# FurkanOM/tf-ssd

Measured on AMD Instinct MI355X. Metric: images/sec SSD300 (MobileNetV2) fwd+NMS, higher is better.
Workload: dtype f32

## Files before the change

### include/ssd_hip.h

```cpp
#ifndef SSD_HIP_H
#define SSD_HIP_H

#include <stddef.h>
#include <stdint.h>

#ifdef __cplusplus
extern "C" {
#endif

#define SSD_OK 0
#define SSD_E_INVALID (-1)
#define SSD_E_HIP (-2)
#define SSD_E_UNSUPPORTED (-3)
#define SSD_E_STATE (-4)

const char* ssd_version(void);
const char* ssd_last_error(void);
int ssd_init(int device);
void* ssd_stream_create(int high_priority);
void* ssd_stream_create_masked(const unsigned* cu_mask, int words);
int ssd_stream_destroy(void* stream);

int ssd_priors_count(const int* fmaps, const int* n_ars, int levels);
int ssd_priors(const int* fmaps, const float* const* ars, const int* n_ars, int levels,
// ... 320 lines not shown
int ssd_iou_loc_loss(const float* priors_dev, const float* variances, const float* actual_deltas_dev,
                     const float* pred_deltas_dev, int B, int N, int mode, float loc_loss_alpha,
                     float* loc_loss_dev, float* per_anchor_out_dev, float* grad_deltas_dev, float grad_scale,
                     void* workspace_dev, size_t workspace_bytes, void* stream);

#define SSD_LOSS_HARD_NEGATIVE 0
#define SSD_LOSS_FOCAL 1
typedef struct ssd_loss_config {
    int kind;
    float neg_pos_ratio, loc_loss_alpha, focal_alpha, focal_gamma;
    int loc_kind;
    const float* priors_dev;
    float variances[4];
} ssd_loss_config;
size_t ssd_loss_config_bytes(void);


enum ssd_act { SSD_ACT_NONE = 0, SSD_ACT_RELU = 1, SSD_ACT_RELU6 = 2 };

typedef struct ssd_conv_desc {
    int B, H, W, Cin;
    int Cout, kh, kw;
    int stride, dilation;
    int pad_t, pad_l, pad_b, pad_r;
    int act;
    int has_residual;
} ssd_conv_desc;

int ssd_same_pads(int in, int k, int stride, int dilation, int* before, int* after);
int ssd_conv_out_size(int in, int k, int stride, int dilation, int pad_before, int pad_after);

size_t ssd_conv_packed_weight_floats(int kh, int kw, int Cin, int Cout);
int ssd_conv_pack_weights(const float* hwio_dev, int kh, int kw, int Cin, int Cout,
                          float* packed_dev, void* stream);

int ssd_conv2d(const ssd_conv_desc* d, const float* in_dev, const float* packed_w_dev,
               const float* scale_dev, const float* shift_dev, const float* residual_dev,
               float* out_dev, long out_batch_stride, long out_pixel_stride, void* stream);

int ssd_conv_num_configs(void);
const char* ssd_conv_config_name(int config);
int ssd_conv2d_ex(const ssd_conv_desc* d, const float* in_dev, const float* packed_w_dev,
                  const float* scale_dev, const float* shift_dev, const float* residual_dev,
                  float* out_dev, long out_batch_stride, long out_pixel_stride, int config,
                  int split_k, float* splitk_ws_dev, void* stream);

int ssd_split_planes(const float* x_dev, long n, int channels, int planes, void* planes_dev, long plane_stride, void* stream);
int ssd_join_planes(const void* planes_dev, long n, int channels, int planes, long plane_stride, float* x_dev, void* stream);
int ssd_conv2d_planes(const ssd_conv_desc* d, const void* in_planes_dev, int planes, long in_plane_stride,
                      const float* packed_w_dev, const float* scale_dev, const float* shift_dev,
                      const float* residual_dev, float* out_dev, long out_batch_stride, long out_pixel_stride,
                      void* out_planes_dev, long out_plane_stride, int config, int split_k,
                      float* splitk_ws_dev, void* stream);

size_t ssd_conv_wino_weight_floats(int Cin, int Cout);
int ssd_conv_wino_pack_weights(const float* hwio_dev, int Cin, int Cout, float* wino_w_dev, void* stream);
int ssd_conv_wino_num_configs(void);
int ssd_conv2d_wino(const ssd_conv_desc* d, const float* in_dev, const float* wino_w_dev,
                    const float* scale_dev, const float* shift_dev, float* out_dev,
                    long out_batch_stride, long out_pixel_stride, int wino_config, int split_k,
                    float* splitk_ws_dev, void* stream);

int ssd_dwconv3x3(const float* in_dev, int B, int H, int W, int C, int stride,
                  int pad_t, int pad_l, int pad_b, int pad_r,
                  const float* w_dev, const float* scale_dev, const float* shift_dev,
                  int act, float* out_dev, void* stream);

int ssd_maxpool2d(const float* in_dev, int B, int H, int W, int C, int k, int stride,
                  int pad_t, int pad_l, int pad_b, int pad_r, float* out_dev, void* stream);

int ssd_l2norm(const float* in_dev, long pixels, int C, const float* gamma_dev,
               float* out_dev, void* stream);

int ssd_softmax(const float* in_dev, long rows, int L, float* out_dev, void* stream);

typedef struct ssd_net ssd_net;

enum ssd_backbone { SSD_MOBILENET_V2 = 0, SSD_VGG16 = 1 };

ssd_net* ssd_net_create(int backbone, int img_size, int levels, const int* n_ars,
                        int total_labels);
void ssd_net_destroy(ssd_net* net);

int ssd_net_num_params(const ssd_net* net);
const char* ssd_net_param_name(const ssd_net* net, int i);
int ssd_net_param_rank(const ssd_net* net, int i);
const int* ssd_net_param_shape(const ssd_net* net, int i);
int ssd_net_set_param(ssd_net* net, const char* name, const float* host_data, size_t count);
int ssd_net_get_param(const ssd_net* net, const char* name, float* host_out, size_t count);
int ssd_net_finalize(ssd_net* net, int max_batch);
long ssd_net_get_tuning(const ssd_net* net, char* buf, size_t cap);
int ssd_net_set_tuning(ssd_net* net, const char* text);
int ssd_net_tuning_stats(const ssd_net* net, int* from_table, int* timed);
int ssd_net_memory_bytes(const ssd_net* net, size_t out[4]);
const char* ssd_build_id(void);
int ssd_net_num_priors(const ssd_net* net);
int ssd_net_feature_map_size(const ssd_net* net, int level);

int ssd_net_forward(ssd_net* net, const float* image_dev, int B, float* deltas_out_dev,
                    float* probs_out_dev, void* stream);

int ssd_net_predict(ssd_net* net, const float* image_dev, int B, const float* priors_dev,
                    const float* var, int max_total, float iou_thr, float score_thr,
                    float* boxes_dev, float* labels_dev, float* scores_dev, int* valid_dev,
                    void* stream);
int ssd_net_predict_cfg(ssd_net* net, const float* image_dev, int B, const float* priors_dev, const float* var,
// ... 77 lines not shown
```

### tf-ssd_amd/csrc/ssd_bf16x3.h

```cpp
#pragma once
#include <hip/hip_runtime.h>

namespace ssd {

typedef float b3_f32x4 __attribute__((ext_vector_type(4)));
typedef short bf16x8 __attribute__((ext_vector_type(8)));

struct B3 {
    bf16x8 h, m, l;
};

__device__ __forceinline__ void split1(float x, short& h, short& m, short& l) {
    const unsigned hb = __float_as_uint(x) & 0xffff0000u;
    const float r1 = x - __uint_as_float(hb);
    const unsigned mb = __float_as_uint(r1) & 0xffff0000u;
    const float r2 = r1 - __uint_as_float(mb);
    h = (short)(hb >> 16);
    m = (short)(mb >> 16);
    l = (short)(__float_as_uint(r2) >> 16);
}
__device__ __forceinline__ void split4(const b3_f32x4 v, uint2& h, uint2& m, uint2& l) {
    unsigned hb[4], mb[4], lb[4];
#pragma unroll
    for (int j = 0; j < 4; ++j) {
        hb[j] = __float_as_uint(v[j]) & 0xffff0000u;
        const float r1 = v[j] - __uint_as_float(hb[j]);
        mb[j] = __float_as_uint(r1) & 0xffff0000u;
        lb[j] = __float_as_uint(r1 - __uint_as_float(mb[j]));
    }
    h = make_uint2(__builtin_amdgcn_perm(hb[1], hb[0], 0x07060302u), __builtin_amdgcn_perm(hb[3], hb[2], 0x07060302u));
    m = make_uint2(__builtin_amdgcn_perm(mb[1], mb[0], 0x07060302u), __builtin_amdgcn_perm(mb[3], mb[2], 0x07060302u));
    l = make_uint2(__builtin_amdgcn_perm(lb[1], lb[0], 0x07060302u), __builtin_amdgcn_perm(lb[3], lb[2], 0x07060302u));
}
__device__ __forceinline__ B3 split3(const b3_f32x4 a, const b3_f32x4 b) {
    B3 r;
#pragma unroll
    for (int j = 0; j < 4; ++j) {
        short h, m, l;
        split1(a[j], h, m, l);
        r.h[j] = h; r.m[j] = m; r.l[j] = l;
        split1(b[j], h, m, l);
        r.h[4 + j] = h; r.m[4 + j] = m; r.l[4 + j] = l;
    }
    return r;
}
__device__ __forceinline__ b3_f32x4 mma6(const B3& w, const B3& x, b3_f32x4 acc) {
    acc = __builtin_amdgcn_mfma_f32_16x16x32_bf16(w.m, x.m, acc, 0, 0, 0);
    acc = __builtin_amdgcn_mfma_f32_16x16x32_bf16(w.h, x.l, acc, 0, 0, 0);
    acc = __builtin_amdgcn_mfma_f32_16x16x32_bf16(w.l, x.h, acc, 0, 0, 0);
    acc = __builtin_amdgcn_mfma_f32_16x16x32_bf16(w.h, x.m, acc, 0, 0, 0);
    acc = __builtin_amdgcn_mfma_f32_16x16x32_bf16(w.m, x.h, acc, 0, 0, 0);
    acc = __builtin_amdgcn_mfma_f32_16x16x32_bf16(w.h, x.h, acc, 0, 0, 0);
    return acc;
}

typedef __bf16 bf16x2_t __attribute__((ext_vector_type(2)));
typedef float b3_f32x2 __attribute__((ext_vector_type(2)));

__device__ __forceinline__ unsigned rne2(float a, float b) {
    const bf16x2_t r = __builtin_convertvector(b3_f32x2{a, b}, bf16x2_t);
    return __builtin_bit_cast(unsigned, r);
}
__device__ __forceinline__ short rne1(float a) { return (short)(rne2(a, 0.f) & 0xffffu); }
__device__ __forceinline__ uint2 rne4(const b3_f32x4 v) { return make_uint2(rne2(v[0], v[1]), rne2(v[2], v[3])); }

template <int NP>
struct BP {
    bf16x8 p[NP];
};
template <int NP>
__device__ __forceinline__ BP<NP> splitN(const b3_f32x4 a, const b3_f32x4 b) {
    BP<NP> r;
    if constexpr (NP == 3) {
        const B3 s = split3(a, b);
        r.p[0] = s.h; r.p[1] = s.m; r.p[2] = s.l;
    } else {
        const uint4 u = make_uint4(rne2(a[0], a[1]), rne2(a[2], a[3]), rne2(b[0], b[1]), rne2(b[2], b[3]));
        r.p[0] = __builtin_bit_cast(bf16x8, u);
    }
    return r;
}
template <int NP>
__device__ __forceinline__ b3_f32x4 mmaN(const BP<NP>& w, const BP<NP>& x, b3_f32x4 acc) {
    if constexpr (NP == 3) {
        acc = __builtin_amdgcn_mfma_f32_16x16x32_bf16(w.p[1], x.p[1], acc, 0, 0, 0);
        acc = __builtin_amdgcn_mfma_f32_16x16x32_bf16(w.p[0], x.p[2], acc, 0, 0, 0);
        acc = __builtin_amdgcn_mfma_f32_16x16x32_bf16(w.p[2], x.p[0], acc, 0, 0, 0);
        acc = __builtin_amdgcn_mfma_f32_16x16x32_bf16(w.p[0], x.p[1], acc, 0, 0, 0);
        acc = __builtin_amdgcn_mfma_f32_16x16x32_bf16(w.p[1], x.p[0], acc, 0, 0, 0);
    }
    return __builtin_amdgcn_mfma_f32_16x16x32_bf16(w.p[0], x.p[0], acc, 0, 0, 0);
}
__device__ __forceinline__ void pack_planes(float x, int bf16_mode, short& h, short& m, short& l) {
    if (bf16_mode) { h = rne1(x); m = 0; l = 0; }
    else split1(x, h, m, l);
}

__device__ __host__ __forceinline__ long plane_elem(const long pix, const int c, const long P) {
    return (((long)(c >> 5) * P + pix) << 5) + (c & 31);
}
__device__ __forceinline__ void store_planes4(short* __restrict__ op, const long plane, const int np, const long pix, const int c,
                                              const long P, const b3_f32x4 v) {
    const long e = plane_elem(pix, c, P);
    if (np == 1) {
        *reinterpret_cast<uint2*>(op + e) = rne4(v);
    } else {
        uint2 h, m, l;
        split4(v, h, m, l);
        *reinterpret_cast<uint2*>(op + e) = h;
        *reinterpret_cast<uint2*>(op + plane + e) = m;
        *reinterpret_cast<uint2*>(op + 2 * plane + e) = l;
    }
}
__device__ __forceinline__ void store_planes4_lin(short* __restrict__ op, const long plane, const int np, const long e, const int C,
                                                  const long P, const b3_f32x4 v) {
    const long pix = e / C;
    store_planes4(op, plane, np, pix, (int)(e - pix * C), P, v);
}

}
```

### tf-ssd_amd/csrc/ssd_conv.h

```cpp
#pragma once
#include "common.h"

namespace ssd {

struct ConvParams {
    const float* in;
    const float* w;
    const short* w3;
    const float* scale;
    const float* shift;
    const float* residual;
    float* out;
    int B, H, W, Cin, Ho, Wo, Cout;
    int kh, kw, stride, dil, pad_t, pad_l;
    int K, Kpad, Npad;
    long M;
    long out_batch_stride, out_pixel_stride;
    int n_split;
    float* out2;
    long out2_batch_stride, out2_pixel_stride;
    int vec_store2;
    int act;
    int vec_store;
    int split_k;
    float* partial;
    const float* wino_w;
    int bf16;
    const short* xp;
    long xp_plane;
    int xp_np;
    short* op;
    long op_plane;
    int op_np;
};
bool conv_config_allowed(int cfg, int precision);
inline int conv_vec_store(const ConvParams& p) {
    return (((uintptr_t)p.out & 15) == 0) && (p.out_pixel_stride % 4 == 0) && (p.out_batch_stride % 4 == 0);
}

struct FusedBlockParams {
    const float* x;
    float* y;
    const float* we;
    const float *es, *eh;
    const float* wd;
    const float *ds, *dh;
    const float* wp;
    const float *ps, *ph;
    int residual;
    int B, H, W, Cin, Ce, Cout, Ho, Wo, stride, pad_t, pad_l;
    int kpad_e, kpad_p, npad_p;
    int tiles_y, tiles_x;
    int bf16;
    int groups;
    const short* we3;
    const short* wp3;
    int bands;
    float* slabs;
    unsigned* tickets;
    float* e_out;
    short* y_planes;
    long y_plane;
    short* e_planes;
    long e_plane;
    int planes_np;
    int planes_only;
    int form2;
};
struct StemParams {
    const float* x;
    float* y;
    const float* w1;
    const float *s1, *h1;
    const float* wd;
    const float *sd, *hd;
    const float* wp;
    const float *sp, *hp;
    int B, H, W, H1, W1, pad_t, pad_l, kpad1, kpadp;
    int tiles_y, tiles_x;
    int bf16;
};
struct DwProjParams {
    const float* e;
    const float* wd;
    const float* dh;
    const float* wp;
    const float* ph;
    const float* res;
    float* y;
    int B, H, W, Ce, Cout, Ho, Wo, stride, pad_t, pad_l;
    int kpad_p, npad_p;
    int tiles_y, tiles_x;
    int bf16;
};
bool dwproj_supported(const DwProjParams& p);
int launch_dwproj(DwProjParams p, hipStream_t st);
bool stem_supported(const StemParams& p);
int launch_stem(StemParams p, hipStream_t st);
bool image_block2_supported(const FusedBlockParams& p);
int launch_image_block2(FusedBlockParams p, hipStream_t st);
bool fused_block_supported(const FusedBlockParams& p);
int launch_fused_block(FusedBlockParams p, hipStream_t st);
bool band3_block_supported(const FusedBlockParams& p);
size_t band3_we_shorts(int Ce);
size_t band3_wp_shorts(int npad_p, int Ce);
int launch_band3_pack(const float* we, int Ce, int Cin, int kpad_e, short* we3, const float* wp, int npad_p, int kpad_p,
                      short* wp3, hipStream_t st);
int launch_band3_block(FusedBlockParams p, hipStream_t st);
bool band_block_supported(const FusedBlockParams& p);
int launch_band_block(FusedBlockParams p, hipStream_t st);
bool image_block_supported(const FusedBlockParams& p);
bool image_block_split_fits(FusedBlockParams p);
int image_block_groups(const FusedBlockParams& p, int B);
size_t image_block_slab_floats(const FusedBlockParams& p, int B);
int launch_image_block(FusedBlockParams p, hipStream_t st);

inline int round_up(int v, int a) { return (v + a - 1) / a * a; }
inline int conv_kpad(int K) { return round_up(K, 32); }
inline int conv_npad(int Cout) { return round_up(Cout, 16); }

int conv_num_configs();
const char* conv_config_name(int cfg);
bool conv_config_valid(int cfg, const ConvParams& p);
int conv_pick_config(const ConvParams& p);
long conv_grid_blocks(int cfg, const ConvParams& p);
int conv_k_tiles(int cfg, const ConvParams& p);
int conv_launch(const ConvParams& p, int cfg, hipStream_t st);
size_t conv_splitk_workspace_floats(const ConvParams& p, int cfg);

int fill_conv_params(const ssd_conv_desc* d, ConvParams* p);
int launch_splitk_reduce(const ConvParams& p, hipStream_t st);

int conv_num_mfma_configs();
int wino_num_configs();
const char* wino_config_name(int i);
bool wino_applicable(const ConvParams& p);
bool wino_config_valid(int i, const ConvParams& p);
long wino_grid_blocks(int i, const ConvParams& p);
int wino_k_tiles(const ConvParams& p);
int wino_launch(const ConvParams& p, int i, hipStream_t st);
size_t wino_weight_floats(int Cin, int Cout);
int launch_wino_pack(const float* hwio, int Cin, int Cout, int Npad, int row_off, float* U, hipStream_t st);

int skinny_num_configs();
const char* skinny_config_name(int i);
bool skinny_config_valid(int i, const ConvParams& p);
long skinny_grid_blocks(int i, const ConvParams& p);
int skinny_launch(const ConvParams& p, int i, hipStream_t st);

int mfma3_num_configs();
const char* mfma3_config_name(int i);
bool mfma3_config_valid(int i, const ConvParams& p);
long mfma3_grid_blocks(int i, const ConvParams& p);
int mfma3_k_tiles(const ConvParams& p);
void mfma3_tile(int i, int* BM, int* BN);
int mfma3_launch(const ConvParams& p, int i, hipStream_t st, bool bf16 = false);
const char* bf16_config_name(int i);

int dma_num_configs();
const char* dma_config_name(int i, int np);
bool dma_config_valid(int i, int np, const ConvParams& p);
long dma_grid_blocks(int i, const ConvParams& p);
int dma_k_tiles(int np, const ConvParams& p);
void dma_tile(int i, int* BM, int* BN);
int dma_launch(const ConvParams& p, int i, int np, hipStream_t st);
int launch_split_planes(const float* x, long n, int C, int np, short* planes, long plane, hipStream_t st);
int launch_join_planes(const short* planes, long n, int C, int np, long plane, float* x, hipStream_t st);
bool conv_config_is_dma(int cfg);
bool conv_config_writes_planes(int cfg, const ConvParams& p);

int launch_dwconv3x3(const float* in, int B, int H, int W, int C, int stride, int pad_t, int pad_l,
                     int Ho, int Wo, const float* w, const float* scale, const float* shift, int act,
                     float* out, hipStream_t st);
int launch_maxpool(const float* in, int B, int H, int W, int C, int k, int stride, int pad_t, int pad_l,
                   int Ho, int Wo, float* out, hipStream_t st, short* planes = nullptr, long plane = 0, int np = 0);
int launch_l2norm(const float* in, long pixels, int C, const float* gamma, float* out, hipStream_t st,
                  short* planes = nullptr, long plane = 0, int np = 0);
int launch_softmax(const float* in, long rows, int L, float* out, hipStream_t st);
bool decode_nms_fused_ok(int L);
int decode_nms_fused(const float* deltas, const float* logits, const float* priors, const float* var, int B, int N, int L,
                     int max_per_class, int max_total, float iou_thr, float score_thr, float* boxes, float* labels,
                     float* scores, int* valid, void* ws, size_t ws_bytes, int ws_batch, hipStream_t st);
int decode_nms_fused_cfg(const float* deltas, const float* logits, const float* priors, const float* var, int B, int N, int L,
                         const ssd_nms_config* cfg, float* boxes, float* labels, float* scores, int* valid, void* ws,
                         size_t ws_bytes, int ws_batch, hipStream_t st);
int launch_pack_weights(const float* hwio, int K, int Cout, int Kpad, int Npad, float* packed, hipStream_t st);
inline size_t conv_packed_floats(int K, int Cout) {
    const size_t n = (size_t)conv_kpad(K) * conv_npad(Cout);
    return n + 2 * n;
}
inline const short* conv_split_planes(const float* packed, int K, int Cout) {
    return reinterpret_cast<const short*>(packed + (size_t)conv_kpad(K) * conv_npad(Cout));
}
int launch_pack_split(float* packed, int K, int Cout, hipStream_t st, bool row_major = false);
int launch_scale_rows(const float* in, const float* scale, int rows, int nvalid, int cols, float* out, hipStream_t st);
int launch_scale_cols(const float* in, const float* scale, int rows, int cols, float* out, hipStream_t st);
int launch_fold_bn(const float* gamma, const float* beta, const float* mean, const float* var, float eps,
                   int C, float* scale, float* shift, hipStream_t st);

}
```

### tf-ssd_amd/csrc/ssd_conv.hip

```cpp
#include "ssd_conv.h"
#include "ssd_conv_mfma.h"

namespace ssd {


template <int V>
__global__ void splitk_reduce_kernel(const ConvParams p) {
    const long total = p.M * p.Cout;
    const long groups = total / V;
    const int HoWo = p.Ho * p.Wo;
    for (long g = (long)blockIdx.x * blockDim.x + threadIdx.x; g < groups; g += (long)gridDim.x * blockDim.x) {
        float t[V];
#pragma unroll
        for (int j = 0; j < V; ++j) t[j] = 0.f;
        for (int s = 0; s < p.split_k; ++s) {
            const float* src = p.partial + (long)s * total + g * V;
            if (V == 4) {
                const f32x4 v = *reinterpret_cast<const f32x4*>(src);
#pragma unroll
                for (int j = 0; j < V; ++j) t[j] += v[j];
            } else {
                t[0] += src[0];
            }
        }
// ... 168 lines not shown
struct ConvCfg {
    const char* name;
    int BM, BN, BK;
    conv_kernel_t gemm, general;
};
#define CFG(MT, NT, WM, WN, BK)                                                            \
    {"mfma_" #MT "x" #NT "_" #WM "x" #WN "_k" #BK, 16 * MT * WM, 16 * NT * WN, BK,          \
     conv_mfma_kernel<MT, NT, WM, WN, BK, true>, conv_mfma_kernel<MT, NT, WM, WN, BK, false>}
static const ConvCfg kCfgs[] = {
    CFG(2, 1, 4, 1, 32),
    CFG(2, 2, 4, 1, 32),
    CFG(2, 4, 4, 1, 32),
    CFG(2, 6, 4, 1, 32),
    CFG(2, 4, 2, 2, 32),
    CFG(1, 2, 2, 2, 32),
    CFG(4, 4, 2, 2, 32),
    CFG(1, 1, 4, 1, 32),
    CFG(2, 9, 4, 1, 32),
    CFG(2, 12, 4, 1, 32),
    CFG(1, 4, 1, 4, 32),
    CFG(2, 2, 2, 2, 32),
    CFG(2, 6, 4, 1, 16),
    CFG(1, 2, 1, 4, 32),
    CFG(4, 2, 4, 1, 32),
    CFG(2, 8, 2, 2, 32),
    CFG(2, 7, 4, 1, 32),
    CFG(2, 5, 2, 2, 32),
    CFG(1, 7, 4, 1, 32),
    CFG(1, 5, 2, 2, 32),
    CFG(4, 3, 2, 2, 32),
    CFG(4, 6, 2, 2, 32),
    CFG(1, 7, 4, 1, 64),
    CFG(1, 5, 2, 2, 64),
    CFG(2, 7, 4, 1, 64),
    CFG(2, 5, 2, 2, 64),
    CFG(1, 2, 2, 2, 64),
    CFG(2, 4, 2, 2, 64),
    CFG(1, 1, 4, 1, 64),
    CFG(2, 2, 2, 2, 64),
    CFG(4, 5, 2, 2, 32),
    CFG(4, 7, 4, 1, 32),
    CFG(4, 4, 4, 1, 32),
    CFG(4, 6, 4, 1, 32),
    CFG(4, 3, 4, 1, 32),
    CFG(4, 5, 4, 1, 32),
    CFG(2, 10, 2, 2, 32),
};
constexpr int kNumMfmaCfgs = sizeof(kCfgs) / sizeof(kCfgs[0]);
static int skinny_cfg0() { return kNumMfmaCfgs + wino_num_configs(); }
static int mfma3_cfg0() { return kNumMfmaCfgs + wino_num_configs() + skinny_num_configs(); }
static int bf16_cfg0() { return kNumMfmaCfgs + wino_num_configs() + skinny_num_configs() + mfma3_num_configs(); }
static int dma3_cfg0() { return kNumMfmaCfgs + wino_num_configs() + skinny_num_configs() + 2 * mfma3_num_configs(); }
static int dmab_cfg0() { return dma3_cfg0() + dma_num_configs(); }
static int direct_cfg() { return dma3_cfg0() + 2 * dma_num_configs(); }
#define kSkinnyCfg0 skinny_cfg0()
#define kMfma3Cfg0 mfma3_cfg0()
#define kBf16Cfg0 bf16_cfg0()
#define kDma3Cfg0 dma3_cfg0()
#define kDmabCfg0 dmab_cfg0()
#define kDirectCfg direct_cfg()
bool conv_config_is_dma(int cfg) { return cfg >= kDma3Cfg0 && cfg < kDirectCfg; }
bool conv_config_writes_planes(int cfg, const ConvParams& p) {
    if (cfg == kDirectCfg) return stem_ok(p);
    return (cfg >= 0 && cfg < kNumMfmaCfgs) || (cfg >= kMfma3Cfg0 && cfg < kDirectCfg);
}

int conv_num_mfma_configs() { return kNumMfmaCfgs; }
int conv_num_configs() { return kDirectCfg + 1; }
const char* conv_config_name(int cfg) {
    if (cfg == kDirectCfg) return "direct_valu";
    if (cfg >= kDmabCfg0 && cfg < kDirectCfg) return dma_config_name(cfg - kDmabCfg0, 1);
    if (cfg >= kDma3Cfg0 && cfg < kDmabCfg0) return dma_config_name(cfg - kDma3Cfg0, 3);
    if (cfg >= kBf16Cfg0 && cfg < kDma3Cfg0) return bf16_config_name(cfg - kBf16Cfg0);
    if (cfg >= kMfma3Cfg0 && cfg < kBf16Cfg0) return mfma3_config_name(cfg - kMfma3Cfg0);
    if (cfg >= kSkinnyCfg0 && cfg < kMfma3Cfg0) return skinny_config_name(cfg - kSkinnyCfg0);
    if (cfg >= kNumMfmaCfgs && cfg < kSkinnyCfg0) return wino_config_name(cfg - kNumMfmaCfgs);
    if (cfg < 0 || cfg >= kNumMfmaCfgs) return "?";
    return kCfgs[cfg].name;
}

bool conv_config_allowed(int cfg, int precision) {
    const bool bf16 = (cfg >= kBf16Cfg0 && cfg < kDma3Cfg0) || (cfg >= kDmabCfg0 && cfg < kDirectCfg);
    if (!precision) return !bf16;
    const bool split = (cfg >= kMfma3Cfg0 && cfg < kBf16Cfg0) || (cfg >= kDma3Cfg0 && cfg < kDmabCfg0);
    const bool wino = cfg >= kNumMfmaCfgs && cfg < kSkinnyCfg0;
    return !split && !wino;
}

static bool is_gemm1x1(const ConvParams& p) {
    return p.kh == 1 && p.kw == 1 && p.stride == 1 && p.pad_t == 0 && p.pad_l == 0 && p.Ho == p.H && p.Wo == p.W;
}

bool conv_config_valid(int cfg, const ConvParams& p) {
    if (cfg == kDirectCfg) return (size_t)p.K * ((p.Cout + 3) & ~3) * 4 <= 64 * 1024;
    if (cfg >= kDmabCfg0 && cfg < kDirectCfg) return dma_config_valid(cfg - kDmabCfg0, 1, p);
    if (cfg >= kDma3Cfg0 && cfg < kDmabCfg0) return dma_config_valid(cfg - kDma3Cfg0, 3, p);
    if (cfg >= kBf16Cfg0 && cfg < kDma3Cfg0) return mfma3_config_valid(cfg - kBf16Cfg0, p);
    if (cfg >= kMfma3Cfg0 && cfg < kBf16Cfg0) return mfma3_config_valid(cfg - kMfma3Cfg0, p);
    if (cfg >= kSkinnyCfg0 && cfg < kMfma3Cfg0) return skinny_config_valid(cfg - kSkinnyCfg0, p);
    if (cfg >= kNumMfmaCfgs && cfg < kSkinnyCfg0) return wino_config_valid(cfg - kNumMfmaCfgs, p);
    if (cfg < 0 || cfg >= kNumMfmaCfgs) return false;
    if (((uintptr_t)p.in & 15) || ((uintptr_t)p.w & 15)) return false;
    if (p.Cin % 4) return false;
    if (p.M > 0x7fffffffL - 1024) return false;
    if (is_gemm1x1(p)) return true;
    if (p.kh * p.kw > 32) return false;
    return p.Cin % kCfgs[cfg].BK == 0;
}

int conv_pick_config(const ConvParams& p) {
    int best = -1;
    double best_cost = 1e300;
    for (int c = 0; c < kNumMfmaCfgs; ++c) {
        if (!conv_config_valid(c, p)) continue;
        const ConvCfg& g = kCfgs[c];
        const double mb = (double)((p.M + g.BM - 1) / g.BM), nb = (double)((p.Cout + g.BN - 1) / g.BN);
        const double kk = (double)round_up(p.K, g.BK);
        const double blocks = mb * nb;
        const double waves = ceil(blocks / 256.0);
        const double t_mfma = waves * (double)g.BM * g.BN * kk * 2.0 / (157.3e12 / 256.0);
        const double bytes = (mb * g.BM * kk * nb + nb * g.BN * kk * mb) * 4.0 + (double)p.M * p.Cout * 4.0;
        const double t_mem = bytes / 6.0e12;
        const double cost = (t_mfma > t_mem ? t_mfma : t_mem) + 0.25 * (t_mfma < t_mem ? t_mfma : t_mem);
        if (cost < best_cost) { best_cost = cost; best = c; }
    }
    if (p.w3 && p.M >= 2048 && p.K >= 64) {
        for (int c = 0; c < mfma3_num_configs(); ++c) {
            if (!mfma3_config_valid(c, p)) continue;
            int BM, BN;
            mfma3_tile(c, &BM, &BN);
            const double mb = (double)((p.M + BM - 1) / BM), nb = (double)((p.Cout + BN - 1) / BN);
            const double kk = (double)round_up(p.K, 32);
            const double waves = ceil(mb * nb / 256.0);
            const double t_mfma = waves * (double)BM * BN * kk * 2.0 / ((p.bf16 ? 1000e12 : 260e12) / 256.0);
            const double bytes = mb * BM * kk * nb * 4.0 + nb * BN * kk * mb * (p.bf16 ? 2.0 : 6.0) + (double)p.M * p.Cout * 4.0;
            const double t_mem = bytes / 6.0e12;
            const double cost = (t_mfma > t_mem ? t_mfma : t_mem) + 0.25 * (t_mfma < t_mem ? t_mfma : t_mem);
            if (cost < best_cost) { best_cost = cost; best = (p.bf16 ? kBf16Cfg0 : kMfma3Cfg0) + c; }
        }
    }
    if (best < 0 && conv_config_valid(kDirectCfg, p)) best = kDirectCfg;
    return best;
}

long conv_grid_blocks(int cfg, const ConvParams& p) {
    if (cfg >= kDmabCfg0 && cfg < kDirectCfg) return dma_grid_blocks(cfg - kDmabCfg0, p);
    if (cfg >= kDma3Cfg0 && cfg < kDmabCfg0) return dma_grid_blocks(cfg - kDma3Cfg0, p);
    if (cfg >= kBf16Cfg0 && cfg < kDma3Cfg0) return mfma3_grid_blocks(cfg - kBf16Cfg0, p);
    if (cfg >= kMfma3Cfg0 && cfg < kBf16Cfg0) return mfma3_grid_blocks(cfg - kMfma3Cfg0, p);
    if (cfg >= kSkinnyCfg0 && cfg < kMfma3Cfg0) return skinny_grid_blocks(cfg - kSkinnyCfg0, p);
    if (cfg >= kNumMfmaCfgs && cfg < kSkinnyCfg0) return wino_grid_blocks(cfg - kNumMfmaCfgs, p);
    if (cfg < 0 || cfg >= kNumMfmaCfgs) return 0;
    const ConvCfg& g = kCfgs[cfg];
    return ((p.M + g.BM - 1) / g.BM) * ((p.Cout + g.BN - 1) / g.BN);
}
int conv_k_tiles(int cfg, const ConvParams& p) {
    if (cfg >= kDma3Cfg0 && cfg < kDirectCfg) return dma_k_tiles(cfg >= kDmabCfg0 ? 1 : 3, p);
    if (cfg >= kMfma3Cfg0 && cfg < kDma3Cfg0) return mfma3_k_tiles(p);
    if (cfg >= kSkinnyCfg0 && cfg < kMfma3Cfg0) return p.K / 16;
    if (cfg >= kNumMfmaCfgs && cfg < kSkinnyCfg0) return wino_k_tiles(p);
    if (cfg < 0 || cfg >= kNumMfmaCfgs) return 0;
    return (p.K + kCfgs[cfg].BK - 1) / kCfgs[cfg].BK;
}

size_t conv_splitk_workspace_floats(const ConvParams& p, int) {
    return p.split_k > 1 ? (size_t)p.split_k * p.M * p.Cout : 0;
}

int conv_launch(const ConvParams& p, int cfg, hipStream_t st) {
    if (p.M == 0 || p.Cout == 0) return SSD_OK;
    if (!conv_config_valid(cfg, p)) {
        set_error("conv2d: config %d (%s) cannot run Cin=%d k=%dx%d stride=%d", cfg, conv_config_name(cfg),
                  p.Cin, p.kh, p.kw, p.stride);
        return SSD_E_UNSUPPORTED;
    }
    SSD_UNSUPPORTED_IF(!p.out && !(p.op && !p.n_split && (p.Cout & 3) == 0 && conv_config_writes_planes(cfg, p)),
                       "conv2d: config %s cannot write a plane-only output", conv_config_name(cfg));
    if (cfg >= kDma3Cfg0 && cfg < kDirectCfg) {
        const bool b1 = cfg >= kDmabCfg0;
        const int rc = dma_launch(p, cfg - (b1 ? kDmabCfg0 : kDma3Cfg0), b1 ? 1 : 3, st);
        if (rc || p.split_k <= 1) return rc;
        return launch_splitk_reduce(p, st);
    }
    if (cfg >= kMfma3Cfg0 && cfg < kDma3Cfg0) {
        const bool bf16 = cfg >= kBf16Cfg0;
        const int rc = mfma3_launch(p, cfg - (bf16 ? kBf16Cfg0 : kMfma3Cfg0), st, bf16);
        if (rc || p.split_k <= 1) return rc;
        return launch_splitk_reduce(p, st);
    }
    if (cfg >= kSkinnyCfg0 && cfg < kMfma3Cfg0) return skinny_launch(p, cfg - kSkinnyCfg0, st);
    if (cfg >= kNumMfmaCfgs && cfg < kSkinnyCfg0) {
        const int rc = wino_launch(p, cfg - kNumMfmaCfgs, st);
        if (rc || p.split_k <= 1) return rc;
        return launch_splitk_reduce(p, st);
    }
    if (cfg == kDirectCfg && stem_ok(p)) {
        constexpr int PX = 2;
        const long blocks = cdiv(p.M, 256 * PX);
        dim3 grid((unsigned)(blocks < 65535 ? blocks : 65535), p.Cout / 32);
        hipLaunchKernelGGL(conv_stem_kernel<PX>, grid, dim3(256), 0, st, p);
        SSD_LAUNCH_CHECK();
        return SSD_OK;
    }
    if (cfg == kDirectCfg) {
        const long total = p.M * ((p.Cout + 3) / 4);
        const int blocks = (int)(cdiv(total, 256) < 8192 ? cdiv(total, 256) : 8192);
        const size_t lds = (size_t)p.K * ((p.Cout + 3) & ~3) * 4;
        hipLaunchKernelGGL(conv_direct_kernel, dim3(blocks), dim3(256), lds, st, p);
        SSD_LAUNCH_CHECK();
        return SSD_OK;
    }
    const ConvCfg& g = kCfgs[cfg];
    const long mb = (p.M + g.BM - 1) / g.BM;
    const int nb = (p.Cout + g.BN - 1) / g.BN;
    SSD_UNSUPPORTED_IF(mb * nb > 0x7fffffffL, "conv2d: grid too large");
    dim3 grid((unsigned)(mb * nb), p.split_k > 1 ? p.split_k : 1);
    conv_kernel_t k = is_gemm1x1(p) ? g.gemm : g.general;
    hipLaunchKernelGGL(k, grid, dim3(256), 0, st, p);
    SSD_LAUNCH_CHECK();
    if (p.split_k > 1) return launch_splitk_reduce(p, st);
    return SSD_OK;
}

int launch_splitk_reduce(const ConvParams& p, hipStream_t st) {
    const long total = p.M * p.Cout;
    const bool vec = (total % 4 == 0) && (((uintptr_t)p.partial & 15) == 0);
    SSD_UNSUPPORTED_IF(!vec && !p.out, "conv2d: a plane-only output needs the 4-wide split-K reduce (16-byte aligned workspace)");
    const long groups = vec ? total / 4 : total;
    const int blocks = (int)(cdiv(groups, 256) < 8192 ? cdiv(groups, 256) : 8192);
    if (vec) hipLaunchKernelGGL(splitk_reduce_kernel<4>, dim3(blocks), dim3(256), 0, st, p);
    else hipLaunchKernelGGL(splitk_reduce_kernel<1>, dim3(blocks), dim3(256), 0, st, p);
// ... 64 lines not shown
    if (kh < 1 || kw < 1 || Cin < 1 || Cout < 1) return 0;
    return conv_packed_floats(kh * kw * Cin, Cout);
}

int ssd_conv_pack_weights(const float* hwio_dev, int kh, int kw, int Cin, int Cout, float* packed_dev,
                          void* stream) {
    SSD_CHECK_ARG(hwio_dev && packed_dev, "ssd_conv_pack_weights: NULL pointer");
    SSD_CHECK_ARG(kh >= 1 && kw >= 1 && Cin >= 1 && Cout >= 1, "ssd_conv_pack_weights: bad shape");
    const int K = kh * kw * Cin;
    int rc = launch_pack_weights(hwio_dev, K, Cout, conv_kpad(K), conv_npad(Cout), packed_dev, (hipStream_t)stream);
    if (!rc) rc = launch_pack_split(packed_dev, K, Cout, (hipStream_t)stream);
    return rc;
}

int ssd_conv_num_configs(void) { return conv_num_configs(); }
const char* ssd_conv_config_name(int cfg) { return conv_config_name(cfg); }

int ssd_conv2d_ex(const ssd_conv_desc* d, const float* in_dev, const float* packed_w_dev,
                  const float* scale_dev, const float* shift_dev, const float* residual_dev, float* out_dev,
                  long out_batch_stride, long out_pixel_stride, int config, int split_k,
                  float* splitk_ws_dev, void* stream) {
    ConvParams p;
    int rc = fill_conv_params(d, &p);
    if (rc) return rc;
    if (p.M == 0) return SSD_OK;
    SSD_CHECK_ARG(in_dev && packed_w_dev && out_dev, "conv2d: NULL pointer");
    SSD_CHECK_ARG(!d->has_residual || residual_dev, "conv2d: has_residual set but residual is NULL");
    p.in = in_dev; p.w = packed_w_dev; p.scale = scale_dev; p.shift = shift_dev;
    p.w3 = conv_split_planes(packed_w_dev, p.K, p.Cout);
    p.residual = d->has_residual ? residual_dev : nullptr;
    p.out = out_dev;
    p.out_pixel_stride = out_pixel_stride > 0 ? out_pixel_stride : p.Cout;
    p.out_batch_stride = out_batch_stride > 0 ? out_batch_stride : (long)p.Ho * p.Wo * p.out_pixel_stride;
    p.vec_store = (((uintptr_t)out_dev & 15) == 0) && (p.out_pixel_stride % 4 == 0) && (p.out_batch_stride % 4 == 0);
    if (split_k > 1) {
        SSD_CHECK_ARG(splitk_ws_dev != nullptr, "conv2d: split_k > 1 needs a workspace");
        p.split_k = split_k;
        p.partial = splitk_ws_dev;
    }
    const int cfg = config >= 0 ? config : conv_pick_config(p);
    SSD_UNSUPPORTED_IF(cfg < 0, "conv2d: no kernel for Cin=%d Cout=%d k=%dx%d", p.Cin, p.Cout, p.kh, p.kw);
    if (cfg == conv_num_configs() - 1) p.split_k = 1;
    return conv_launch(p, cfg, (hipStream_t)stream);
}

int ssd_split_planes(const float* x_dev, long n, int channels, int planes, void* planes_dev, long plane_stride, void* stream) {
    SSD_CHECK_ARG(x_dev && planes_dev && n >= 0, "ssd_split_planes: bad arguments");
    SSD_CHECK_ARG(plane_stride >= n && plane_stride % 8 == 0, "ssd_split_planes: plane_stride %ld must be >= n and a multiple of 8", plane_stride);
    SSD_CHECK_ARG((((uintptr_t)x_dev | (uintptr_t)planes_dev) & 15) == 0, "ssd_split_planes: pointers must be 16-byte aligned");
    return launch_split_planes(x_dev, n, channels, planes, static_cast<short*>(planes_dev), plane_stride, (hipStream_t)stream);
}

int ssd_join_planes(const void* planes_dev, long n, int channels, int planes, long plane_stride, float* x_dev, void* stream) {
    SSD_CHECK_ARG(x_dev && planes_dev && n >= 0 && (planes == 1 || planes == 3) && plane_stride >= n, "ssd_join_planes: bad arguments");
    return launch_join_planes(static_cast<const short*>(planes_dev), n, channels, planes, plane_stride, x_dev, (hipStream_t)stream);
}

int ssd_conv2d_planes(const ssd_conv_desc* d, const void* in_planes_dev, int planes, long in_plane_stride,
                      const float* packed_w_dev, const float* scale_dev, const float* shift_dev, const float* residual_dev,
                      float* out_dev, long out_batch_stride, long out_pixel_stride, void* out_planes_dev,
                      long out_plane_stride, int config, int split_k, float* splitk_ws_dev, void* stream) {
    ConvParams p;
    int rc = fill_conv_params(d, &p);
    if (rc) return rc;
    if (p.M == 0) return SSD_OK;
    SSD_CHECK_ARG(in_planes_dev && packed_w_dev && (out_dev || out_planes_dev), "conv2d_planes: NULL pointer");
    SSD_CHECK_ARG(planes == 1 || planes == 3, "conv2d_planes: planes must be 1 (bf16 mode) or 3 (exact split)");
    SSD_CHECK_ARG(in_plane_stride >= (long)p.B * p.H * p.W * p.Cin, "conv2d_planes: in_plane_stride shorter than the tensor");
    SSD_CHECK_ARG(!d->has_residual || residual_dev, "conv2d_planes: has_residual set but residual is NULL");
    SSD_CHECK_ARG(config >= 0 && config < conv_num_configs() && conv_config_is_dma(config), "conv2d_planes: config %d is not an LDS-DMA tile", config);
    p.xp = static_cast<const short*>(in_planes_dev); p.xp_plane = in_plane_stride; p.xp_np = planes;
    p.bf16 = planes == 1;
    p.w = packed_w_dev; p.scale = scale_dev; p.shift = shift_dev;
    p.w3 = conv_split_planes(packed_w_dev, p.K, p.Cout);
    p.residual = d->has_residual ? residual_dev : nullptr;
    p.out = out_dev;
    p.out_pixel_stride = out_pixel_stride > 0 ? out_pixel_stride : p.Cout;
    p.out_batch_stride = out_batch_stride > 0 ? out_batch_stride : (long)p.Ho * p.Wo * p.out_pixel_stride;
    p.vec_store = (((uintptr_t)out_dev & 15) == 0) && (p.out_pixel_stride % 4 == 0) && (p.out_batch_stride % 4 == 0);
    if (out_planes_dev) {
        SSD_CHECK_ARG(p.out_pixel_stride == p.Cout && p.out_batch_stride == (long)p.Ho * p.Wo * p.Cout && p.Cout % 4 == 0,
                      "conv2d_planes: plane output needs a dense [B,Ho,Wo,Cout] destination with Cout %% 4 == 0");
        SSD_CHECK_ARG(out_plane_stride >= p.M * ((p.Cout + 31) / 32 * 32) && out_plane_stride % 8 == 0 && ((uintptr_t)out_planes_dev & 7) == 0,
                      "conv2d_planes: bad out_plane_stride (whole 32-channel slices of all %ld pixels) or unaligned planes", p.M);
        p.op = static_cast<short*>(out_planes_dev); p.op_plane = out_plane_stride; p.op_np = planes;
    }
    if (split_k > 1) {
        SSD_CHECK_ARG(splitk_ws_dev != nullptr, "conv2d_planes: split_k > 1 needs a workspace");
        p.split_k = split_k;
        p.partial = splitk_ws_dev;
    }
    return conv_launch(p, config, (hipStream_t)stream);
}

size_t ssd_conv_wino_weight_floats(int Cin, int Cout) {
    if (Cin < 1 || Cout < 1) return 0;
    return wino_weight_floats(Cin, Cout);
}

int ssd_conv_wino_pack_weights(const float* hwio_dev, int Cin, int Cout, float* wino_w_dev, void* stream) {
    SSD_CHECK_ARG(hwio_dev && wino_w_dev && Cin >= 1 && Cout >= 1, "ssd_conv_wino_pack_weights: bad arguments");
    SSD_HIP(hipMemsetAsync(wino_w_dev, 0, wino_weight_floats(Cin, Cout) * sizeof(float), (hipStream_t)stream));
    return launch_wino_pack(hwio_dev, Cin, Cout, conv_npad(Cout), 0, wino_w_dev, (hipStream_t)stream);
}

int ssd_conv_wino_num_configs(void) { return wino_num_configs(); }

int ssd_conv2d_wino(const ssd_conv_desc* d, const float* in_dev, const float* wino_w_dev, const float* scale_dev,
                    const float* shift_dev, float* out_dev, long out_batch_stride, long out_pixel_stride,
                    int wino_config, int split_k, float* splitk_ws_dev, void* stream) {
    ConvParams p;
    int rc = fill_conv_params(d, &p);
    if (rc) return rc;
    if (p.M == 0) return SSD_OK;
    SSD_CHECK_ARG(in_dev && wino_w_dev && out_dev, "conv2d_wino: NULL pointer");
    SSD_CHECK_ARG(!d->has_residual, "conv2d_wino: residual is not supported");
    p.in = in_dev; p.wino_w = wino_w_dev; p.scale = scale_dev; p.shift = shift_dev;
    p.out = out_dev;
    p.out_pixel_stride = out_pixel_stride > 0 ? out_pixel_stride : p.Cout;
    p.out_batch_stride = out_batch_stride > 0 ? out_batch_stride : (long)p.Ho * p.Wo * p.out_pixel_stride;
// ... 21 lines not shown
```

### tf-ssd_amd/csrc/ssd_convdma.hip

```cpp
#include "ssd_block_common.h"
#include "ssd_conv_mfma.h"

namespace ssd {

template <int MT, int NT, int WM, int WN, int NP, bool GEMM1X1>
__device__ __forceinline__ void conv_dma_body(const ConvParams& p, char* __restrict__ dsm) {
    constexpr int KS = NP == 1 ? 2 : 1;
    constexpr int WPL = NP == 1 ? 3 : 0;
    constexpr int BM = 16 * MT * WM, BN = 16 * NT * WN, NW = WM * WN;
    constexpr int RBX = BM / 16, RBW = BN / 16;
    constexpr int RPX = (RBX + NW - 1) / NW, RPW = (RBW + NW - 1) / NW;
    constexpr int XBYTES = KS * NP * BM * 64, STAGE = KS * NP * (BM + BN) * 64;

    const int tid = threadIdx.x, lane = tid & 63;
    const int wave = __builtin_amdgcn_readfirstlane(tid >> 6);
    const int wm = wave / WN, wn = wave % WN;
    const int nb_n = (p.Cout + BN - 1) / BN;
    const int mblk = blockIdx.x / nb_n, nblk = blockIdx.x - mblk * nb_n;
    const long m0 = (long)mblk * BM;
    const int n0 = nblk * BN;
    const int HoWo = p.Ho * p.Wo;
    const int ntaps = p.kh * p.kw;

    const int r16 = lane >> 2;
    const int q8 = ((lane & 3) ^ ((lane >> 3) & 3)) * 8;
    const int b_first = (int)(m0 / HoWo);
    const long npix = (long)p.B * p.H * p.W;
    const long xbase_e = (GEMM1X1 ? m0 : (long)b_first * p.H * p.W) * 32;
    const long xrange = min((long)0x7fffffffL, (npix * p.Cin - xbase_e) * 2);
    const int slice_b = (int)(npix * 64);
    __amdgpu_buffer_rsrc_t xrs[NP];
#pragma unroll
    for (int pl = 0; pl < NP; ++pl)
        xrs[pl] = __builtin_amdgcn_make_buffer_rsrc(const_cast<short*>(p.xp + pl * p.xp_plane + xbase_e), 0, (int)xrange, 0x00020000);
    const long wplane_b = (long)p.Npad * p.Kpad * 2;
    const __amdgpu_buffer_rsrc_t wrs = __builtin_amdgcn_make_buffer_rsrc(const_cast<short*>(p.w3), 0, (int)(4 * wplane_b), 0x00020000);

    int xoff[RPX];
    unsigned xvalid[RPX];
#pragma unroll
    for (int j = 0; j < RPX; ++j) {
        const int rb = wave + j * NW;
        const long m = m0 + rb * 16 + r16;
        xoff[j] = 0;
        xvalid[j] = 0;
        if (rb < RBX && m < p.M) {
            if (GEMM1X1) {
                xoff[j] = ((rb * 16 + r16) * 32 + q8) * 2;
                xvalid[j] = 1u;
            } else {
                const int b = (int)(m / HoWo);
                const int pix = (int)(m - (long)b * HoWo);
                const int oy = pix / p.Wo, ox = pix - oy * p.Wo;
                const int iy0 = oy * p.stride - p.pad_t, ix0 = ox * p.stride - p.pad_l;
                xoff[j] = ((((b - b_first) * p.H + iy0) * p.W + ix0) * 32 + q8) * 2;
                for (int ky = 0; ky < p.kh; ++ky)
                    for (int kx = 0; kx < p.kw; ++kx) {
                        const int iy = iy0 + ky * p.dil, ix = ix0 + kx * p.dil;
                        if ((unsigned)iy < (unsigned)p.H && (unsigned)ix < (unsigned)p.W) xvalid[j] |= 1u << (ky * p.kw + kx);
                    }
            }
        }
    }
    int woff[RPW];
#pragma unroll
    for (int j = 0; j < RPW; ++j) {
        const int rb = wave + j * NW;
        const int r = min(rb * 16 + r16, min(BN, p.Npad - n0) - 1);
        woff[j] = ((n0 + r) * 32 + q8) * 2;
    }

    const int nks = p.K / 32;
    const int ntiles = GEMM1X1 ? (nks + KS - 1) / KS : ntaps * (p.Cin / (32 * KS));
    int kt_begin = 0, kt_end = ntiles;
    if (p.split_k > 1) {
        const int per = (ntiles + p.split_k - 1) / p.split_k;
        kt_begin = blockIdx.y * per;
        kt_end = min(ntiles, kt_begin + per);
    }
    int l_k0 = 0, l_tap = 0, l_ci = 0, l_ky = 0, l_kx = 0, l_xtile = 0, l_xs = 0;
    auto tile_setup = [&](int kt) {
        if (GEMM1X1) {
            l_k0 = kt * 32 * KS;
            l_xtile = 0;
            l_xs = kt * KS * slice_b;
        } else {
            const int cs = kt / ntaps;
            l_tap = kt - cs * ntaps;
            l_ci = cs * 32 * KS;
            l_ky = l_tap / p.kw;
            l_kx = l_tap - l_ky * p.kw;
            l_k0 = l_tap * p.Cin + l_ci;
            l_xtile = (l_ky * p.dil * p.W + l_kx * p.dil) * 64;
            l_xs = (l_ci >> 5) * slice_b;
        }
    };
    auto tile_advance = [&]() {
        if (GEMM1X1) {
            l_k0 += 32 * KS;
            l_xs += KS * slice_b;
        } else {
            ++l_tap;
            if (++l_kx == p.kw) { l_kx = 0; ++l_ky; }
            if (l_tap == ntaps) { l_tap = 0; l_ky = 0; l_kx = 0; l_ci += 32 * KS; }
            l_k0 = l_tap * p.Cin + l_ci;
            l_xtile = (l_ky * p.dil * p.W + l_kx * p.dil) * 64;
            l_xs = (l_ci >> 5) * slice_b;
        }
    };
    auto steps_here = [&]() -> int { return KS == 1 ? 1 : min(KS, nks - l_k0 / 32); };

    auto issue = [&](int stage) {
        char* sb = dsm + stage * STAGE;
        const int ns = steps_here();
#pragma unroll
        for (int j = 0; j < RPX; ++j) {
            const int rb = wave + j * NW;
            if (RBX % NW != 0 && rb >= RBX) continue;
            const bool ok = GEMM1X1 ? (xvalid[j] != 0) : (((xvalid[j] >> l_tap) & 1u) != 0);
            const int vo = ok ? xoff[j] + l_xtile : (int)0x80000000;
#pragma unroll
            for (int s = 0; s < KS; ++s) {
                if (KS > 1 && s >= ns) break;
#pragma unroll
                for (int pl = 0; pl < NP; ++pl)
                    __builtin_amdgcn_raw_ptr_buffer_load_lds(xrs[pl], (lds_dst_t)(sb + ((s * NP + pl) * BM + rb * 16) * 64), 16, vo, l_xs + s * slice_b, 0, 0);
            }
        }
#pragma unroll
        for (int j = 0; j < RPW; ++j) {
            const int rb = wave + j * NW;
            if (RBW % NW != 0 && rb >= RBW) continue;
#pragma unroll
            for (int s = 0; s < KS; ++s) {
                if (KS > 1 && s >= ns) break;
#pragma unroll
                for (int pl = 0; pl < NP; ++pl)
                    __builtin_amdgcn_raw_ptr_buffer_load_lds(wrs, (lds_dst_t)(sb + XBYTES + ((s * NP + pl) * BN + rb * 16) * 64), 16, woff[j],
                                                             (int)((pl + WPL) * wplane_b) + ((l_k0 >> 5) + s) * p.Npad * 64, 0, 0);
            }
        }
    };

    f32x4 acc[MT][NT];
#pragma unroll
    for (int mi = 0; mi < MT; ++mi)
#pragma unroll
        for (int ni = 0; ni < NT; ++ni) acc[mi][ni] = f32x4{0.f, 0.f, 0.f, 0.f};

    const int frow = lane & 15;
    const int fq = ((lane >> 4) ^ ((frow >> 1) & 3)) << 4;
    auto mma_tile = [&](int stage, int ns) {
        const char* sb = dsm + stage * STAGE;
#pragma unroll
        for (int s = 0; s < KS; ++s) {
            if (KS > 1 && s >= ns) break;
            const char* Xb = sb + s * NP * BM * 64;
            const char* Wb = sb + XBYTES + s * NP * BN * 64;
            BP<NP> b[MT];
#pragma unroll
            for (int mi = 0; mi < MT; ++mi) {
                const char* r = Xb + ((wm * MT + mi) * 16 + frow) * 64 + fq;
#pragma unroll
                for (int pl = 0; pl < NP; ++pl) b[mi].p[pl] = *reinterpret_cast<const bf16x8*>(r + pl * BM * 64);
            }
#pragma unroll
            for (int ni = 0; ni < NT; ++ni) {
                const char* r = Wb + ((wn * NT + ni) * 16 + frow) * 64 + fq;
                BP<NP> a;
#pragma unroll
                for (int pl = 0; pl < NP; ++pl) a.p[pl] = *reinterpret_cast<const bf16x8*>(r + pl * BN * 64);
#pragma unroll
                for (int mi = 0; mi < MT; ++mi) acc[mi][ni] = mmaN<NP>(a, b[mi], acc[mi][ni]);
            }
        }
    };

    int ns_cur = 1;
    if (kt_begin < kt_end) {
        tile_setup(kt_begin);
        ns_cur = steps_here();
        issue(0);
    }
    asm volatile("s_waitcnt vmcnt(0)" ::: "memory");
    __syncthreads();
    for (int kt = kt_begin; kt < kt_end; ++kt) {
        const int stage = (kt - kt_begin) & 1;
        int ns_next = 1;
        if (kt + 1 < kt_end) {
            tile_advance();
            ns_next = steps_here();
            issue(stage ^ 1);
        }
        mma_tile(stage, ns_cur);
        ns_cur = ns_next;
        asm volatile("s_waitcnt vmcnt(0)" ::: "memory");
        __syncthreads();
    }
    conv_epilogue<MT, NT>(p, acc, m0, n0, wm, wn, lane, HoWo);
}

template <int MT, int NT, int WM, int WN, int NP, bool GEMM1X1>
__global__ __launch_bounds__(64 * WM * WN) void conv_dma_kernel(const ConvParams p) {
    extern __shared__ __attribute__((aligned(1024))) char dsm_dma[];
    conv_dma_body<MT, NT, WM, WN, NP, GEMM1X1>(p, dsm_dma);
}

namespace {

typedef void (*convd_kernel_t)(const ConvParams);
struct ConvDCfg {
    const char* name3;
    const char* name1;
    int BM, BN, threads;
    convd_kernel_t gemm3, general3, gemm1, general1;
};
#define DCFG(MT, NT, WM, WN)                                                                                  \
    {"dma3_" #MT "x" #NT "_" #WM "x" #WN, "dmab_" #MT "x" #NT "_" #WM "x" #WN, 16 * MT * WM, 16 * NT * WN, 64 * WM * WN, \
     conv_dma_kernel<MT, NT, WM, WN, 3, true>, conv_dma_kernel<MT, NT, WM, WN, 3, false>,                       \
     conv_dma_kernel<MT, NT, WM, WN, 1, true>, conv_dma_kernel<MT, NT, WM, WN, 1, false>}
const ConvDCfg kCfgD[] = {
    DCFG(4, 4, 4, 2),
    DCFG(2, 4, 4, 2),
    DCFG(4, 4, 2, 4),
    DCFG(4, 2, 4, 2),
    DCFG(2, 7, 8, 1),
    DCFG(4, 5, 4, 2),
    DCFG(4, 4, 2, 2),
    DCFG(2, 7, 4, 1),
    DCFG(2, 5, 2, 2),
    DCFG(2, 4, 6, 2),
    DCFG(3, 4, 4, 3),
    DCFG(2, 4, 8, 2),
    DCFG(2, 2, 2, 2),
    DCFG(2, 5, 6, 2),
};
constexpr int kNumCfgD = sizeof(kCfgD) / sizeof(kCfgD[0]);

bool cd_gemm1x1(const ConvParams& p) {
    return p.kh == 1 && p.kw == 1 && p.stride == 1 && p.pad_t == 0 && p.pad_l == 0 && p.Ho == p.H && p.Wo == p.W;
}

__global__ __launch_bounds__(256) void split_planes_kernel(const float* __restrict__ x, const long n4, const int C, const int np,
                                                           short* __restrict__ planes, const long plane) {
    const long P = n4 * 4 / C;
    for (long e = (long)blockIdx.x * 256 + threadIdx.x; e < n4; e += (long)gridDim.x * 256)
        store_planes4_lin(planes, plane, np, e * 4, C, P, *reinterpret_cast<const f32x4*>(x + e * 4));
}

__global__ __launch_bounds__(256) void join_planes_kernel(const short* __restrict__ planes, const long n, const int C, const int np,
                                                          const long plane, float* __restrict__ x) {
    const long P = n / C;
    for (long e = (long)blockIdx.x * 256 + threadIdx.x; e < n; e += (long)gridDim.x * 256) {
        const long pix = e / C;
        const long s = plane_elem(pix, (int)(e - pix * C), P);
        float v = __uint_as_float((unsigned)(unsigned short)planes[s] << 16);
        if (np == 3) {
            v += __uint_as_float((unsigned)(unsigned short)planes[plane + s] << 16);
            v += __uint_as_float((unsigned)(unsigned short)planes[2 * plane + s] << 16);
        }
        x[e] = v;
    }
}

}

int dma_num_configs() { return kNumCfgD; }
const char* dma_config_name(int i, int np) { return (i >= 0 && i < kNumCfgD) ? (np == 1 ? kCfgD[i].name1 : kCfgD[i].name3) : "?"; }
bool dma_config_valid(int i, int np, const ConvParams& p) {
    if (i < 0 || i >= kNumCfgD) return false;
    if (!p.xp || !p.w3 || p.xp_np != np) return false;
    if (((uintptr_t)p.xp & 15) || ((uintptr_t)p.w3 & 15) || (p.xp_plane & 7)) return false;
    if (p.M > 0x7fffffffL - 1024) return false;
    if (4 * (long)p.Npad * p.Kpad * 2 > 0x7fffffffL) return false;
    if ((long)p.B * p.H * p.W * p.Cin * 2 > 0x7fffffffL) return false;
    if (cd_gemm1x1(p)) return p.Cin % 32 == 0;
    if (p.kh * p.kw > 32) return false;
    if (((long)kCfgD[i].BM / (p.Ho * p.Wo) + 3) * p.H * p.W * 64 > 0x3fffffffL) return false;
    return p.Cin % (np == 1 ? 64 : 32) == 0;
}
long dma_grid_blocks(int i, const ConvParams& p) {
    if (i < 0 || i >= kNumCfgD) return 0;
    return ((p.M + kCfgD[i].BM - 1) / kCfgD[i].BM) * ((p.Cout + kCfgD[i].BN - 1) / kCfgD[i].BN);
}
int dma_k_tiles(int np, const ConvParams& p) { return (p.K + 31) / 32 / (np == 1 ? 2 : 1); }
void dma_tile(int i, int* BM, int* BN) {
    *BM = (i >= 0 && i < kNumCfgD) ? kCfgD[i].BM : 0;
    *BN = (i >= 0 && i < kNumCfgD) ? kCfgD[i].BN : 0;
}

int dma_launch(const ConvParams& p, int i, int np, hipStream_t st) {
    if (!dma_config_valid(i, np, p)) {
        set_error("conv2d: LDS-DMA config %d cannot run Cin=%d k=%dx%d (input planes %s)", i, p.Cin, p.kh, p.kw, p.xp ? "present" : "missing");
        return SSD_E_UNSUPPORTED;
    }
    const long blocks = dma_grid_blocks(i, p);
    SSD_UNSUPPORTED_IF(blocks > 0x7fffffffL, "conv2d: grid too large");
    const ConvDCfg& g = kCfgD[i];
    const convd_kernel_t fn = np == 1 ? (cd_gemm1x1(p) ? g.gemm1 : g.general1) : (cd_gemm1x1(p) ? g.gemm3 : g.general3);
    const int lds = 2 * (np == 1 ? 2 : 3) * (g.BM + g.BN) * 64;
    if (lds > 64 * 1024) SSD_HIP(hipFuncSetAttribute(reinterpret_cast<const void*>(fn), hipFuncAttributeMaxDynamicSharedMemorySize, lds));
    dim3 grid((unsigned)blocks, p.split_k > 1 ? p.split_k : 1);
    hipLaunchKernelGGL(fn, grid, dim3(g.threads), lds, st, p);
    SSD_LAUNCH_CHECK();
    return SSD_OK;
}

int launch_split_planes(const float* x, long n, int C, int np, short* planes, long plane, hipStream_t st) {
    SSD_CHECK_ARG(n % 4 == 0 && (np == 1 || np == 3), "split_planes: element count %ld must be a multiple of 4, planes 1 or 3", n);
    SSD_CHECK_ARG(C > 0 && C % 32 == 0 && n % C == 0, "split_planes: %d channels (slice-major planes need a multiple of 32 that divides the %ld elements)", C, n);
    SSD_UNSUPPORTED_IF((((uintptr_t)x) & 15) || (((uintptr_t)planes) & 7) || (plane & 3),
                       "split_planes: needs a 16-byte aligned source and 8-byte aligned planes (16-byte loads, 8-byte stores)");
    if (n == 0) return SSD_OK;
    const long n4 = n / 4;
    const int blocks = (int)((n4 + 255) / 256 < 16384 ? (n4 + 255) / 256 : 16384);
    hipLaunchKernelGGL(split_planes_kernel, dim3(blocks), dim3(256), 0, st, x, n4, C, np, planes, plane);
    SSD_LAUNCH_CHECK();
    return SSD_OK;
}

int launch_join_planes(const short* planes, long n, int C, int np, long plane, float* x, hipStream_t st) {
    if (n == 0) return SSD_OK;
    SSD_CHECK_ARG(C > 0 && n % C == 0, "join_planes: %d channels do not divide the %ld elements", C, n);
    const int blocks = (int)((n + 255) / 256 < 16384 ? (n + 255) / 256 : 16384);
    hipLaunchKernelGGL(join_planes_kernel, dim3(blocks), dim3(256), 0, st, planes, n, C, np, plane, x);
    SSD_LAUNCH_CHECK();
    return SSD_OK;
}

}
```

### tf-ssd_amd/csrc/ssd_imgblock.hip

```cpp

#include "ssd_bf16x3.h"
#include "ssd_block_common.h"
#include "ssd_conv.h"

namespace ssd {

namespace {

constexpr int kIC = 16;
constexpr int kILD = 24;
constexpr int kIThreads = 512;

__device__ __forceinline__ void gstore16_sc1(float* ptr, f32x4 v) {
    asm volatile("global_store_dwordx4 %0, %1, off sc1\n\ts_nop 1" ::"v"(ptr), "v"(v) : "memory");
}

template <int CIN, int NT, int T, int S = 1>
__global__ __launch_bounds__(kIThreads) void mbv2_image_block_kernel(const FusedBlockParams p) {
    constexpr int TO = S == 1 ? T : 1;
    constexpr int KC = CIN / 16;
    constexpr int LDW = CIN + 8;
    constexpr int NCH = T == 1 ? 2 : 1;
    constexpr int WE_U = kIC * CIN / 4, WE_R = (WE_U + kIThreads - 1) / kIThreads;
    constexpr int WP_U = NT * 16 * kIC / 4, WP_R = (WP_U + kIThreads - 1) / kIThreads;
// ... 87 lines not shown
            opo[t] = opix[t];
            realo[t] = real[t];
        } else {
            const int Po = Wo + 1, tile = wave * TO + t;
            const int q = tile * 16 + l15;
            const int ro = q / Po, co = q - ro * Po;
            realo[t] = tile * 16 < Ho * Po && q < Ho * Po && co < Wo;
            qo[t] = (tile * 16 < Ho * Po && q < Ho * Po) ? (2 * ro - p.pad_t + 1) * P + (2 * co - p.pad_l + 1) : 0;
            opo[t] = realo[t] ? ro * Wo + co : 0;
        }
    }
    for (int u = tid; u < 11 * (CeG / 4); u += kIThreads) {
        const int row = u / (CeG / 4), c4 = (u - row * (CeG / 4)) * 4;
        const float* src = row == 0 ? p.eh : row == 10 ? p.dh : p.wd + (long)(row - 1) * p.Ce;
        *reinterpret_cast<f32x4*>(Ps + row * CeG + c4) = *reinterpret_cast<const f32x4*>(src + cbeg + c4);
    }
    wait_prefetch(wer0);
    store_we_from(wer0, 0);
    wait_prefetch(wpr);
    store_wp(0);
    if (nchunk > 1) { wait_prefetch(wer); store_we(1); }
    __syncthreads();

    auto expand = [&](int j) {
        f32x4 ea[T][NCH];
        const f32x4 sh = *reinterpret_cast<const f32x4*>(Ps + j * kIC + g4 * 4);
#pragma unroll
        for (int t = 0; t < T; ++t) {
            ea[t][0] = sh;
            if (NCH == 2) ea[t][NCH - 1] = f32x4{0.f, 0.f, 0.f, 0.f};
        }
        const float* wes = Wes + ((j & 1) * kIC + l15) * LDW + g4 * 4;
#pragma unroll
        for (int kc = 0; kc < KC; ++kc) {
            const f32x4 wa = *reinterpret_cast<const f32x4*>(wes + kc * 16);
#pragma unroll
            for (int s = 0; s < 4; ++s)
#pragma unroll
                for (int t = 0; t < T; ++t)
                    ea[t][kc % NCH] = __builtin_amdgcn_mfma_f32_16x16x4f32(wa[s], xb[t][kc][s], ea[t][kc % NCH], 0, 0, 0);
        }
        float* es = Es + ((j & 1) * NE + P + 1) * kILD + g4 * 4;
#pragma unroll
        for (int t = 0; t < T; ++t) {
            f32x4 v = ea[t][0];
            if (NCH == 2) v = v + ea[t][NCH - 1];
            const float hi = real[t] ? 6.0f : 0.0f;
#pragma unroll
            for (int e = 0; e < 4; ++e) v[e] = __builtin_amdgcn_fmed3f(v[e], 0.0f, hi);
            if (tvalid[t]) *reinterpret_cast<f32x4*>(es + qs[t] * kILD) = v;
            if (p.e_out && real[t]) {
                const long eo = ((long)img * H * W + opix[t]) * p.Ce + cbeg + j * kIC + g4 * 4;
                if (!(p.planes_only & 2)) *reinterpret_cast<f32x4*>(p.e_out + eo) = v;
                if (p.e_planes) store_planes4(p.e_planes, p.e_plane, p.planes_np, (long)img * H * W + opix[t], cbeg + j * kIC + g4 * 4, (long)B * H * W, v);
            }
        }
    };

    f32x4 acc[TO][NT];
#pragma unroll
    for (int t = 0; t < TO; ++t)
#pragma unroll
        for (int ni = 0; ni < NT; ++ni) acc[t][ni] = f32x4{0.f, 0.f, 0.f, 0.f};

    expand(0);
    if (nchunk > 1) {
        load_wp(1);
        if (nchunk > 2) load_we(2);
    }

    for (int i = 0; i < nchunk; ++i) {
        lds_barrier();
        if (i + 1 < nchunk) {
            wait_prefetch(wpr);
            store_wp((i + 1) & 1);
            if (i + 2 < nchunk) {
                wait_prefetch(wer);
                store_we(i & 1);
                load_wp(i + 2);
                if (i + 3 < nchunk) load_we(i + 3);
            }
        }
        f32x4 a[TO];
        {
            const f32x4 dh = *reinterpret_cast<const f32x4*>(Ps + 10 * CeG + i * kIC + g4 * 4);
#pragma unroll
            for (int t = 0; t < TO; ++t) a[t] = dh;
            const float* es = Es + ((i & 1) * NE + P + 1) * kILD + g4 * 4;
#pragma unroll
            for (int dy = -1; dy <= 1; ++dy)
#pragma unroll
                for (int dx = -1; dx <= 1; ++dx) {
                    const f32x4 w = *reinterpret_cast<const f32x4*>(Ps + (1 + (dy + 1) * 3 + dx + 1) * CeG + i * kIC + g4 * 4);
#pragma unroll
                    for (int t = 0; t < TO; ++t) {
                        const f32x4 e = *reinterpret_cast<const f32x4*>(es + (qo[t] + dy * P + dx) * kILD);
                        a[t] += e * w;
                    }
                }
#pragma unroll
            for (int t = 0; t < TO; ++t)
#pragma unroll
                for (int e = 0; e < 4; ++e) a[t][e] = __builtin_amdgcn_fmed3f(a[t][e], 0.0f, 6.0f);
        }
        __builtin_amdgcn_sched_barrier(0);
        {
            const float* wps = Wps + ((i & 1) * NT * 16 + l15) * kILD + g4 * 4;
// ... 192 lines not shown
            const int ro = q / Po, co = q - ro * Po;
            realo[t] = tile * 16 < Ho * Po && q < Ho * Po && co < Wo;
            qo[t] = (tile * 16 < Ho * Po && q < Ho * Po) ? (2 * ro - p.pad_t + 1) * P + (2 * co - p.pad_l + 1) : 0;
            opo[t] = realo[t] ? ro * Wo + co : 0;
        }
    }
    for (int u = tid; u < 11 * (CeG / 4); u += kIThreads) {
        const int row = u / (CeG / 4), c4 = (u - row * (CeG / 4)) * 4;
        const float* src = row == 0 ? p.eh : row == 10 ? p.dh : p.wd + (long)(row - 1) * p.Ce;
        *reinterpret_cast<f32x4*>(Ps + row * CeG + c4) = *reinterpret_cast<const f32x4*>(src + cbeg + c4);
    }
    {
        bf16x8 w0[WE_N], w1[WE_N];
        stage_we_load_to(w0, 0);
        stage_we_load_to(w1, nchunk > 1 ? 1 : 0);
        stage_wp_load(0);
        stage_we_store_from(w0, 0);
        stage_we_store_from(w1, 1);
        stage_wp_store();
        if (nchunk > 2) stage_we_load(2);
        if (nchunk > 2) stage_wp_load(1);
    }
    __syncthreads();

    auto expand = [&](int j) {
        f32x4 ea[T][NCH];
        const f32x4 sh = *reinterpret_cast<const f32x4*>(Ps + j * kIC + g4 * 4);
#pragma unroll
        for (int t = 0; t < T; ++t) {
            ea[t][0] = sh;
            if (NCH == 2) ea[t][NCH - 1] = f32x4{0.f, 0.f, 0.f, 0.f};
        }
        const short* wl = Wes + ((j & 1) * NP * 16 + l15) * SEH + g4 * 8;
#pragma unroll
        for (int ks = 0; ks < KS; ++ks) {
            BP<NP> wea;
#pragma unroll
            for (int pl = 0; pl < NP; ++pl) wea.p[pl] = *reinterpret_cast<const bf16x8*>(wl + pl * 16 * SEH + ks * 32);
#pragma unroll
            for (int t = 0; t < T; ++t) ea[t][ks % NCH] = mmaN<NP>(wea, xs[t][ks], ea[t][ks % NCH]);
        }
        float* es = Es + ((j & 1) * NE + P + 1) * kILD + g4 * 4;
#pragma unroll
        for (int t = 0; t < T; ++t) {
            f32x4 v = ea[t][0];
            if (NCH == 2) v = v + ea[t][NCH - 1];
            const float hi = real[t] ? 6.0f : 0.0f;
#pragma unroll
            for (int e = 0; e < 4; ++e) v[e] = __builtin_amdgcn_fmed3f(v[e], 0.0f, hi);
            if (tvalid[t]) *reinterpret_cast<f32x4*>(es + qs[t] * kILD) = v;
            if (p.e_out && real[t]) {
                const long eo = ((long)img * H * W + opix[t]) * p.Ce + cbeg + j * kIC + g4 * 4;
                if (!(p.planes_only & 2)) *reinterpret_cast<f32x4*>(p.e_out + eo) = v;
                if (p.e_planes) store_planes4(p.e_planes, p.e_plane, p.planes_np, (long)img * H * W + opix[t], cbeg + j * kIC + g4 * 4, (long)B * H * W, v);
            }
        }
    };

    f32x4 acc[TO][NT];
#pragma unroll
    for (int t = 0; t < TO; ++t)
#pragma unroll
        for (int ni = 0; ni < NT; ++ni) acc[t][ni] = f32x4{0.f, 0.f, 0.f, 0.f};

    expand(0);
    f32x4 dprev[TO];

    for (int i = 0; i < nchunk; ++i) {
        lds_barrier();
        const bool odd = i & 1;
        const bool flush = odd || i + 1 == nchunk;
        {
            if (i + 2 < nchunk) stage_we_store(i & 1);
            if (i + 3 < nchunk) stage_we_load(i + 3);
            if (!odd && i > 0 && i + 1 < nchunk) {
                stage_wp_store();
                if (i + 2 < nchunk) stage_wp_load((i >> 1) + 1);
            }
        }
        f32x4 a[TO];
        {
            const f32x4 dh = *reinterpret_cast<const f32x4*>(Ps + 10 * CeG + i * kIC + g4 * 4);
#pragma unroll
            for (int t = 0; t < TO; ++t) a[t] = dh;
            const float* es = Es + ((i & 1) * NE + P + 1) * kILD + g4 * 4;
#pragma unroll
            for (int dy = -1; dy <= 1; ++dy)
#pragma unroll
                for (int dx = -1; dx <= 1; ++dx) {
                    const f32x4 w = *reinterpret_cast<const f32x4*>(Ps + (1 + (dy + 1) * 3 + dx + 1) * CeG + i * kIC + g4 * 4);
#pragma unroll
                    for (int t = 0; t < TO; ++t) {
                        const f32x4 e = *reinterpret_cast<const f32x4*>(es + (qo[t] + (S == 1 ? dy * P + dx : dy * P + dx)) * kILD);
                        a[t] += e * w;
                    }
                }
#pragma unroll
            for (int t = 0; t < TO; ++t)
#pragma unroll
                for (int e = 0; e < 4; ++e) a[t][e] = __builtin_amdgcn_fmed3f(a[t][e], 0.0f, 6.0f);
        }
        if (!flush) {
#pragma unroll
            for (int t = 0; t < TO; ++t) dprev[t] = a[t];
        } else {
            BP<NP> d[TO];
#pragma unroll
// ... 194 lines not shown
```

### tf-ssd_amd/csrc/ssd_imgblock2.hip

```cpp

#include "ssd_bf16x3.h"
#include "ssd_block_common.h"
#include "ssd_conv.h"

namespace ssd {

namespace {

constexpr int kC = 16;

template <int CIN, int NT, int NW, int T, int H, int W, int NP, int LOOP, int S = 1>
__device__ __forceinline__ void image16v2_body(const FusedBlockParams& p, float* __restrict__ sm2) {
    static_assert(CIN % 32 == 0, "whole 32-channel k-steps");
    constexpr int NTH = NW * 64;
    constexpr int P = W + 1, Q = H * P;
    static_assert(NW * 16 * T >= Q, "the waves' pixel slots cover the padded map");
    constexpr int NPIX = NW * 16 * T;
    constexpr int NE = NPIX + 2 * P + 2;
    constexpr int ROW = S == 2 ? 20 : (T & 1) ? 24 : 20;
    static_assert(((S == 2 ? 2 : T) * ROW) % 16 == 8, "neighbouring lanes must sit 8 (mod 16) words apart");
    constexpr int TO = S == 1 ? T : 1;
    constexpr int Ho = S == 1 ? H : (H + 1) / 2, Wo = S == 1 ? W : (W + 1) / 2, Po = Wo + 1;
    static_assert(S == 1 || NW * 16 >= Ho * Po, "stride 2: one output pixel per lane covers the output map");
    constexpr int WPL = NP == 1 ? 3 : 0;
// ... 71 lines not shown
        const float* src = row == 0 ? p.eh : row == 10 ? p.dh : p.wd + (long)(row - 1) * p.Ce;
        const int w = c4 & 31, j = 2 * (c4 >> 5) + ((w >> 2) & 1), r = (w >> 3) * 4;
        *reinterpret_cast<f32x4*>(Ps + (j * 11 + row) * kC + r) = *reinterpret_cast<const f32x4*>(src + cbeg + c4);
    }
    dma_wait();
    __syncthreads();

    const float* e_rd = Es + (q0 + P + 1) * ROW + g4 * 4;
    float* e_wr = Es + (q0 + P + 1) * ROW + g4 * 4;
    const float* ps_l = Ps + g4 * 4;
    const int fslot = l15 * 32 + ((g4 ^ ((l15 >> 1) & 3)) * 8);
    const short* we_l = Wes + fslot;
    const short* wp_l = Wps + fslot;
    float relu_hi[T];
#pragma unroll
    for (int t = 0; t < T; ++t) relu_hi[t] = real[t] ? 6.0f : 0.0f;
    bool realo[TO];
    int opo[TO];
    if constexpr (S == 1) {
#pragma unroll
        for (int t = 0; t < T; ++t) { realo[t] = real[t]; opo[t] = opix[t]; }
    } else {
        const int qo = wave * 16 + l15, ro = qo / Po, co = qo - ro * Po;
        const bool in = qo < Ho * Po;
        realo[0] = in && co < Wo;
        opo[0] = realo[0] ? ro * Wo + co : 0;
        e_rd = Es + ((in ? (2 * ro - p.pad_t + 1) * P + (2 * co - p.pad_l + 1) : 0) + P + 1) * ROW + g4 * 4;
    }

    auto expand = [&](const int j, const int pb) {
        f32x4 ea[T];
        const f32x4 sh = *reinterpret_cast<const f32x4*>(ps_l + j * PCH);
#pragma unroll
        for (int t = 0; t < T; ++t) ea[t] = sh;
        const short* wl = we_l + pb * NBE * 512;
#pragma unroll
        for (int ks = 0; ks < KS; ++ks) {
            BP<NP> wea;
#pragma unroll
            for (int pl = 0; pl < NP; ++pl) wea.p[pl] = *reinterpret_cast<const bf16x8*>(wl + (pl * KS + ks) * 512);
#pragma unroll
            for (int t = 0; t < T; ++t) ea[t] = mmaN<NP>(wea, xs[t][ks], ea[t]);
        }
        float* ew = e_wr + pb * EBUF;
#pragma unroll
        for (int t = 0; t < T; ++t) {
            f32x4 v = ea[t];
#pragma unroll
            for (int e = 0; e < 4; ++e) v[e] = __builtin_amdgcn_fmed3f(v[e], 0.0f, relu_hi[t]);
            *reinterpret_cast<f32x4*>(ew + t * ROW) = v;
            if (S == 2 && p.e_out && real[t]) {
                const int ch = cbeg + (j >> 1) * 32 + g4 * 8 + (j & 1) * 4;
                if (!(p.planes_only & 2)) *reinterpret_cast<f32x4*>(p.e_out + ((long)img * (H * W) + opix[t]) * p.Ce + ch) = v;
                if (p.e_planes) store_planes4(p.e_planes, p.e_plane, p.planes_np, (long)img * (H * W) + opix[t], ch, (long)B * (H * W), v);
            }
        }
    };
    auto depthwise = [&](const int i, const int pb, f32x4 (&a)[TO]) {
        const float* pc = ps_l + i * PCH;
        const f32x4 dh = *reinterpret_cast<const f32x4*>(pc + 10 * kC);
#pragma unroll
        for (int t = 0; t < TO; ++t) a[t] = dh;
        const float* es = e_rd + pb * EBUF;
#pragma unroll
        for (int dy = -1; dy <= 1; ++dy) {
            f32x4 w[3], e[TO + 2];
#pragma unroll
            for (int dx = 0; dx < 3; ++dx) w[dx] = *reinterpret_cast<const f32x4*>(pc + (1 + (dy + 1) * 3 + dx) * kC);
#pragma unroll
            for (int j = 0; j < TO + 2; ++j)
                e[j] = *reinterpret_cast<const f32x4*>(es + (dy * P + j - 1) * ROW);
#pragma unroll
            for (int dx = 0; dx < 3; ++dx)
#pragma unroll
                for (int t = 0; t < TO; ++t) a[t] += e[t + dx] * w[dx];
        }
#pragma unroll
        for (int t = 0; t < TO; ++t)
#pragma unroll
            for (int e = 0; e < 4; ++e) a[t][e] = __builtin_amdgcn_fmed3f(a[t][e], 0.0f, 6.0f);
    };
    f32x4 acc[TO][NT];
#pragma unroll
    for (int t = 0; t < TO; ++t)
#pragma unroll
        for (int ni = 0; ni < NT; ++ni) acc[t][ni] = f32x4{0.f, 0.f, 0.f, 0.f};
    auto project = [&](const f32x4 (&a0)[TO], const f32x4 (&a1)[TO]) {
        BP<NP> d[TO];
#pragma unroll
        for (int t = 0; t < TO; ++t) d[t] = splitN<NP>(a0[t], a1[t]);
#pragma unroll
        for (int ni = 0; ni < NT; ++ni) {
            BP<NP> wa;
#pragma unroll
            for (int pl = 0; pl < NP; ++pl) wa.p[pl] = *reinterpret_cast<const bf16x8*>(wp_l + (pl * NT + ni) * 512);
#pragma unroll
            for (int t = 0; t < TO; ++t) acc[t][ni] = mmaN<NP>(wa, d[t], acc[t][ni]);
        }
    };

    expand(0, 0);

    if constexpr (LOOP == 0) {
        f32x4 dprev[TO];
        for (int c = 0; c < nchunk; ++c) {
            dma_wait();
            lds_barrier();
// ... 131 lines not shown
```

### tf-ssd_amd/csrc/ssd_net.h

```cpp
#pragma once
#include <map>
#include <set>
#include <string>
#include <vector>

#include "ssd_conv.h"

struct ssd_train_state;
void ssd_train_state_free(ssd_train_state*);

namespace ssd {

enum LayerKind { LK_CONV = 0, LK_DW, LK_POOL, LK_L2NORM, LK_SOFTMAX, LK_FUSED };
static const char* kKindName[] = {"conv", "dw", "pool", "l2norm", "softmax", "fused"};

enum Route { RT_OFF = 0, RT_LAYER, RT_STEM, RT_DWPROJ, RT_TILE, RT_BAND, RT_BAND3, RT_IMAGE, RT_IMAGE_SPLIT };

struct Param {
    std::string name;
    std::vector<int> shape;
    size_t count = 0;
    float* dev = nullptr;
    bool set = false;
    bool in_flat = false;
};

struct Tensor {
    std::string name;
    int H = 0, W = 0, C = 0;
    size_t per_image = 0;
    float* dev = nullptr;
    short* planes = nullptr;
    long plane_stride = 0;
    int planes_np = 0;
    bool planes_live = false;
    bool plane_only = false;
};

struct Layer {
    std::string name;
    LayerKind kind = LK_CONV;
    int in = -1, out = -1, res = -1;
    int H = 0, W = 0, Cin = 0, Ho = 0, Wo = 0, Cout = 0;
    int kh = 1, kw = 1, stride = 1, dil = 1, pt = 0, pl = 0, pb = 0, pr = 0, act = 0;
    int p_kernel = -1, p_bias = -1, p_bn = -1;
    int p_kernel2 = -1, p_bias2 = -1, Cout1 = 0;
    int p_gamma = -1;
    int head_kind = 0;
    long head_off = 0, head_bs = 0, head_ps = 0;
    long head2_off = 0, head2_bs = 0, head2_ps = 0;
    float* packed = nullptr;
    float* wino = nullptr;
    float* scale = nullptr;
    float* shift = nullptr;
    int cfg = -1;
    int split_k = 1;
    int f_expand = -1, f_dw = -1, f_project = -1;
    int f_type = 0;
    int fused_by = -1;
    int e_out = -1;
    int img_choice = -1;
    int fused_by2 = -1;
    Route route = RT_OFF;
    float* splitk_part = nullptr;
    float *fz_we = nullptr, *fz_wd = nullptr, *fz_wp = nullptr;
    float *fz_we3 = nullptr, *fz_wp3 = nullptr;
    int side = 0;
    hipEvent_t ev_ready = nullptr;
};

inline void conv_route_head(ConvParams& p, const Layer& l, float* probs, float* deltas) {
    p.out = probs + l.head_off;
    p.out_pixel_stride = l.head_ps;
    p.out_batch_stride = l.head_bs;
    p.n_split = l.Cout1;
    p.out2 = deltas + l.head2_off;
    p.out2_pixel_stride = l.head2_ps;
    p.out2_batch_stride = l.head2_bs;
    p.vec_store2 = (p.out2_pixel_stride % 4 == 0) && (p.out2_batch_stride % 4 == 0);
}

struct ScopedDev {
    float* p = nullptr;
    ~ScopedDev() { if (p) (void)hipFree(p); }
};
struct ScopedEvent {
    hipEvent_t e = nullptr;
    ~ScopedEvent() { if (e) (void)hipEventDestroy(e); }
};

struct Step {
    int layer = -1;
    int sid = -1;
    int wait[2] = {-1, -1};
    bool after_main = false;
    bool publishes = false;
    bool join_first = false;
};

}

struct ssd_net {
    int backbone = 0, img_size = 300, levels = 6, L = 21;
    std::vector<int> n_ars;
    std::vector<ssd::Param> params;
    std::map<std::string, int> param_index;
    std::vector<ssd::Tensor> tensors;
    std::map<std::string, int> tensor_index;
    std::vector<ssd::Layer> layers;
    std::vector<int> fmap;
    std::vector<long> level_off;
    int num_priors = 0;
    bool finalized = false;
    bool fuse_blocks = true;
    bool fuse_softmax = true;
    bool fuse_dwproj = true;
    bool use_wino = true;
    int precision = 0;
    int fuse_band = 2;
    int fuse_image = 1;
    int lanes_hint = 1;
    bool tail_on_side = false;
    bool image_split = true;
    bool image_v2 = true;
    bool conv_dma = true;
    bool plane_only = true;
    bool image_ticket = false;
    float* img_slabs = nullptr;
    unsigned* img_tickets = nullptr;
    int max_batch = 0;
    int last_batch = 0;
    std::vector<float*> owned;
    float* arena = nullptr;
    size_t arena_bytes = 0, plane_bytes = 0, slab_bytes = 0;
    float* splitk_ws = nullptr;
    size_t splitk_floats = 0;
    float* deltas = nullptr;
    float* probs = nullptr;
    void* nms_ws = nullptr;
    size_t nms_ws_bytes = 0;
    int nms_ws_batch = 0;
    int nms_ws_total = 0;
    int scratch_batch = 0;
    std::map<std::string, std::pair<std::string, int>> preset;
    int n_preset = 0;
    int n_autotuned = 0;
    bool launch_raced = false;
    bool use_graph = true;
    bool graphs_unsafe = false;
    bool use_graph_auto = true;
    struct GraphEntry {
        std::vector<const void*> key;
        hipGraphExec_t exec = nullptr;
        hipGraph_t graph = nullptr;
        const float* image = nullptr;
        int batch = 0;
    };
    std::vector<GraphEntry> graphs;
    hipStream_t gstream = nullptr;
    bool overlap_heads = true;
    static constexpr int kSides = 2;
    hipStream_t side[kSides] = {nullptr, nullptr};
    hipEvent_t ev_side_done[kSides] = {nullptr, nullptr};
    std::vector<ssd::Step> steps;
    float* splitk_layers = nullptr;
    bool timing = false;
    ssd_train_state* train = nullptr;
    std::set<std::string> frozen;
    unsigned trainable_rev = 0;
    std::vector<std::vector<hipEvent_t>> timing_events;

    ~ssd_net() {
        for (auto& p : params)
            if (p.dev && !p.in_flat) (void)hipFree(p.dev);
        if (train) ssd_train_state_free(train);
        for (float* p : owned)
            if (p) (void)hipFree(p);
        if (arena) (void)hipFree(arena);
        if (splitk_ws) (void)hipFree(splitk_ws);
        if (deltas) (void)hipFree(deltas);
        if (probs) (void)hipFree(probs);
        if (nms_ws) (void)hipFree(nms_ws);
        for (auto& v : timing_events)
            for (auto e : v) (void)hipEventDestroy(e);
        drop_graphs();
        if (gstream) (void)hipStreamDestroy(gstream);
        for (int k = 0; k < kSides; ++k) {
// ... 18 lines not shown
```

### tf-ssd_amd/csrc/ssd_net.hip

```cpp
#include <algorithm>
#include <cstdlib>
#include <cstring>
#include <map>
#include <memory>
#include <string>
#include <vector>

#include "ssd_net.h"

using namespace ssd;

namespace ssd {

struct Builder {
    ssd_net& net;
    explicit Builder(ssd_net& n) : net(n) {}

    int add_param(const std::string& name, std::vector<int> shape) {
        Param p;
        p.name = name;
        p.shape = std::move(shape);
        p.count = 1;
        for (int d : p.shape) p.count *= (size_t)d;
        net.params.push_back(p);
// ... 211 lines not shown
        x = b.conv(e + "_1", e + "_1", x, extras[i - 1][0], 1, 1, 0, 1, "", true, SSD_ACT_RELU);
        x = b.conv(e + "_2", e + "_2", x, extras[i - 1][1], 3, 2, 1, 1, "", true, SSD_ACT_RELU);
        feats.push_back(x);
    }
    b.heads(feats);
}

static void build_vgg16(ssd_net& net) {
    Builder b(net);
    const int S = net.img_size;
    int x = b.add_tensor("input", S, S, 3);
    auto c3 = [&](const char* name, int cout) { x = b.conv(name, name, x, cout, 3, 1, 1, 1, "", true, SSD_ACT_RELU); };
    c3("conv1_1", 64); c3("conv1_2", 64); x = b.pool("pool1", x, 2, 2);
    c3("conv2_1", 128); c3("conv2_2", 128); x = b.pool("pool2", x, 2, 2);
    c3("conv3_1", 256); c3("conv3_2", 256); c3("conv3_3", 256); x = b.pool("pool3", x, 2, 2);
    c3("conv4_1", 512); c3("conv4_2", 512); c3("conv4_3", 512);
    const int conv4_3 = x;
    x = b.pool("pool4", x, 2, 2);
    c3("conv5_1", 512); c3("conv5_2", 512); c3("conv5_3", 512); x = b.pool("pool5", x, 3, 1);
    x = b.conv("conv6", "conv6", x, 1024, 3, 1, 1, 6, "", true, SSD_ACT_RELU);
    x = b.conv("conv7", "conv7", x, 1024, 1, 1, 1, 1, "", true, SSD_ACT_RELU);
    const int conv7 = x;
    x = b.conv("conv8_1", "conv8_1", x, 256, 1, 1, 0, 1, "", true, SSD_ACT_RELU);
    x = b.conv("conv8_2", "conv8_2", x, 512, 3, 2, 1, 1, "", true, SSD_ACT_RELU);
    const int conv8_2 = x;
    x = b.conv("conv9_1", "conv9_1", x, 128, 1, 1, 0, 1, "", true, SSD_ACT_RELU);
    x = b.conv("conv9_2", "conv9_2", x, 256, 3, 2, 1, 1, "", true, SSD_ACT_RELU);
    const int conv9_2 = x;
    x = b.conv("conv10_1", "conv10_1", x, 128, 1, 1, 0, 1, "", true, SSD_ACT_RELU);
    x = b.conv("conv10_2", "conv10_2", x, 256, 3, 1, 0, 1, "", true, SSD_ACT_RELU);
    const int conv10_2 = x;
    x = b.conv("conv11_1", "conv11_1", x, 128, 1, 1, 0, 1, "", true, SSD_ACT_RELU);
    x = b.conv("conv11_2", "conv11_2", x, 256, 3, 1, 0, 1, "", true, SSD_ACT_RELU);
    const int conv11_2 = x;
    Layer l;
    l.name = "l2_normalization";
    l.kind = LK_L2NORM;
    l.in = conv4_3;
    const Tensor t = net.tensors[conv4_3];
    l.H = l.Ho = t.H; l.W = l.Wo = t.W; l.Cin = l.Cout = t.C;
    l.p_gamma = b.add_param("l2_normalization/scale", {t.C});
    l.out = b.add_tensor("l2_normalization", t.H, t.W, t.C);
    net.layers.push_back(l);
    b.heads({l.out, conv7, conv8_2, conv9_2, conv10_2, conv11_2});
}

static ConvParams layer_conv_params(const ssd_net& net, const Layer& l, int B, const float* in, float* out,
                                    const float* res, float* deltas_out, float* probs_out) {
    ConvParams p{};
    p.in = in;
    p.w = l.packed;
    p.w3 = conv_split_planes(l.packed, l.kh * l.kw * l.Cin, l.Cout);
    p.bf16 = net.precision;
    if (l.in >= 0 && net.tensors[l.in].planes) {
        const Tensor& ti = net.tensors[l.in];
        p.xp = ti.planes; p.xp_plane = ti.plane_stride; p.xp_np = ti.planes_np;
    }
    if (l.out >= 0 && l.head_kind == 0 && net.tensors[l.out].planes_live && (l.Cout & 3) == 0) {
        const Tensor& to = net.tensors[l.out];
        p.op = to.planes; p.op_plane = to.plane_stride; p.op_np = to.planes_np;
    }
    p.wino_w = l.wino;
    p.scale = l.scale;
    p.shift = l.shift;
    p.residual = res;
    p.B = B; p.H = l.H; p.W = l.W; p.Cin = l.Cin; p.Ho = l.Ho; p.Wo = l.Wo; p.Cout = l.Cout;
    p.kh = l.kh; p.kw = l.kw; p.stride = l.stride; p.dil = l.dil; p.pad_t = l.pt; p.pad_l = l.pl;
    p.K = l.kh * l.kw * l.Cin;
    p.Kpad = conv_kpad(p.K);
    p.Npad = conv_npad(l.Cout);
    p.M = (long)B * l.Ho * l.Wo;
    p.act = l.act;
    p.split_k = l.split_k;
    p.partial = l.splitk_part ? l.splitk_part : net.splitk_ws;
    if (l.head_kind == 0) {
        p.out = l.out >= 0 && net.tensors[l.out].plane_only && p.op ? nullptr : out;
        p.out_pixel_stride = l.Cout;
        p.out_batch_stride = (long)l.Ho * l.Wo * l.Cout;
    } else {
        conv_route_head(p, l, probs_out, deltas_out);
    }
    p.vec_store = conv_vec_store(p);
    return p;
}

static FusedBlockParams fused_shape(const ssd_net& net, const Layer& f, int B) {
    const Layer& le = net.layers[f.f_expand];
    const Layer& ld = net.layers[f.f_dw];
    const Layer& lp = net.layers[f.f_project];
    FusedBlockParams p{};
    p.x = net.tensors[f.in].dev;
    p.y = net.tensors[f.out].dev;
    p.we = f.fz_we; p.es = le.scale; p.eh = le.shift;
    p.wd = f.fz_wd; p.ds = ld.scale; p.dh = ld.shift;
    p.wp = f.fz_wp; p.ps = lp.scale; p.ph = lp.shift;
    p.residual = lp.res >= 0 ? 1 : 0;
    p.B = B; p.H = f.H; p.W = f.W; p.Cin = f.Cin; p.Ce = le.Cout; p.Cout = f.Cout;
    p.Ho = f.Ho; p.Wo = f.Wo; p.stride = f.stride; p.pad_t = f.pt; p.pad_l = f.pl;
    p.kpad_e = conv_kpad(le.Cin);
    p.kpad_p = conv_kpad(lp.Cin);
    p.npad_p = conv_npad(lp.Cout);
    p.e_out = f.e_out >= 0 ? net.tensors[f.e_out].dev : nullptr;
    if (f.out >= 0 && net.tensors[f.out].planes_live) {
        const Tensor& to = net.tensors[f.out];
        p.y_planes = to.planes; p.y_plane = to.plane_stride; p.planes_np = to.planes_np;
    }
    if (f.e_out >= 0 && net.tensors[f.e_out].planes_live) {
        const Tensor& te = net.tensors[f.e_out];
        p.e_planes = te.planes; p.e_plane = te.plane_stride; p.planes_np = te.planes_np;
    }
    if (f.route == RT_IMAGE || f.route == RT_IMAGE_SPLIT)
        p.planes_only = (p.y_planes && net.tensors[f.out].plane_only ? 1 : 0) | (p.e_planes && net.tensors[f.e_out].plane_only ? 2 : 0);
    p.we3 = reinterpret_cast<const short*>(f.fz_we3);
    p.wp3 = reinterpret_cast<const short*>(f.fz_wp3);
    p.bf16 = net.precision;
    p.form2 = net.image_v2 ? 1 : 0;
    return p;
}

static FusedBlockParams fused_params(const ssd_net& net, const Layer& f, int B) {
    FusedBlockParams p = fused_shape(net, f, B);
    if (f.route == RT_IMAGE || f.route == RT_IMAGE_SPLIT) {
        const Layer& le = net.layers[f.f_expand];
        const Layer& lp = net.layers[f.f_project];
        p.we3 = conv_split_planes(f.fz_we, le.Cin, le.Cout);
        p.wp3 = conv_split_planes(f.fz_wp, lp.Cin, lp.Cout);
        p.groups = net.img_slabs ? image_block_groups(p, B * net.lanes_hint) : 1;
        p.slabs = net.img_slabs;
        p.tickets = net.image_ticket && !p.bf16 ? net.img_tickets : nullptr;
        if (f.route == RT_IMAGE_SPLIT) { p.bf16 = 3; p.tickets = nullptr; }
    }
    return p;
}

static DwProjParams dwproj_params(const ssd_net& net, const Layer& f, int B) {
    const Layer& ld = net.layers[f.f_dw];
    const Layer& lp = net.layers[f.f_project];
    DwProjParams p{};
    p.e = net.tensors[f.in].dev;
    p.y = net.tensors[f.out].dev;
    p.wd = f.fz_wd; p.dh = ld.shift;
    p.wp = f.fz_wp; p.ph = lp.shift;
    p.res = lp.res >= 0 ? net.tensors[lp.res].dev : nullptr;
    p.B = B; p.H = f.H; p.W = f.W; p.Ce = ld.Cout; p.Cout = f.Cout;
    p.Ho = f.Ho; p.Wo = f.Wo; p.stride = f.stride; p.pad_t = f.pt; p.pad_l = f.pl;
    p.kpad_p = conv_kpad(lp.Cin);
    p.npad_p = conv_npad(lp.Cout);
    p.bf16 = net.precision;
    return p;
}

static StemParams stem_params(const ssd_net& net, const Layer& f, int B) {
    const Layer& l1 = net.layers[f.f_expand];
    const Layer& ld = net.layers[f.f_dw];
    const Layer& lp = net.layers[f.f_project];
    StemParams p{};
    p.x = net.tensors[f.in].dev;
    p.y = net.tensors[f.out].dev;
    p.w1 = l1.packed; p.s1 = l1.scale; p.h1 = l1.shift;
    p.wd = net.params[ld.p_kernel].dev; p.sd = ld.scale; p.hd = ld.shift;
    p.wp = lp.packed; p.sp = lp.scale; p.hp = lp.shift;
    p.B = B; p.H = f.H; p.W = f.W; p.H1 = f.Ho; p.W1 = f.Wo; p.pad_t = f.pt; p.pad_l = f.pl;
// ... 80 lines not shown
    return f.kind == LK_FUSED && f.f_type == 0 && image_kernel_takes(fused_shape(net, f, 1));
}

static Route fused_route(const ssd_net& net, const Layer& f) {
    if (!net.fuse_blocks) return RT_OFF;
    if (f.f_type == 1) return stem_supported(stem_params(net, f, 1)) ? RT_STEM : RT_OFF;
    if (f.f_type == 2) {
        if (!net.fuse_dwproj) return RT_OFF;
        if (f.fused_by >= 0 && net.layers[f.fused_by].route != RT_OFF) return RT_OFF;
        return dwproj_supported(dwproj_params(net, f, 1)) ? RT_DWPROJ : RT_OFF;
    }
    const FusedBlockParams p = fused_shape(net, f, 1);
    if (fused_block_supported(p)) {
        if (net.fuse_band == 2 && f.fz_we3 && band3_block_supported(p)) return RT_BAND3;
        return net.fuse_band && band_block_supported(p) ? RT_BAND : RT_TILE;
    }
    if (!net.fuse_image || (net.fuse_image == 1 && f.img_choice < 1)) return RT_OFF;
    if (!image_block_supported(p)) return RT_OFF;
    return f.img_choice == 2 && net.precision == 0 ? RT_IMAGE_SPLIT : RT_IMAGE;
}

static void resolve_routes(ssd_net& net) {
    for (Layer& l : net.layers) {
        const bool owned = (l.fused_by >= 0 && net.layers[l.fused_by].route != RT_OFF) ||
                           (l.fused_by2 >= 0 && net.layers[l.fused_by2].route != RT_OFF);
        l.route = l.kind == LK_FUSED ? fused_route(net, l) : owned ? RT_OFF : RT_LAYER;
    }
}
static bool layer_runs(const Layer& l) { return l.route != RT_OFF; }

template <typename F>
static std::vector<char> plane_only_candidates(const ssd_net& net, F reads_planes) {
    const int nt = (int)net.tensors.size();
    std::vector<char> ok(nt, 0), readers(nt, 0);
    if (!net.plane_only || net.image_ticket) return ok;
    for (int t = 1; t < nt; ++t) ok[t] = net.tensors[t].planes != nullptr;
    auto bar = [&](int t) { if (t >= 0) ok[t] = 0; };
    for (int i = 0; i < (int)net.layers.size(); ++i) {
        const Layer& l = net.layers[i];
        if (!layer_runs(l)) continue;
        if (l.kind == LK_CONV && l.in >= 0 && reads_planes(i)) readers[l.in] = 1;
        else bar(l.in);
        bar(l.res);
        if (l.kind == LK_FUSED && l.f_project >= 0) bar(net.layers[l.f_project].res);
        const bool image = l.kind == LK_FUSED && (l.route == RT_IMAGE || l.route == RT_IMAGE_SPLIT);
        bool writes = image || l.kind == LK_POOL || l.kind == LK_L2NORM;
        if (l.kind == LK_CONV)
            writes = l.head_kind == 0 && (l.Cout & 3) == 0 && l.cfg >= 0 && l.cfg != conv_num_configs() - 1 &&
                     conv_config_writes_planes(l.cfg, ConvParams{});
        if (!writes) { bar(l.out); bar(l.e_out); }
    }
    for (int t = 0; t < nt; ++t) ok[t] = ok[t] && readers[t];
    return ok;
}

static int dev_alloc(ssd_net& net, size_t floats, float** out) {
    *out = nullptr;
    if (floats == 0) return SSD_OK;
    SSD_HIP(hipMalloc((void**)out, floats * sizeof(float)));
    net.owned.push_back(*out);
    return SSD_OK;
}

static int tune_image_blocks(ssd_net& net, int B, hipStream_t st) {
    ScopedEvent se0, se1;
    SSD_HIP(hipEventCreate(&se0.e));
    SSD_HIP(hipEventCreate(&se1.e));
    struct ModeGuard {
        ssd_net& n;
        int mode;
        ~ModeGuard() { n.fuse_image = mode; }
    } guard{net, net.fuse_image};
    net.fuse_image = 1;
    int rc = SSD_OK;
    for (size_t fi = 0; fi < net.layers.size() && !rc; ++fi) {
        Layer& f = net.layers[fi];
        if (f.kind != LK_FUSED || f.f_type != 0) continue;
        if (!image_kernel_takes(net, f)) { f.img_choice = 0; continue; }
        if (f.img_choice >= 0) continue;
        float ms[3] = {1e30f, 1e30f, 1e30f};
        const int nchoice = net.precision == 0 && net.image_split ? 3 : 2;
        for (int choice = 0; choice < nchoice && !rc; ++choice) {
            f.img_choice = choice;
            resolve_routes(net);
            if (choice == 2 && !image_block_split_fits(fused_params(net, f, B))) continue;
            for (int trial = 0; trial < 4 && !rc; ++trial) {
                (void)hipEventRecord(se0.e, st);
                for (int r = 0; r < 4 && !rc; ++r)
                    for (int j = (int)fi; j <= f.f_project && !rc; ++j)
                        if (layer_runs(net.layers[j])) rc = run_layer(net, net.layers[j], B, nullptr, nullptr, st);
                (void)hipEventRecord(se1.e, st);
                if (rc) break;
                SSD_HIP(hipEventSynchronize(se1.e));
                float t = 0.f;
                (void)hipEventElapsedTime(&t, se0.e, se1.e);
                if (trial && t < ms[choice]) ms[choice] = t;
            }
        }
        f.img_choice = ms[2] < ms[1] && ms[2] < ms[0] ? 2 : ms[1] < ms[0] ? 1 : 0;
    }
    return rc;
}

static int autotune(ssd_net& net, int B, hipStream_t st) {
    ScopedEvent se0, se1;
    SSD_HIP(hipEventCreate(&se0.e));
    SSD_HIP(hipEventCreate(&se1.e));
    hipEvent_t e0 = se0.e, e1 = se1.e;
    ScopedDev sd, spr;
    SSD_HIP(hipMalloc((void**)&sd.p, (size_t)B * net.num_priors * 4 * sizeof(float)));
    SSD_HIP(hipMalloc((void**)&spr.p, (size_t)B * net.num_priors * net.L * sizeof(float)));
    float *d = sd.p, *pr = spr.p;
    static const int kSplits[] = {1, 2, 3, 4, 5, 6, 7, 8, 10, 12, 14, 16, 20, 24, 32};
    constexpr int kNumSplits = sizeof(kSplits) / sizeof(kSplits[0]);
    size_t ws_floats = 0;
    for (auto& l : net.layers) {
        if (l.kind != LK_CONV) continue;
        const size_t mc = (size_t)B * l.Ho * l.Wo * l.Cout;
        if (mc <= (size_t)4 << 20) ws_floats = std::max(ws_floats, mc * 32);
    }
    if (ws_floats > net.splitk_floats) {
        if (net.splitk_ws) (void)hipFree(net.splitk_ws);
        net.splitk_ws = nullptr;
        SSD_HIP(hipMalloc((void**)&net.splitk_ws, ws_floats * sizeof(float)));
        net.splitk_floats = ws_floats;
    }
    int rc = SSD_OK;
    const bool dbg_sync = getenv("SSD_HIP_DEBUG_SYNC") != nullptr;
    const bool dbg_tune = getenv("SSD_HIP_DEBUG_TUNE") != nullptr;
    struct Best { float ms[2] = {1e30f, 1e30f}; int cfg[2] = {-1, -1}; int split[2] = {1, 1}; bool timed = false; };
    std::vector<Best> bests(net.layers.size());
    constexpr int kReps = 4;
    for (size_t li = 0; li < net.layers.size(); ++li) {
        Layer& l = net.layers[li];
        Best& bb = bests[li];
        if (l.kind != LK_CONV) continue;
        if (l.cfg >= 0) continue;
        bb.timed = true;
        const float* in = net.tensors[l.in].dev;
        float* out = l.out >= 0 ? net.tensors[l.out].dev : nullptr;
        const float* res = l.res >= 0 ? net.tensors[l.res].dev : nullptr;
        for (int c = 0; c < conv_num_configs() && !rc; ++c) {
            const int fam = conv_config_is_dma(c) ? 1 : 0;
            for (int si = 0; si < kNumSplits && !rc; ++si) {
                const int split = kSplits[si];
                l.split_k = split;
                ConvParams p = layer_conv_params(net, l, B, in, out, res, d, pr);
                if (!conv_config_valid(c, p) || !conv_config_allowed(c, net.precision)) break;
                const bool direct = (c == conv_num_configs() - 1);
                if (direct && (bb.cfg[0] >= 0 || bb.cfg[1] >= 0 || split > 1)) break;
                if (split > 1) {
                    const long blocks = conv_grid_blocks(c, p);
                    const int nkt = conv_k_tiles(c, p);
                    if (blocks > 384 || nkt < 4 * split) break;
                    if ((size_t)split * p.M * p.Cout > net.splitk_floats) break;
                }
                const int reps = kReps;
                if (dbg_sync) fprintf(stderr, "[ssd dbg] tune %s %s split %d\n", l.name.c_str(), conv_config_name(c), split);
                rc = conv_launch(p, c, st);
                if (rc) break;
                if (dbg_sync) SSD_HIP(hipStreamSynchronize(st));
                float ms = 1e30f;
                for (int trial = 0; trial < 3 && !rc; ++trial) {
                    (void)hipEventRecord(e0, st);
                    for (int r = 0; r < reps && !rc; ++r) rc = conv_launch(p, c, st);
                    (void)hipEventRecord(e1, st);
                    if (rc) break;
                    SSD_HIP(hipEventSynchronize(e1));
                    float t = 0.f;
                    (void)hipEventElapsedTime(&t, e0, e1);
                    ms = t < ms ? t : ms;
                    if (trial == 0 && ms > 1.5f * bb.ms[fam]) break;
                }
                if (rc) break;
                if (ms < bb.ms[fam]) { bb.ms[fam] = ms; bb.cfg[fam] = c; bb.split[fam] = split; }
            }
        }
        if (rc) break;
        if (bb.cfg[0] < 0 && bb.cfg[1] < 0) {
            set_error("finalize: no conv kernel can run layer %s", l.name.c_str());
            rc = SSD_E_UNSUPPORTED;
            break;
        }
        const int f0 = bb.cfg[0] >= 0 ? 0 : 1;
        l.cfg = bb.cfg[f0];
        l.split_k = bb.split[f0];
        if (dbg_tune)
            fprintf(stderr, "[ssd] tune %s: %s/s%d %.4f ms | %s/s%d %.4f ms\n", l.name.c_str(), bb.cfg[0] >= 0 ? conv_config_name(bb.cfg[0]) : "-",
                    bb.split[0], bb.cfg[0] >= 0 ? bb.ms[0] / kReps : 0.f, bb.cfg[1] >= 0 ? conv_config_name(bb.cfg[1]) : "-", bb.split[1],
                    bb.cfg[1] >= 0 ? bb.ms[1] / kReps : 0.f);
    }
    if (rc) return rc;
    std::vector<int> img_saved;
    for (auto& f : net.layers) {
        img_saved.push_back(f.img_choice);
        if (f.img_choice < 0 && image_kernel_takes(net, f)) f.img_choice = 1;
    }
    resolve_routes(net);
    for (size_t t = 1; t < net.tensors.size(); ++t) {
        const Tensor& tt = net.tensors[t];
        std::vector<size_t> flip;
        bool planes_anyway = false;
        double sum0 = 0, sum1 = 0;
        for (size_t li = 0; li < net.layers.size(); ++li) {
            const Layer& l = net.layers[li];
            if (l.kind != LK_CONV || l.in != (int)t) continue;
            const Best& bb = bests[li];
            if (!bb.timed) { if (layer_runs(l) && conv_config_is_dma(l.cfg)) planes_anyway = true; continue; }
            if (bb.cfg[1] < 0) continue;
            if (bb.cfg[0] < 0) { planes_anyway = true; continue; }
            if (!layer_runs(l)) {
                if (bb.ms[1] + kReps * ((double)B * tt.per_image * 2.0 * tt.planes_np / 3.0e12 * 1e3) < bb.ms[0]) {
                    net.layers[li].cfg = bb.cfg[1];
                    net.layers[li].split_k = bb.split[1];
                }
                continue;
            }
            flip.push_back(li);
            sum0 += bb.ms[0];
            sum1 += bb.ms[1];
        }
        if (flip.empty()) continue;
        for (size_t li : flip) { net.layers[li].cfg = bests[li].cfg[1]; net.layers[li].split_k = bests[li].split[1]; }
        const bool only = plane_only_candidates(net, [&](int i) { return conv_config_is_dma(net.layers[i].cfg); })[t];
        const double bytes = only ? 2.0 * tt.planes_np - 4.0 : planes_anyway ? 0.0 : 2.0 * tt.planes_np;
        const double store_ms = kReps * ((double)B * tt.per_image * bytes / 3.0e12 * 1e3);
        const bool take = sum1 + store_ms < sum0;
        if (!take)
            for (size_t li : flip) { net.layers[li].cfg = bests[li].cfg[0]; net.layers[li].split_k = bests[li].split[0]; }
        if (dbg_tune)
            fprintf(stderr, "[ssd] tune tensor %s: fp32 readers %.4f ms, plane readers %.4f + store %+.4f ms (%s) -> %s\n", tt.name.c_str(),
                    sum0 / kReps, sum1 / kReps, store_ms / kReps, only ? "plane-only" : "both copies", take ? "planes" : "fp32");
    }
    for (size_t i = 0; i < net.layers.size(); ++i) net.layers[i].img_choice = img_saved[i];
    resolve_routes(net);
    return rc;
}

}

template <typename F>
static int run_graphed(ssd_net* net, std::vector<const void*> key, hipStream_t& st, F body) {
    if (!net->use_graph || net->timing) return body();
    if (net->graphs_unsafe && net->overlap_heads) return body();
    const hipStream_t caller = st;
    if (st == nullptr) {
        if (!net->gstream && hipStreamCreateWithFlags(&net->gstream, hipStreamDefault) != hipSuccess) {
            (void)hipGetLastError();
            return body();
        }
        st = net->gstream;
    }
    key.push_back((const void*)st);
    for (auto& g : net->graphs)
        if (g.key == key) {
            SSD_HIP(hipGraphLaunch(g.exec, st));
            net->tensors[0].dev = const_cast<float*>(g.image);
            net->last_batch = g.batch;
            return SSD_OK;
        }
    if (net->graphs.size() >= 16) net->drop_graphs();
    st = caller;
    int rc = body();
    if (rc) return rc;
    st = caller ? caller : net->gstream;
    ssd_net::GraphEntry e;
    e.key = std::move(key);
    if (hipStreamBeginCapture(st, hipStreamCaptureModeThreadLocal) != hipSuccess) {
        (void)hipGetLastError();
        return SSD_OK;
    }
    rc = body();
    const hipError_t ce = hipStreamEndCapture(st, &e.graph);
    if (rc || ce != hipSuccess || !e.graph) {
        (void)hipGetLastError();
        if (e.graph) (void)hipGraphDestroy(e.graph);
        net->use_graph = false;
        return rc ? rc : SSD_OK;
    }
    if (hipGraphInstantiate(&e.exec, e.graph, nullptr, nullptr, 0) != hipSuccess) {
        (void)hipGetLastError();
        (void)hipGraphDestroy(e.graph);
        net->use_graph = false;
        return SSD_OK;
    }
// ... 98 lines not shown
    SSD_HIP(hipMalloc((void**)&del.p, (size_t)B * net->num_priors * 4 * sizeof(float)));
    SSD_HIP(hipMalloc((void**)&prb.p, (size_t)B * net->num_priors * net->L * sizeof(float)));
    SSD_HIP(hipMemset(img.p, 0, n_img * sizeof(float)));
    hipStream_t st = nullptr;
    SSD_HIP(hipStreamCreateWithFlags(&st, hipStreamNonBlocking));
    ScopedEvent e0, e1;
    int rc = SSD_OK;
    float ms[2] = {1e30f, 1e30f};
    if (hipEventCreate(&e0.e) != hipSuccess || hipEventCreate(&e1.e) != hipSuccess) rc = SSD_E_HIP;
    for (int mode = 0; mode < 2 && !rc; ++mode) {
        net->use_graph = mode != 0;
        for (int w = 0; w < 3 && !rc; ++w) rc = ssd_net_forward(net, img.p, B, del.p, prb.p, st);
    }
    for (int trial = 0; trial < 4 && !rc; ++trial)
        for (int mode = 0; mode < 2 && !rc; ++mode) {
            net->use_graph = mode != 0;
            (void)hipEventRecord(e0.e, st);
            for (int r = 0; r < 6 && !rc; ++r) rc = ssd_net_forward(net, img.p, B, del.p, prb.p, st);
            (void)hipEventRecord(e1.e, st);
            if (rc || hipEventSynchronize(e1.e) != hipSuccess) { rc = rc ? rc : SSD_E_HIP; break; }
            float t = 0.f;
            (void)hipEventElapsedTime(&t, e0.e, e1.e);
            if (t < ms[mode]) ms[mode] = t;
        }
    (void)hipStreamSynchronize(st);
    net->drop_graphs();
    (void)hipStreamDestroy(st);
    net->tensors[0].dev = nullptr;
    net->use_graph = rc ? true : ms[1] < ms[0] * 0.99f;
    net->launch_raced = !rc;
    if (getenv("SSD_HIP_DEBUG_TUNE"))
        fprintf(stderr, "[ssd] launch mode race at B=%d: direct %.4f ms, graph replay %.4f ms per forward -> %s\n", B, ms[0] / 6,
                ms[1] / 6, net->use_graph ? "replay" : "direct");
    return rc;
}


static int finalize_pack_conv(ssd_net* net, Layer& l, hipStream_t st) {
    const int K = l.kh * l.kw * l.Cin;
    int rc = dev_alloc(*net, conv_packed_floats(K, l.Cout), &l.packed);
    if (rc) return rc;
    if (l.p_kernel2 < 0) {
        rc = launch_pack_weights(net->params[l.p_kernel].dev, K, l.Cout, conv_kpad(K), conv_npad(l.Cout),
                                 l.packed, st);
    } else {
        SSD_HIP(hipMemsetAsync(l.packed, 0, (size_t)conv_kpad(K) * conv_npad(l.Cout) * sizeof(float), st));
        rc = launch_pack_weights(net->params[l.p_kernel].dev, K, l.Cout1, conv_kpad(K), l.Cout1, l.packed, st);
        if (!rc)
            rc = launch_pack_weights(net->params[l.p_kernel2].dev, K, l.Cout - l.Cout1, conv_kpad(K),
                                     l.Cout - l.Cout1, l.packed + (size_t)l.Cout1 * conv_kpad(K), st);
    }
    if (!rc) rc = launch_pack_split(l.packed, K, l.Cout, st);
    if (rc) return rc;
    if (l.kh == 3 && l.kw == 3 && l.stride == 1 && l.dil == 1 && l.Cin % 16 == 0 && l.res < 0 && net->use_wino) {
        const int np = conv_npad(l.Cout);
        rc = dev_alloc(*net, wino_weight_floats(l.Cin, l.Cout), &l.wino);
        if (rc) return rc;
        SSD_HIP(hipMemsetAsync(l.wino, 0, wino_weight_floats(l.Cin, l.Cout) * sizeof(float), st));
        if (l.p_kernel2 < 0) {
            rc = launch_wino_pack(net->params[l.p_kernel].dev, l.Cin, l.Cout, np, 0, l.wino, st);
        } else {
            rc = launch_wino_pack(net->params[l.p_kernel].dev, l.Cin, l.Cout1, np, 0, l.wino, st);
            if (!rc) rc = launch_wino_pack(net->params[l.p_kernel2].dev, l.Cin, l.Cout - l.Cout1, np, l.Cout1, l.wino, st);
        }
    }
    return rc;
}

static int finalize_fold_bn(ssd_net* net, Layer& l, hipStream_t st) {
    if (l.p_bn >= 0) {
        int rc = dev_alloc(*net, l.Cout, &l.scale);
        if (!rc) rc = dev_alloc(*net, l.Cout, &l.shift);
        if (rc) return rc;
        return launch_fold_bn(net->params[l.p_bn].dev, net->params[l.p_bn + 1].dev, net->params[l.p_bn + 2].dev,
                              net->params[l.p_bn + 3].dev, 1e-3f, l.Cout, l.scale, l.shift, st);
    }
    if (l.p_bias2 >= 0) {
        const int rc = dev_alloc(*net, l.Cout, &l.shift);
        if (rc) return rc;
        SSD_HIP(hipMemcpyAsync(l.shift, net->params[l.p_bias].dev, (size_t)l.Cout1 * sizeof(float),
                               hipMemcpyDeviceToDevice, st));
        SSD_HIP(hipMemcpyAsync(l.shift + l.Cout1, net->params[l.p_bias2].dev,
                               (size_t)(l.Cout - l.Cout1) * sizeof(float), hipMemcpyDeviceToDevice, st));
    } else if (l.p_bias >= 0) {
        l.shift = net->params[l.p_bias].dev;
    }
    return SSD_OK;
}

static int finalize_fused_weights(ssd_net* net, hipStream_t st) {
    for (auto& f : net->layers) {
        if (f.kind == LK_FUSED && f.f_type == 2) {
            const Layer& ld = net->layers[f.f_dw];
            const Layer& lp = net->layers[f.f_project];
            const size_t nd = (size_t)9 * ld.Cout, np = (size_t)conv_kpad(lp.Cin) * conv_npad(lp.Cout);
            int rc = dev_alloc(*net, nd, &f.fz_wd);
            if (!rc) rc = dev_alloc(*net, np, &f.fz_wp);
            if (rc) return rc;
            rc = launch_scale_cols(net->params[ld.p_kernel].dev, ld.scale, 9, ld.Cout, f.fz_wd, st);
            if (!rc) rc = launch_scale_rows(lp.packed, lp.scale, conv_npad(lp.Cout), lp.Cout, conv_kpad(lp.Cin), f.fz_wp, st);
            if (rc) return rc;
            continue;
        }
        if (f.kind != LK_FUSED || f.f_type != 0) continue;
        const Layer& le = net->layers[f.f_expand];
        const Layer& ld = net->layers[f.f_dw];
// ... 7 lines not shown
        if (!rc) rc = launch_scale_cols(net->params[ld.p_kernel].dev, ld.scale, 9, ld.Cout, f.fz_wd, st);
        if (!rc) rc = launch_scale_rows(lp.packed, lp.scale, conv_npad(lp.Cout), lp.Cout, conv_kpad(lp.Cin), f.fz_wp, st);
        if (!rc) rc = launch_pack_split(f.fz_we, le.Cin, le.Cout, st, true);
        if (!rc) rc = launch_pack_split(f.fz_wp, lp.Cin, lp.Cout, st, true);
        if (rc) return rc;
        f.fz_we3 = f.fz_wp3 = nullptr;
        if (band3_block_supported(fused_shape(*net, f, 1))) {
            rc = dev_alloc(*net, (band3_we_shorts(le.Cout) + 1) / 2, &f.fz_we3);
            if (!rc) rc = dev_alloc(*net, (band3_wp_shorts(conv_npad(lp.Cout), le.Cout) + 1) / 2, &f.fz_wp3);
            if (!rc) rc = launch_band3_pack(f.fz_we, le.Cout, le.Cin, conv_kpad(le.Cin), reinterpret_cast<short*>(f.fz_we3), f.fz_wp,
                                            conv_npad(lp.Cout), conv_kpad(lp.Cin), reinterpret_cast<short*>(f.fz_wp3), st);
            if (rc) return rc;
        }
    }
    return SSD_OK;
}

static int finalize_image_slabs(ssd_net* net, int max_batch, hipStream_t st) {
    size_t slab = 0;
    for (auto& f : net->layers) {
        if (!image_kernel_takes(*net, f)) continue;
        const FusedBlockParams p = fused_shape(*net, f, 1);
        for (int b = 1; b <= max_batch; ++b) slab = std::max(slab, image_block_slab_floats(p, b));
    }
    net->img_slabs = nullptr;
    net->img_tickets = nullptr;
    net->slab_bytes = slab * sizeof(float);
    if (slab) {
        float* tk = nullptr;
        int rc = dev_alloc(*net, slab, &net->img_slabs);
        if (!rc) rc = dev_alloc(*net, (size_t)max_batch, &tk);
        if (rc) return rc;
        net->img_tickets = reinterpret_cast<unsigned*>(tk);
        SSD_HIP(hipMemsetAsync(tk, 0, (size_t)max_batch * sizeof(unsigned), st));
    }
    return SSD_OK;
}

static int finalize_arena(ssd_net* net, int max_batch, hipStream_t st) {
    if (net->arena) (void)hipFree(net->arena);
    net->arena = nullptr;
    const bool poison = getenv("SSD_HIP_DEBUG_POISON") != nullptr;
    const size_t gap = poison ? 1024 : 0;
    size_t total = gap;
    for (auto& t : net->tensors) total += align_up(t.per_image * max_batch, 64) + gap;
    SSD_HIP(hipMalloc((void**)&net->arena, total * sizeof(float)));
    net->arena_bytes = total * sizeof(float);
    size_t off = gap;
    for (auto& t : net->tensors) {
        t.dev = net->arena + off;
        off += align_up(t.per_image * max_batch, 64) + gap;
    }
    SSD_HIP(hipMemset(net->arena, poison ? 0xFF : 0, total * sizeof(float)));
    for (auto& t : net->tensors) { t.planes = nullptr; t.planes_live = false; t.plane_only = false; t.planes_np = 0; t.plane_stride = 0; }
    if (net->conv_dma)
        for (const auto& l : net->layers) {
            if (l.kind != LK_CONV || l.in < 0 || l.Cin % 32 != 0) continue;
            Tensor& t = net->tensors[l.in];
            if (t.planes) continue;
            t.planes_np = net->precision ? 1 : 3;
            t.plane_stride = (long)align_up(t.per_image * max_batch, 64);
            float* pl = nullptr;
            const int rcp = dev_alloc(*net, (size_t)t.planes_np * t.plane_stride / 2 + 64, &pl);
            if (rcp) return rcp;
            t.planes = reinterpret_cast<short*>(pl);
            SSD_HIP(hipMemsetAsync(pl, 0, ((size_t)t.planes_np * t.plane_stride / 2 + 64) * sizeof(float), st));
        }
    net->max_batch = max_batch;
    return SSD_OK;
}

static int finalize_apply_preset(ssd_net* net, int max_batch, bool* image_preset_ok) {
    for (auto& l : net->layers) { l.cfg = -1; l.split_k = 1; }
    size_t ws_need = 0;
    int n_tuned = 0, n_preset = 0;
    for (auto& l : net->layers) {
        if (l.kind != LK_CONV) continue;
        auto it = net->preset.find(l.name);
        if (it == net->preset.end()) { ++n_tuned; continue; }
        int cfg = -1;
        for (int c = 0; c < conv_num_configs(); ++c)
            if (it->second.first == conv_config_name(c)) cfg = c;
        if (cfg < 0 || !conv_config_allowed(cfg, net->precision)) { ++n_tuned; continue; }
        l.cfg = cfg;
        l.split_k = it->second.second;
        ConvParams p = layer_conv_params(*net, l, max_batch, net->tensors[l.in].dev,
                                         l.out >= 0 ? net->tensors[l.out].dev : nullptr, nullptr,
                                         net->arena, net->arena);
        const bool split_ok = l.split_k == 1 || conv_k_tiles(cfg, p) >= l.split_k;
        if (l.split_k < 1 || !split_ok || !conv_config_valid(cfg, p)) { l.cfg = -1; l.split_k = 1; ++n_tuned; continue; }
        ++n_preset;
        if (l.split_k > 1) ws_need = std::max(ws_need, (size_t)l.split_k * p.M * p.Cout);
    }
    *image_preset_ok = true;
    for (auto& f : net->layers) {
        if (f.kind != LK_FUSED || f.f_type != 0) continue;
        f.img_choice = -1;
        if (!image_kernel_takes(*net, f)) continue;
        auto it = net->preset.find(f.name);
        if (it == net->preset.end() || it->second.first != "image") { *image_preset_ok = false; continue; }
        f.img_choice = it->second.second < 0 ? 0 : it->second.second > 2 ? 2 : it->second.second;
        if (f.img_choice == 2 && (net->precision != 0 || !net->image_split)) f.img_choice = 1;
    }
    if (ws_need > net->splitk_floats) {
        if (net->splitk_ws) (void)hipFree(net->splitk_ws);
        net->splitk_ws = nullptr;
        SSD_HIP(hipMalloc((void**)&net->splitk_ws, ws_need * sizeof(float)));
        net->splitk_floats = ws_need;
    }
    net->n_autotuned = n_tuned;
    net->n_preset = n_preset;
    return SSD_OK;
}

static int finalize_free_unread_planes(ssd_net* net, hipStream_t st) {
    std::vector<char> read(net->tensors.size(), 0);
    for (const auto& l : net->layers)
        if (l.kind == LK_CONV && l.in >= 0 && conv_config_is_dma(l.cfg)) read[l.in] = 1;
    SSD_HIP(hipStreamSynchronize(st));
    net->plane_bytes = 0;
    for (size_t i = 0; i < net->tensors.size(); ++i) {
        Tensor& t = net->tensors[i];
        if (!t.planes) continue;
        const size_t bytes = ((size_t)t.planes_np * t.plane_stride / 2 + 64) * sizeof(float);
        if (read[i]) { net->plane_bytes += bytes; continue; }
        float* pl = reinterpret_cast<float*>(t.planes);
        net->owned.erase(std::remove(net->owned.begin(), net->owned.end(), pl), net->owned.end());
        (void)hipFree(pl);
        t.planes = nullptr; t.planes_np = 0; t.plane_stride = 0;
    }
    return SSD_OK;
}

static int finalize_streams(ssd_net* net, int max_batch) {
    size_t total_ws = 0;
    for (auto& l : net->layers)
        if (l.kind == LK_CONV && l.split_k > 1) total_ws += align_up((size_t)l.split_k * max_batch * l.Ho * l.Wo * l.Cout, 64);
    if (total_ws) {
        SSD_HIP(hipMalloc((void**)&net->splitk_layers, total_ws * sizeof(float)));
        size_t o = 0;
        for (auto& l : net->layers)
            if (l.kind == LK_CONV && l.split_k > 1) {
                l.splitk_part = net->splitk_layers + o;
                o += align_up((size_t)l.split_k * max_batch * l.Ho * l.Wo * l.Cout, 64);
            }
    }
    for (int k = 0; k < ssd_net::kSides; ++k) {
        if (!net->side[k]) SSD_HIP(hipStreamCreateWithFlags(&net->side[k], hipStreamNonBlocking));
        if (!net->ev_side_done[k]) SSD_HIP(hipEventCreateWithFlags(&net->ev_side_done[k], hipEventDisableTiming));
    }
    for (auto& l : net->layers)
        if (!l.ev_ready) SSD_HIP(hipEventCreateWithFlags(&l.ev_ready, hipEventDisableTiming));
    return SSD_OK;
}

int ssd_net_finalize(ssd_net* net, int max_batch) {
    SSD_CHECK_ARG(net && max_batch >= 1, "ssd_net_finalize: bad arguments");
    for (const auto& p : net->params)
        if (!p.set) {
            set_error("ssd_net_finalize: parameter '%s' was never set", p.name.c_str());
            return SSD_E_STATE;
        }
    hipStream_t st = nullptr;
    for (float* p : net->owned)
        if (p) (void)hipFree(p);
    net->owned.clear();
    if (net->splitk_layers) (void)hipFree(net->splitk_layers);
    net->splitk_layers = nullptr;
    int rc = SSD_OK;
    for (auto& l : net->layers) {
        l.packed = l.scale = l.shift = nullptr;
        l.wino = nullptr;
        l.splitk_part = nullptr;
        if (l.kind == LK_CONV) rc = finalize_pack_conv(net, l, st);
        if (!rc && (l.kind == LK_CONV || l.kind == LK_DW)) rc = finalize_fold_bn(net, l, st);
        if (rc) return rc;
    }
    rc = finalize_fused_weights(net, st);
    if (!rc) rc = finalize_image_slabs(net, max_batch, st);
    if (!rc) rc = finalize_arena(net, max_batch, st);
    bool image_preset_ok = true;
    if (!rc) rc = finalize_apply_preset(net, max_batch, &image_preset_ok);
    if (!rc && net->n_autotuned) rc = autotune(*net, max_batch, st);
    if (!rc) rc = finalize_free_unread_planes(net, st);
    if (!rc) rc = finalize_streams(net, max_batch);
    if (rc) return rc;
    if (!image_preset_ok) {
        rc = tune_image_blocks(*net, max_batch, st);
        if (rc) return rc;
        ++net->n_autotuned;
    }
    SSD_HIP(hipDeviceSynchronize());
    net->drop_graphs();
    resolve_routes(*net);
    net->finalized = true;
    return tune_launch_mode(net, max_batch);
}

long ssd_net_get_tuning(const ssd_net* net, char* buf, size_t cap) {
    if (!net) return SSD_E_INVALID;
    std::string out;
    for (const auto& l : net->layers)
        if (l.kind == LK_CONV && l.cfg >= 0)
            out += l.name + " " + conv_config_name(l.cfg) + " " + std::to_string(l.split_k) + "\n";
    for (const auto& l : net->layers)
        if (l.img_choice >= 0 && image_kernel_takes(*net, l)) out += l.name + " image " + std::to_string(l.img_choice) + "\n";
    if (net->finalized && net->use_graph_auto && net->launch_raced)
        out += std::string("__launch graph ") + (net->use_graph ? "1" : "0") + "\n";
    if (buf && cap > out.size()) memcpy(buf, out.c_str(), out.size() + 1);
    return (long)out.size();
}

int ssd_net_memory_bytes(const ssd_net* net, size_t out[4]) {
    SSD_CHECK_ARG(net != nullptr && out != nullptr, "ssd_net_memory_bytes: NULL argument");
    SSD_CHECK_ARG(net->finalized, "ssd_net_memory_bytes: net is not finalized");
    out[0] = net->arena_bytes;
    out[1] = net->plane_bytes;
    out[2] = net->slab_bytes;
    size_t sk = net->splitk_floats;
    for (const auto& l : net->layers)
        if (l.kind == LK_CONV && l.split_k > 1) sk += align_up((size_t)l.split_k * net->max_batch * l.Ho * l.Wo * l.Cout, 64);
    out[3] = sk * sizeof(float);
    return SSD_OK;
}

int ssd_net_tuning_stats(const ssd_net* net, int* from_table, int* timed) {
    SSD_CHECK_ARG(net != nullptr, "ssd_net_tuning_stats: net is NULL");
    if (from_table) *from_table = net->n_preset;
    if (timed) *timed = net->n_autotuned;
    return SSD_OK;
}

int ssd_net_set_tuning(ssd_net* net, const char* text) {
    SSD_CHECK_ARG(net && text, "ssd_net_set_tuning: NULL argument");
    net->preset.clear();
    std::string s(text);
// ... 239 lines not shown
                                      valid_dev, nullptr, net->nms_ws, net->nms_ws_bytes, (void*)st);
        if (fused_sm)
            return decode_nms_fused(net->deltas, net->probs, priors_dev, v4, B, N, L, max_total, max_total, iou_thr, score_thr,
                                    boxes_dev, labels_dev, scores_dev, valid_dev, net->nms_ws, net->nms_ws_bytes, net->nms_ws_batch, st);
        return ssd_decode_nms(net->deltas, net->probs, priors_dev, v4, B, N, L, max_total, max_total, iou_thr,
                              score_thr, boxes_dev, labels_dev, scores_dev, valid_dev, nullptr, net->nms_ws,
                              net->nms_ws_bytes, (void*)st);
    });
    if (rc && fused_sm && net->nms_ws) {
        (void)hipDeviceSynchronize();
        (void)hipMemset(net->nms_ws, 0, net->nms_ws_bytes);
    }
    if (!rc && net->timing && !net->timing_events.empty())
        (void)hipEventRecord(net->timing_events.back().back(), st);
    return rc;
}

int ssd_net_predict(ssd_net* net, const float* image_dev, int B, const float* priors_dev, const float* var,
                    int max_total, float iou_thr, float score_thr, float* boxes_dev, float* labels_dev,
                    float* scores_dev, int* valid_dev, void* stream) {
    return predict_impl(net, image_dev, B, priors_dev, var, max_total, iou_thr, score_thr, nullptr, boxes_dev, labels_dev,
                        scores_dev, valid_dev, stream);
}

int ssd_net_predict_cfg(ssd_net* net, const float* image_dev, int B, const float* priors_dev, const float* var,
                        const ssd_nms_config* cfg, float* boxes_dev, float* labels_dev, float* scores_dev,
                        int* valid_dev, void* stream) {
    SSD_CHECK_ARG(cfg != nullptr, "ssd_net_predict_cfg: config is NULL");
    return predict_impl(net, image_dev, B, priors_dev, var, cfg->max_total, cfg->iou_threshold, cfg->score_threshold, cfg,
                        boxes_dev, labels_dev, scores_dev, valid_dev, stream);
}

struct OptionSpec {
    const char* name;
    bool ssd_net::*flag;
    int ssd_net::*num;
    int lo, hi, refinalize;
};
static const OptionSpec kOptions[] = {
    {"fuse_blocks", &ssd_net::fuse_blocks, nullptr, 0, 1, 0},
    {"precision", nullptr, &ssd_net::precision, 0, 1, 1},
    {"fuse_band", nullptr, &ssd_net::fuse_band, 0, 2, 0},
    {"fuse_image", nullptr, &ssd_net::fuse_image, 0, 2, 0},
    {"lanes_hint", nullptr, &ssd_net::lanes_hint, 1, 8, 0},
    {"tail_on_side", &ssd_net::tail_on_side, nullptr, 0, 1, 0},
    {"image_split", &ssd_net::image_split, nullptr, 0, 1, 1},
    {"image_ticket", &ssd_net::image_ticket, nullptr, 0, 1, 0},
    {"fuse_softmax", &ssd_net::fuse_softmax, nullptr, 0, 1, 0},
    {"fuse_dwproj", &ssd_net::fuse_dwproj, nullptr, 0, 1, 0},
    {"overlap_heads", &ssd_net::overlap_heads, nullptr, 0, 1, 0},
    {"use_wino", &ssd_net::use_wino, nullptr, 0, 1, 2},
    {"image_v2", &ssd_net::image_v2, nullptr, 0, 1, 0},
    {"conv_dma", &ssd_net::conv_dma, nullptr, 0, 1, 1},
    {"plane_only", &ssd_net::plane_only, nullptr, 0, 1, 0},
    {"use_graph", &ssd_net::use_graph, nullptr, 0, 1, 0},
};

int ssd_net_set_option(ssd_net* net, const char* name, int value) {
    SSD_CHECK_ARG(net && name, "ssd_net_set_option: NULL argument");
    const std::string n(name);
    const OptionSpec* o = nullptr;
    for (const OptionSpec& k : kOptions)
        if (n == k.name) o = &k;
    if (!o) {
        set_error("ssd_net_set_option: unknown option '%s'", name);
        return SSD_E_INVALID;
    }
    if (n == "precision") SSD_CHECK_ARG(value == 0 || value == 1, "ssd_net_set_option: precision must be 0 (fp32) or 1 (bf16)");
    if (n == "use_graph") {
        if (value && net->graphs_unsafe && net->overlap_heads) {
            set_error("ssd_net_set_option: use_graph 1 needs overlap_heads 0 with GPU_MAX_HW_QUEUES < 4 (hipGraph capture of the forked step crashes in the runtime; a single in-order stream replays fine)");
            return SSD_E_UNSUPPORTED;
        }
        net->use_graph_auto = false;
    }
    const int v = o->flag ? value != 0 : std::min(std::max(value, o->lo), o->hi);
    const int old = o->flag ? (int)(net->*o->flag) : net->*o->num;
    if (o->flag) net->*o->flag = v != 0;
    else net->*o->num = v;
    if (o->refinalize == 2 || (o->refinalize == 1 && v != old)) net->finalized = false;
    net->drop_graphs();
    resolve_routes(*net);
    if (n == "fuse_softmax" && net->nms_ws) {
        (void)hipDeviceSynchronize();
        SSD_HIP(hipMemset(net->nms_ws, 0, net->nms_ws_bytes));
    }
    return SSD_OK;
}

int ssd_net_set_timing(ssd_net* net, int enabled) {
    SSD_CHECK_ARG(net != nullptr, "ssd_net_set_timing: net is NULL");
    net->timing = enabled != 0;
    net->steps.clear();
    return SSD_OK;
}

int ssd_net_read_timing(ssd_net* net, float* ms_sum_out, int* forwards_out) {
    SSD_CHECK_ARG(net && ms_sum_out && forwards_out, "ssd_net_read_timing: NULL argument");
    const size_t nl = net->layers.size();
    for (size_t i = 0; i <= nl; ++i) ms_sum_out[i] = 0.f;
    SSD_HIP(hipDeviceSynchronize());
    for (auto& ev : net->timing_events) {
        for (size_t i = 0; i < nl; ++i) {
            float ms = 0.f;
            if (hipEventElapsedTime(&ms, ev[i], ev[i + 1]) == hipSuccess) ms_sum_out[i] += ms;
        }
// ... 158 lines not shown
```

### tf-ssd_amd/models/_net.py

```python
import ctypes
import os
import re

import numpy as np
import torch

import ssd_hip as _h

_TABLE_OPTIONS = ("use_wino", "image_split", "conv_dma")
_REFINALIZE_OPTIONS = ("precision", "image_split", "use_wino", "conv_dma")
_STALE_WARNED = set()


class _LayerProxy(object):

    def __init__(self, model, name):
        self._model = model
        self.name = name

    @property
    def trainable(self):
        return self._model._is_trainable(self.name)

    @trainable.setter
    def trainable(self, value):
        self._model._set_trainable(self.name, bool(value))


class SSDModel(object):

    def __init__(self, backbone, hyper_params, max_batch=None, precision="fp32"):
        if precision not in ("fp32", "bf16"):
            raise ValueError("precision must be 'fp32' or 'bf16', got %r" % (precision,))
        self.precision = precision
        self.backbone = backbone
        self.hyper_params = hyper_params
        self.img_size = int(hyper_params["img_size"])
        self.total_labels = int(hyper_params["total_labels"])
        n_ars = [len(a) for a in hyper_params["aspect_ratios"]]
        arr = (ctypes.c_int * len(n_ars))(*n_ars)
        lib = _h.lib()
        self._net = lib.ssd_net_create(_h.MOBILENET_V2 if backbone == "mobilenet_v2" else _h.VGG16,
                                       self.img_size, len(n_ars), arr, self.total_labels)
        if not self._net:
            raise ValueError("ssd_net_create: %s" % lib.ssd_last_error().decode())
        self.param_specs = []
        for i in range(lib.ssd_net_num_params(self._net)):
            name = lib.ssd_net_param_name(self._net, i).decode()
            rank = lib.ssd_net_param_rank(self._net, i)
            shp = lib.ssd_net_param_shape(self._net, i)
            self.param_specs.append((name, tuple(shp[j] for j in range(rank))))
        self.num_priors = lib.ssd_net_num_priors(self._net)
        fm = [lib.ssd_net_feature_map_size(self._net, l) for l in range(len(n_ars))]
        if list(fm) != [int(f) for f in hyper_params["feature_map_shapes"]]:
            raise ValueError("feature_map_shapes %s do not match the %s graph at img_size %d (%s)" % (
                hyper_params["feature_map_shapes"], backbone, self.img_size, fm))
        self._max_batch = max_batch
        self._finalized_for = 0
        self._weights_set = False
        self._weights_version = 0
        self._options = {}
        if precision == "bf16":
            self.set_option("precision", 1)
# ... 620 lines not shown
```

### tf-ssd_amd/ssd_hip.py

```python
import ctypes
import os
import sys


def configure_serving(lanes=3):
    if "GPU_MAX_HW_QUEUES" in os.environ:
        return os.environ["GPU_MAX_HW_QUEUES"] == str(lanes)
    t = sys.modules.get("torch")
    try:
        if t is not None and t.cuda.is_initialized():
            return False
    except Exception:
        return False
    os.environ["GPU_MAX_HW_QUEUES"] = str(int(lanes))
    return True


if os.environ.get("SSD_HIP_HW_QUEUES", "").isdigit() and int(os.environ["SSD_HIP_HW_QUEUES"]) > 0:
    configure_serving(int(os.environ["SSD_HIP_HW_QUEUES"]))

import numpy as np
import torch

_HERE = os.path.dirname(os.path.abspath(__file__))
# ... 122 lines not shown
    "ssd_png_encode_workspace_bytes": (ctypes.c_size_t, [vp, ctypes.c_int]),
    "ssd_png_encode": (ctypes.c_int, [vp, ctypes.c_size_t, vp, vp, ctypes.c_int, vp, ctypes.c_size_t, vp, vp, ctypes.c_size_t, vp]),
    "ssd_png_encode_host": (ctypes.c_int, [vp, ctypes.c_int, ctypes.c_int, ctypes.c_int, vp, ctypes.c_size_t,
                                            ctypes.POINTER(ctypes.c_size_t)]),
    "ssd_png_parse": (ctypes.c_int, [vp, ctypes.c_size_t, ctypes.POINTER(PngInfo)]),
    "ssd_png_idat": (ctypes.c_int, [vp, ctypes.c_size_t, ctypes.POINTER(PngInfo), vp, ctypes.c_size_t]),
    "ssd_png_decode_host": (ctypes.c_int, [ctypes.POINTER(PngInfo), vp, ctypes.c_size_t, vp, ctypes.c_size_t]),
    "ssd_png_decode_workspace_bytes": (ctypes.c_size_t, [vp, ctypes.c_int]),
    "ssd_png_decode": (ctypes.c_int, [vp, ctypes.c_size_t, vp, vp, ctypes.c_int, vp, ctypes.c_size_t, vp, ctypes.c_size_t, vp]),
    "ssd_png_inflate": (ctypes.c_int, [vp, ctypes.c_size_t, vp, vp, ctypes.c_int, vp, vp]),
    "ssd_png_inflate_host": (ctypes.c_int, [vp, ctypes.c_size_t, vp, ctypes.c_size_t, ctypes.c_longlong, c_int_p]),
    "ssd_jpeg_scan_plan": (ctypes.c_int, [vp, ctypes.c_size_t, ctypes.POINTER(JpegInfo), ctypes.POINTER(JpegScanPlan), vp, ctypes.c_size_t]),
    "ssd_jpeg_entropy_decode_subseq": (ctypes.c_int, [vp, ctypes.c_size_t, ctypes.POINTER(JpegInfo), vp, ctypes.c_size_t, ctypes.c_int]),
    "ssd_jpeg_unpack_slots": (ctypes.c_int, [ctypes.c_longlong, ctypes.c_int, ctypes.c_int]),
    "ssd_jpeg_unpack_workspace_bytes": (ctypes.c_size_t, [vp, ctypes.c_int, ctypes.c_int]),
    "ssd_jpeg_unpack": (ctypes.c_int, [vp, ctypes.c_size_t, vp, vp, ctypes.c_int, ctypes.c_int, vp, ctypes.c_size_t, vp, vp,
                                        ctypes.c_size_t, vp]),
    "ssd_image_mean": (ctypes.c_int, [vp] + [ctypes.c_int] * 4 + [vp, vp, vp]),
    "ssd_augment_geometry": (ctypes.c_int, [vp] + [ctypes.c_int] * 6 + [vp, vp, vp, vp]),
    "ssd_augment_color": (ctypes.c_int, [vp] + [ctypes.c_int] * 3 + [vp, vp, vp, vp]),
    "ssd_augment_plan": (ctypes.c_int, [vp, vp, vp] + [ctypes.c_int] * 4 + [ctypes.c_ulonglong] + [vp] * 7),
    "ssd_image_minmax_workspace_bytes": (ctypes.c_size_t, [ctypes.c_int]),
    "ssd_image_minmax": (ctypes.c_int, [vp] + [ctypes.c_int] * 4 + [vp, vp, ctypes.c_size_t, vp]),
    "ssd_draw_detections": (ctypes.c_int, [vp, vp] + [ctypes.c_int] * 4 + [vp, vp, vp, vp, ctypes.c_int, ctypes.c_int, vp,
                                           ctypes.c_int, vp, ctypes.c_int, ctypes.c_int, vp, vp]),
    "ssd_draw_bounding_boxes": (ctypes.c_int, [vp] + [ctypes.c_int] * 4 + [vp, ctypes.c_int, vp, ctypes.c_int, vp, vp]),
    "ssd_loss_workspace_bytes": (ctypes.c_size_t, [ctypes.c_int, ctypes.c_int]),
    "ssd_loss": (ctypes.c_int, [vp, vp, vp, vp, ctypes.c_int, ctypes.c_int, ctypes.c_int, ctypes.c_float,
                                ctypes.c_float, vp, vp, vp, vp, vp, vp, ctypes.c_float, vp, ctypes.c_size_t, vp]),
    "ssd_focal_loss_tile": (ctypes.c_int, [ctypes.c_int, c_int_p]),
    "ssd_focal_loss_workspace_bytes": (ctypes.c_size_t, [ctypes.c_int, ctypes.c_int, ctypes.c_int]),
    "ssd_focal_loss": (ctypes.c_int, [vp, vp, vp, vp, ctypes.c_int, ctypes.c_int, ctypes.c_int, ctypes.c_float,
                                      ctypes.c_float, ctypes.c_float, vp, vp, vp, vp, vp, vp, ctypes.c_float, vp,
                                      ctypes.c_size_t, vp]),
    "ssd_iou_loc_loss_tile": (ctypes.c_int, []),
    "ssd_iou_loc_loss_workspace_bytes": (ctypes.c_size_t, [ctypes.c_int, ctypes.c_int]),
    "ssd_iou_loc_loss": (ctypes.c_int, [vp, ctypes.POINTER(ctypes.c_float), vp, vp, ctypes.c_int, ctypes.c_int, ctypes.c_int,
                                        ctypes.c_float, vp, vp, vp, ctypes.c_float, vp, ctypes.c_size_t, vp]),
    "ssd_loss_config_bytes": (ctypes.c_size_t, []),
    "ssd_same_pads": (ctypes.c_int, [ctypes.c_int] * 4 + [c_int_p, c_int_p]),
    "ssd_conv_out_size": (ctypes.c_int, [ctypes.c_int] * 6),
    "ssd_conv_packed_weight_floats": (ctypes.c_size_t, [ctypes.c_int] * 4),
    "ssd_conv_pack_weights": (ctypes.c_int, [vp] + [ctypes.c_int] * 4 + [vp, vp]),
    "ssd_conv2d": (ctypes.c_int, [ctypes.POINTER(ConvDesc), vp, vp, vp, vp, vp, vp,
                                  ctypes.c_long, ctypes.c_long, vp]),
    "ssd_conv_num_configs": (ctypes.c_int, []),
    "ssd_conv_config_name": (ctypes.c_char_p, [ctypes.c_int]),
    "ssd_conv2d_ex": (ctypes.c_int, [ctypes.POINTER(ConvDesc), vp, vp, vp, vp, vp, vp,
                                     ctypes.c_long, ctypes.c_long, ctypes.c_int, ctypes.c_int, vp, vp]),
    "ssd_split_planes": (ctypes.c_int, [vp, ctypes.c_long, ctypes.c_int, ctypes.c_int, vp, ctypes.c_long, vp]),
    "ssd_join_planes": (ctypes.c_int, [vp, ctypes.c_long, ctypes.c_int, ctypes.c_int, ctypes.c_long, vp, vp]),
    "ssd_conv2d_planes": (ctypes.c_int, [ctypes.POINTER(ConvDesc), vp, ctypes.c_int, ctypes.c_long, vp, vp, vp, vp, vp,
                                         ctypes.c_long, ctypes.c_long, vp, ctypes.c_long, ctypes.c_int, ctypes.c_int, vp, vp]),
    "ssd_conv_wino_weight_floats": (ctypes.c_size_t, [ctypes.c_int, ctypes.c_int]),
    "ssd_conv_wino_pack_weights": (ctypes.c_int, [vp, ctypes.c_int, ctypes.c_int, vp, vp]),
    "ssd_conv_wino_num_configs": (ctypes.c_int, []),
    "ssd_conv2d_wino": (ctypes.c_int, [ctypes.POINTER(ConvDesc), vp, vp, vp, vp, vp, ctypes.c_long, ctypes.c_long,
                                       ctypes.c_int, ctypes.c_int, vp, vp]),
    "ssd_dwconv3x3": (ctypes.c_int, [vp] + [ctypes.c_int] * 9 + [vp, vp, vp, ctypes.c_int, vp, vp]),
    "ssd_maxpool2d": (ctypes.c_int, [vp] + [ctypes.c_int] * 10 + [vp, vp]),
    "ssd_l2norm": (ctypes.c_int, [vp, ctypes.c_long, ctypes.c_int, vp, vp, vp]),
    "ssd_softmax": (ctypes.c_int, [vp, ctypes.c_long, ctypes.c_int, vp, vp]),
    "ssd_net_create": (vp, [ctypes.c_int, ctypes.c_int, ctypes.c_int, c_int_p, ctypes.c_int]),
    "ssd_net_destroy": (None, [vp]),
    "ssd_net_num_params": (ctypes.c_int, [vp]),
    "ssd_net_param_name": (ctypes.c_char_p, [vp, ctypes.c_int]),
    "ssd_net_param_rank": (ctypes.c_int, [vp, ctypes.c_int]),
    "ssd_net_param_shape": (c_int_p, [vp, ctypes.c_int]),
    "ssd_net_set_param": (ctypes.c_int, [vp, ctypes.c_char_p, c_float_p, ctypes.c_size_t]),
    "ssd_net_get_param": (ctypes.c_int, [vp, ctypes.c_char_p, c_float_p, ctypes.c_size_t]),
    "ssd_net_finalize": (ctypes.c_int, [vp, ctypes.c_int]),
    "ssd_net_get_tuning": (ctypes.c_long, [vp, ctypes.c_char_p, ctypes.c_size_t]),
    "ssd_net_set_tuning": (ctypes.c_int, [vp, ctypes.c_char_p]),
    "ssd_net_tuning_stats": (ctypes.c_int, [vp, ctypes.POINTER(ctypes.c_int), ctypes.POINTER(ctypes.c_int)]),
    "ssd_net_memory_bytes": (ctypes.c_int, [vp, ctypes.POINTER(ctypes.c_size_t)]),
    "ssd_build_id": (ctypes.c_char_p, []),
    "ssd_stream_create": (vp, [ctypes.c_int]),
    "ssd_stream_create_masked": (vp, [ctypes.POINTER(ctypes.c_uint), ctypes.c_int]),
    "ssd_stream_destroy": (ctypes.c_int, [vp]),
    "ssd_net_regularization_loss": (ctypes.c_int, [vp, c_float_p]),
    "ssd_net_train_set_buckets": (ctypes.c_int, [vp, ctypes.c_int, ctypes.POINTER(ctypes.c_long)]),
    "ssd_net_train_wait_bucket": (ctypes.c_int, [vp, ctypes.c_int, vp]),
    "ssd_net_num_priors": (ctypes.c_int, [vp]),
    "ssd_net_feature_map_size": (ctypes.c_int, [vp, ctypes.c_int]),
    "ssd_net_forward": (ctypes.c_int, [vp, vp, ctypes.c_int, vp, vp, vp]),
    "ssd_net_predict": (ctypes.c_int, [vp, vp, ctypes.c_int, vp, c_float_p, ctypes.c_int,
                                       ctypes.c_float, ctypes.c_float, vp, vp, vp, vp, vp]),
    "ssd_net_predict_cfg": (ctypes.c_int, [vp, vp, ctypes.c_int, vp, c_float_p, ctypes.POINTER(NmsConfig), vp, vp, vp, vp, vp]),
    "ssd_net_fetch_activation": (ctypes.c_long, [vp, ctypes.c_char_p, c_float_p, ctypes.c_size_t]),
    "ssd_net_fetch_planes": (ctypes.c_long, [vp, ctypes.c_char_p, c_float_p, ctypes.c_size_t, c_int_p]),
    "ssd_net_num_layers": (ctypes.c_int, [vp]),
    "ssd_net_layer_name": (ctypes.c_char_p, [vp, ctypes.c_int]),
    "ssd_net_layer_kind": (ctypes.c_char_p, [vp, ctypes.c_int]),
    "ssd_net_layer_config": (ctypes.c_char_p, [vp, ctypes.c_int]),
    "ssd_net_layer_flops": (ctypes.c_double, [vp, ctypes.c_int, ctypes.c_int]),
    "ssd_net_layer_bytes": (ctypes.c_double, [vp, ctypes.c_int, ctypes.c_int]),
    "ssd_net_layer_executed_flops": (ctypes.c_double, [vp, ctypes.c_int, ctypes.c_int]),
    "ssd_net_set_option": (ctypes.c_int, [vp, ctypes.c_char_p, ctypes.c_int]),
    "ssd_net_set_timing": (ctypes.c_int, [vp, ctypes.c_int]),
    "ssd_net_read_timing": (ctypes.c_int, [vp, c_float_p, c_int_p]),
    "ssd_net_profile_layers": (ctypes.c_int, [vp, vp, ctypes.c_int, ctypes.c_int, c_float_p, vp]),
    "ssd_net_train_begin": (ctypes.c_int, [vp, ctypes.c_int]),
    "ssd_net_trainable_floats": (ctypes.c_size_t, [vp]),
    "ssd_net_trainable_offset": (ctypes.c_long, [vp, ctypes.c_char_p]),
    "ssd_net_train_forward_backward": (ctypes.c_int, [vp, vp, ctypes.c_int, vp, vp, ctypes.c_float, ctypes.c_float,
                                                      vp, vp, vp, vp]),
# ... 206 lines not shown
```

Before: 58830.

## Add two-plane fp16 split MFMA conv path for fp32 nets

Adds a new family of DMA conv configs that store activations as two scaled fp16 planes (hi/lo) and weights as exponent-scaled fp16 hi/lo planes. Each product then takes three f16 MFMAs instead of the six bf16 MFMAs of the three-plane bf16 split. Plane traffic also drops from three planes to two. The path is enabled by default through the conv_f16x2 option, applies only to layers whose input is ReLU6-bounded, and falls back to the bf16x3 twin otherwise. The risk is accuracy, because fp16 range and split error depend on the activation scaling.

New measurement: 63340, median of 6. 1.08x the previous value.

```diff
diff --git a/include/ssd_hip.h b/include/ssd_hip.h
--- a/include/ssd_hip.h
+++ b/include/ssd_hip.h
@@ -396,6 +396,15 @@
                       const float* residual_dev, float* out_dev, long out_batch_stride, long out_pixel_stride,
                       void* out_planes_dev, long out_plane_stride, int config, int split_k,
                       float* splitk_ws_dev, void* stream);
+
+size_t ssd_conv_f16x2_weight_bytes(int kh, int kw, int Cin, int Cout);
+int ssd_conv_pack_weights_f16x2(const float* packed_w_dev, int kh, int kw, int Cin, int Cout, void* w_planes_dev,
+                                int* k_out, void* stream);
+int ssd_conv2d_planes_f16x2(const ssd_conv_desc* d, const void* in_planes_dev, long in_plane_stride,
+                            const float* packed_w_dev, const void* w_planes_dev, int w_exp, const float* scale_dev,
+                            const float* shift_dev, const float* residual_dev, float* out_dev,
+                            long out_batch_stride, long out_pixel_stride, void* out_planes_dev,
+                            long out_plane_stride, int config, int split_k, float* splitk_ws_dev, void* stream);
 
 size_t ssd_conv_wino_weight_floats(int Cin, int Cout);
 int ssd_conv_wino_pack_weights(const float* hwio_dev, int Cin, int Cout, float* wino_w_dev, void* stream);
diff --git a/tf-ssd_amd/csrc/ssd_bf16x3.h b/tf-ssd_amd/csrc/ssd_bf16x3.h
--- a/tf-ssd_amd/csrc/ssd_bf16x3.h
+++ b/tf-ssd_amd/csrc/ssd_bf16x3.h
@@ -64,6 +64,26 @@
 __device__ __forceinline__ short rne1(float a) { return (short)(rne2(a, 0.f) & 0xffffu); }
 __device__ __forceinline__ uint2 rne4(const b3_f32x4 v) { return make_uint2(rne2(v[0], v[1]), rne2(v[2], v[3])); }
 
+typedef _Float16 f16x2_t __attribute__((ext_vector_type(2)));
+typedef _Float16 f16x8 __attribute__((ext_vector_type(8)));
+constexpr float kF16x2ActScale = 256.f;
+
+__device__ __forceinline__ void split_h2(const float a, const float b, unsigned& h, unsigned& l) {
+    const f16x2_t hh = __builtin_convertvector(b3_f32x2{a, b}, f16x2_t);
+    const b3_f32x2 back = __builtin_convertvector(hh, b3_f32x2);
+    const f16x2_t ll = __builtin_convertvector(b3_f32x2{a - back[0], b - back[1]}, f16x2_t);
+    h = __builtin_bit_cast(unsigned, hh);
+    l = __builtin_bit_cast(unsigned, ll);
+}
+__device__ __forceinline__ void split4_h(const b3_f32x4 v, uint2& h, uint2& l) {
+    split_h2(v[0] * kF16x2ActScale, v[1] * kF16x2ActScale, h.x, l.x);
+    split_h2(v[2] * kF16x2ActScale, v[3] * kF16x2ActScale, h.y, l.y);
+}
+__device__ __forceinline__ float join_h(const short h, const short l) {
+    const float fh = (float)__builtin_bit_cast(_Float16, h), fl = (float)__builtin_bit_cast(_Float16, l);
+    return (fh + fl) * (1.f / kF16x2ActScale);
+}
+
 template <int NP>
 struct BP {
     bf16x8 p[NP];
@@ -82,6 +102,13 @@
 }
 template <int NP>
 __device__ __forceinline__ b3_f32x4 mmaN(const BP<NP>& w, const BP<NP>& x, b3_f32x4 acc) {
+    if constexpr (NP == 2) {
+        const f16x8 wh = __builtin_bit_cast(f16x8, w.p[0]), wl = __builtin_bit_cast(f16x8, w.p[1]);
+        const f16x8 xh = __builtin_bit_cast(f16x8, x.p[0]), xl = __builtin_bit_cast(f16x8, x.p[1]);
+        acc = __builtin_amdgcn_mfma_f32_16x16x32_f16(wl, xh, acc, 0, 0, 0);
+        acc = __builtin_amdgcn_mfma_f32_16x16x32_f16(wh, xl, acc, 0, 0, 0);
+        return __builtin_amdgcn_mfma_f32_16x16x32_f16(wh, xh, acc, 0, 0, 0);
+    }
     if constexpr (NP == 3) {
         acc = __builtin_amdgcn_mfma_f32_16x16x32_bf16(w.p[1], x.p[1], acc, 0, 0, 0);
         acc = __builtin_amdgcn_mfma_f32_16x16x32_bf16(w.p[0], x.p[2], acc, 0, 0, 0);
@@ -104,6 +131,11 @@
     const long e = plane_elem(pix, c, P);
     if (np == 1) {
         *reinterpret_cast<uint2*>(op + e) = rne4(v);
+    } else if (np == 2) {
+        uint2 h, l;
+        split4_h(v, h, l);
+        *reinterpret_cast<uint2*>(op + e) = h;
+        *reinterpret_cast<uint2*>(op + plane + e) = l;
     } else {
         uint2 h, m, l;
         split4(v, h, m, l);
diff --git a/tf-ssd_amd/csrc/ssd_conv.h b/tf-ssd_amd/csrc/ssd_conv.h
--- a/tf-ssd_amd/csrc/ssd_conv.h
+++ b/tf-ssd_amd/csrc/ssd_conv.h
@@ -1,4 +1,7 @@
 #pragma once
+#include <cmath>
+#include <cstring>
+
 #include "common.h"
 
 namespace ssd {
@@ -32,6 +35,8 @@
     short* op;
     long op_plane;
     int op_np;
+    const short* wh;
+    float acc_scale;
 };
 bool conv_config_allowed(int cfg, int precision);
 inline int conv_vec_store(const ConvParams& p) {
@@ -64,6 +69,7 @@
     short* e_planes;
     long e_plane;
     int planes_np;
+    int e_planes_np;
     int planes_only;
     int form2;
 };
@@ -164,6 +170,25 @@
 int dma_k_tiles(int np, const ConvParams& p);
 void dma_tile(int i, int* BM, int* BN);
 int dma_launch(const ConvParams& p, int i, int np, hipStream_t st);
+int dmah_num_configs();
+const char* dmah_config_name(int j);
+int dmah_tile_index(int j);
+bool dmah_config_valid(int j, const ConvParams& p);
+int dmah_k_tiles(int j, const ConvParams& p);
+int dmah_launch(const ConvParams& p, int j, hipStream_t st);
+int launch_absmax_bits(const float* packed, int K, int Cout, unsigned* absmax_bits_dev, hipStream_t st);
+int launch_pack_f16x2(const float* packed, int K, int Cout, int k, short* planes, hipStream_t st);
+inline int conv_f16x2_weight_exp(unsigned absmax_bits) {
+    float wmax;
+    std::memcpy(&wmax, &absmax_bits, sizeof(float));
+    if (!(wmax > 0.f)) return 0;
+    int e = 0;
+    (void)std::frexp(wmax, &e);
+    return 14 - e;
+}
+inline size_t conv_f16x2_plane_shorts(int K, int Cout) { return (size_t)2 * conv_kpad(K) * conv_npad(Cout); }
+bool conv_config_is_dmah(int cfg);
+int conv_dmah_twin(int cfg);
 int launch_split_planes(const float* x, long n, int C, int np, short* planes, long plane, hipStream_t st);
 int launch_join_planes(const short* planes, long n, int C, int np, long plane, float* x, hipStream_t st);
 bool conv_config_is_dma(int cfg);
diff --git a/tf-ssd_amd/csrc/ssd_conv.hip b/tf-ssd_amd/csrc/ssd_conv.hip
--- a/tf-ssd_amd/csrc/ssd_conv.hip
+++ b/tf-ssd_amd/csrc/ssd_conv.hip
@@ -244,14 +244,18 @@
 static int bf16_cfg0() { return kNumMfmaCfgs + wino_num_configs() + skinny_num_configs() + mfma3_num_configs(); }
 static int dma3_cfg0() { return kNumMfmaCfgs + wino_num_configs() + skinny_num_configs() + 2 * mfma3_num_configs(); }
 static int dmab_cfg0() { return dma3_cfg0() + dma_num_configs(); }
-static int direct_cfg() { return dma3_cfg0() + 2 * dma_num_configs(); }
+static int dmah_cfg0() { return dma3_cfg0() + 2 * dma_num_configs(); }
+static int direct_cfg() { return dmah_cfg0() + dmah_num_configs(); }
 #define kSkinnyCfg0 skinny_cfg0()
 #define kMfma3Cfg0 mfma3_cfg0()
 #define kBf16Cfg0 bf16_cfg0()
 #define kDma3Cfg0 dma3_cfg0()
 #define kDmabCfg0 dmab_cfg0()
+#define kDmahCfg0 dmah_cfg0()
 #define kDirectCfg direct_cfg()
 bool conv_config_is_dma(int cfg) { return cfg >= kDma3Cfg0 && cfg < kDirectCfg; }
+bool conv_config_is_dmah(int cfg) { return cfg >= kDmahCfg0 && cfg < kDirectCfg; }
+int conv_dmah_twin(int cfg) { return conv_config_is_dmah(cfg) ? kDma3Cfg0 + dmah_tile_index(cfg - kDmahCfg0) : cfg; }
 bool conv_config_writes_planes(int cfg, const ConvParams& p) {
     if (cfg == kDirectCfg) return stem_ok(p);
     return (cfg >= 0 && cfg < kNumMfmaCfgs) || (cfg >= kMfma3Cfg0 && cfg < kDirectCfg);
@@ -261,7 +265,8 @@
 int conv_num_configs() { return kDirectCfg + 1; }
 const char* conv_config_name(int cfg) {
     if (cfg == kDirectCfg) return "direct_valu";
-    if (cfg >= kDmabCfg0 && cfg < kDirectCfg) return dma_config_name(cfg - kDmabCfg0, 1);
+    if (cfg >= kDmahCfg0 && cfg < kDirectCfg) return dmah_config_name(cfg - kDmahCfg0);
+    if (cfg >= kDmabCfg0 && cfg < kDmahCfg0) return dma_config_name(cfg - kDmabCfg0, 1);
     if (cfg >= kDma3Cfg0 && cfg < kDmabCfg0) return dma_config_name(cfg - kDma3Cfg0, 3);
     if (cfg >= kBf16Cfg0 && cfg < kDma3Cfg0) return bf16_config_name(cfg - kBf16Cfg0);
     if (cfg >= kMfma3Cfg0 && cfg < kBf16Cfg0) return mfma3_config_name(cfg - kMfma3Cfg0);
@@ -272,9 +277,9 @@
 }
 
 bool conv_config_allowed(int cfg, int precision) {
-    const bool bf16 = (cfg >= kBf16Cfg0 && cfg < kDma3Cfg0) || (cfg >= kDmabCfg0 && cfg < kDirectCfg);
+    const bool bf16 = (cfg >= kBf16Cfg0 && cfg < kDma3Cfg0) || (cfg >= kDmabCfg0 && cfg < kDmahCfg0);
     if (!precision) return !bf16;
-    const bool split = (cfg >= kMfma3Cfg0 && cfg < kBf16Cfg0) || (cfg >= kDma3Cfg0 && cfg < kDmabCfg0);
+    const bool split = (cfg >= kMfma3Cfg0 && cfg < kBf16Cfg0) || (cfg >= kDma3Cfg0 && cfg < kDmabCfg0) || conv_config_is_dmah(cfg);
     const bool wino = cfg >= kNumMfmaCfgs && cfg < kSkinnyCfg0;
     return !split && !wino;
 }
@@ -285,7 +290,8 @@
 
 bool conv_config_valid(int cfg, const ConvParams& p) {
     if (cfg == kDirectCfg) return (size_t)p.K * ((p.Cout + 3) & ~3) * 4 <= 64 * 1024;
-    if (cfg >= kDmabCfg0 && cfg < kDirectCfg) return dma_config_valid(cfg - kDmabCfg0, 1, p);
+    if (cfg >= kDmahCfg0 && cfg < kDirectCfg) return dmah_config_valid(cfg - kDmahCfg0, p);
+    if (cfg >= kDmabCfg0 && cfg < kDmahCfg0) return dma_config_valid(cfg - kDmabCfg0, 1, p);
     if (cfg >= kDma3Cfg0 && cfg < kDmabCfg0) return dma_config_valid(cfg - kDma3Cfg0, 3, p);
     if (cfg >= kBf16Cfg0 && cfg < kDma3Cfg0) return mfma3_config_valid(cfg - kBf16Cfg0, p);
     if (cfg >= kMfma3Cfg0 && cfg < kBf16Cfg0) return mfma3_config_valid(cfg - kMfma3Cfg0, p);
@@ -336,7 +342,8 @@
 }
 
 long conv_grid_blocks(int cfg, const ConvParams& p) {
-    if (cfg >= kDmabCfg0 && cfg < kDirectCfg) return dma_grid_blocks(cfg - kDmabCfg0, p);
+    if (cfg >= kDmahCfg0 && cfg < kDirectCfg) return dma_grid_blocks(dmah_tile_index(cfg - kDmahCfg0), p);
+    if (cfg >= kDmabCfg0 && cfg < kDmahCfg0) return dma_grid_blocks(cfg - kDmabCfg0, p);
     if (cfg >= kDma3Cfg0 && cfg < kDmabCfg0) return dma_grid_blocks(cfg - kDma3Cfg0, p);
     if (cfg >= kBf16Cfg0 && cfg < kDma3Cfg0) return mfma3_grid_blocks(cfg - kBf16Cfg0, p);
     if (cfg >= kMfma3Cfg0 && cfg < kBf16Cfg0) return mfma3_grid_blocks(cfg - kMfma3Cfg0, p);
@@ -347,7 +354,8 @@
     return ((p.M + g.BM - 1) / g.BM) * ((p.Cout + g.BN - 1) / g.BN);
 }
 int conv_k_tiles(int cfg, const ConvParams& p) {
-    if (cfg >= kDma3Cfg0 && cfg < kDirectCfg) return dma_k_tiles(cfg >= kDmabCfg0 ? 1 : 3, p);
+    if (cfg >= kDmahCfg0 && cfg < kDirectCfg) return dmah_k_tiles(cfg - kDmahCfg0, p);
+    if (cfg >= kDma3Cfg0 && cfg < kDmahCfg0) return dma_k_tiles(cfg >= kDmabCfg0 ? 1 : 3, p);
     if (cfg >= kMfma3Cfg0 && cfg < kDma3Cfg0) return mfma3_k_tiles(p);
     if (cfg >= kSkinnyCfg0 && cfg < kMfma3Cfg0) return p.K / 16;
     if (cfg >= kNumMfmaCfgs && cfg < kSkinnyCfg0) return wino_k_tiles(p);
@@ -368,7 +376,12 @@
     }
     SSD_UNSUPPORTED_IF(!p.out && !(p.op && !p.n_split && (p.Cout & 3) == 0 && conv_config_writes_planes(cfg, p)),
                        "conv2d: config %s cannot write a plane-only output", conv_config_name(cfg));
-    if (cfg >= kDma3Cfg0 && cfg < kDirectCfg) {
+    if (cfg >= kDmahCfg0 && cfg < kDirectCfg) {
+        const int rc = dmah_launch(p, cfg - kDmahCfg0, st);
+        if (rc || p.split_k <= 1) return rc;
+        return launch_splitk_reduce(p, st);
+    }
+    if (cfg >= kDma3Cfg0 && cfg < kDmahCfg0) {
         const bool b1 = cfg >= kDmabCfg0;
         const int rc = dma_launch(p, cfg - (b1 ? kDmabCfg0 : kDma3Cfg0), b1 ? 1 : 3, st);
         if (rc || p.split_k <= 1) return rc;
@@ -539,20 +552,78 @@
 }
 
 int ssd_join_planes(const void* planes_dev, long n, int channels, int planes, long plane_stride, float* x_dev, void* stream) {
-    SSD_CHECK_ARG(x_dev && planes_dev && n >= 0 && (planes == 1 || planes == 3) && plane_stride >= n, "ssd_join_planes: bad arguments");
+    SSD_CHECK_ARG(x_dev && planes_dev && n >= 0 && planes >= 1 && planes <= 3 && plane_stride >= n, "ssd_join_planes: bad arguments");
     return launch_join_planes(static_cast<const short*>(planes_dev), n, channels, planes, plane_stride, x_dev, (hipStream_t)stream);
 }
+
+size_t ssd_conv_f16x2_weight_bytes(int kh, int kw, int Cin, int Cout) {
+    if (kh < 1 || kw < 1 || Cin < 1 || Cout < 1) return 0;
+    return conv_f16x2_plane_shorts(kh * kw * Cin, Cout) * sizeof(short);
+}
+
+int ssd_conv_pack_weights_f16x2(const float* packed_w_dev, int kh, int kw, int Cin, int Cout, void* w_planes_dev, int* k_out,
+                                void* stream) {
+    SSD_CHECK_ARG(packed_w_dev && w_planes_dev && k_out, "ssd_conv_pack_weights_f16x2: NULL pointer");
+    SSD_CHECK_ARG(kh >= 1 && kw >= 1 && Cin >= 1 && Cout >= 1, "ssd_conv_pack_weights_f16x2: bad shape");
+    SSD_CHECK_ARG(((uintptr_t)w_planes_dev & 15) == 0, "ssd_conv_pack_weights_f16x2: the planes must be 16-byte aligned");
+    const int K = kh * kw * Cin;
+    hipStream_t st = (hipStream_t)stream;
+    unsigned* bits_dev = nullptr;
+    unsigned bits = 0;
+    SSD_HIP(hipMalloc((void**)&bits_dev, sizeof(unsigned)));
+    int rc = hipMemsetAsync(bits_dev, 0, sizeof(unsigned), st) == hipSuccess ? SSD_OK : SSD_E_HIP;
+    if (!rc) rc = launch_absmax_bits(packed_w_dev, K, Cout, bits_dev, st);
+    if (!rc && (hipMemcpyAsync(&bits, bits_dev, sizeof(unsigned), hipMemcpyDeviceToHost, st) != hipSuccess ||
+                hipStreamSynchronize(st) != hipSuccess)) rc = SSD_E_HIP;
+    (void)hipFree(bits_dev);
+    if (rc) return rc;
+    SSD_UNSUPPORTED_IF(bits >= 0x7f800000u, "ssd_conv_pack_weights_f16x2: a non-finite weight: the layer cannot take the two-plane fp16 tiles");
+    *k_out = conv_f16x2_weight_exp(bits);
+    return launch_pack_f16x2(packed_w_dev, K, Cout, *k_out, static_cast<short*>(w_planes_dev), st);
+}
+
+static int conv2d_planes_impl(const ssd_conv_desc* d, const void* in_planes_dev, int planes, long in_plane_stride,
+                              const float* packed_w_dev, const void* w_planes_dev, int w_exp, const float* scale_dev,
+                              const float* shift_dev, const float* residual_dev, float* out_dev, long out_batch_stride,
+                              long out_pixel_stride, void* out_planes_dev, long out_plane_stride, int config, int split_k,
+                              float* splitk_ws_dev, void* stream);
 
 int ssd_conv2d_planes(const ssd_conv_desc* d, const void* in_planes_dev, int planes, long in_plane_stride,
                       const float* packed_w_dev, const float* scale_dev, const float* shift_dev, const float* residual_dev,
                       float* out_dev, long out_batch_stride, long out_pixel_stride, void* out_planes_dev,
                       long out_plane_stride, int config, int split_k, float* splitk_ws_dev, void* stream) {
+    return conv2d_planes_impl(d, in_planes_dev, planes, in_plane_stride, packed_w_dev, nullptr, 0, scale_dev, shift_dev, residual_dev,
+                              out_dev, out_batch_stride, out_pixel_stride, out_planes_dev, out_plane_stride, config, split_k,
+                              splitk_ws_dev, stream);
+}
+
+int ssd_conv2d_planes_f16x2(const ssd_conv_desc* d, const void* in_planes_dev, long in_plane_stride, const float* packed_w_dev,
+                            const void* w_planes_dev, int w_exp, const float* scale_dev, const float* shift_dev,
+                            const float* residual_dev, float* out_dev, long out_batch_stride, long out_pixel_stride,
+                            void* out_planes_dev, long out_plane_stride, int config, int split_k, float* splitk_ws_dev,
+                            void* stream) {
+    SSD_CHECK_ARG(w_planes_dev != nullptr, "conv2d_planes_f16x2: the fp16 weight planes are NULL");
+    SSD_CHECK_ARG(w_exp >= -100 && w_exp <= 100, "conv2d_planes_f16x2: weight exponent %d out of range", w_exp);
+    return conv2d_planes_impl(d, in_planes_dev, 2, in_plane_stride, packed_w_dev, w_planes_dev, w_exp, scale_dev, shift_dev,
+                              residual_dev, out_dev, out_batch_stride, out_pixel_stride, out_planes_dev, out_plane_stride, config,
+                              split_k, splitk_ws_dev, stream);
+}
+
+static int conv2d_planes_impl(const ssd_conv_desc* d, const void* in_planes_dev, int planes, long in_plane_stride,
+                              const float* packed_w_dev, const void* w_planes_dev, int w_exp, const float* scale_dev,
+                              const float* shift_dev, const float* residual_dev, float* out_dev, long out_batch_stride,
+                              long out_pixel_stride, void* out_planes_dev, long out_plane_stride, int config, int split_k,
+                              float* splitk_ws_dev, void* stream) {
     ConvParams p;
     int rc = fill_conv_params(d, &p);
     if (rc) return rc;
     if (p.M == 0) return SSD_OK;
     SSD_CHECK_ARG(in_planes_dev && packed_w_dev && (out_dev || out_planes_dev), "conv2d_planes: NULL pointer");
-    SSD_CHECK_ARG(planes == 1 || planes == 3, "conv2d_planes: planes must be 1 (bf16 mode) or 3 (exact split)");
+    SSD_CHECK_ARG(planes >= 1 && planes <= 3, "conv2d_planes: planes must be 1 (bf16 mode), 2 (fp16 pair) or 3 (exact split)");
+    if (w_planes_dev) {
+        p.wh = static_cast<const short*>(w_planes_dev);
+        p.acc_scale = ldexpf(1.f, -(8 + w_exp));
+    }
     SSD_CHECK_ARG(in_plane_stride >= (long)p.B * p.H * p.W * p.Cin, "conv2d_planes: in_plane_stride shorter than the tensor");
     SSD_CHECK_ARG(!d->has_residual || residual_dev, "conv2d_planes: has_residual set but residual is NULL");
     SSD_CHECK_ARG(config >= 0 && config < conv_num_configs() && conv_config_is_dma(config), "conv2d_planes: config %d is not an LDS-DMA tile", config);
diff --git a/tf-ssd_amd/csrc/ssd_convdma.hip b/tf-ssd_amd/csrc/ssd_convdma.hip
--- a/tf-ssd_amd/csrc/ssd_convdma.hip
+++ b/tf-ssd_amd/csrc/ssd_convdma.hip
@@ -3,9 +3,9 @@
 
 namespace ssd {
 
-template <int MT, int NT, int WM, int WN, int NP, bool GEMM1X1>
+template <int MT, int NT, int WM, int WN, int NP, bool GEMM1X1, int KSH = 1>
 __device__ __forceinline__ void conv_dma_body(const ConvParams& p, char* __restrict__ dsm) {
-    constexpr int KS = NP == 1 ? 2 : 1;
+    constexpr int KS = NP == 1 ? 2 : NP == 2 ? KSH : 1;
     constexpr int WPL = NP == 1 ? 3 : 0;
     constexpr int BM = 16 * MT * WM, BN = 16 * NT * WN, NW = WM * WN;
     constexpr int RBX = BM / 16, RBW = BN / 16;
@@ -34,7 +34,7 @@
     for (int pl = 0; pl < NP; ++pl)
         xrs[pl] = __builtin_amdgcn_make_buffer_rsrc(const_cast<short*>(p.xp + pl * p.xp_plane + xbase_e), 0, (int)xrange, 0x00020000);
     const long wplane_b = (long)p.Npad * p.Kpad * 2;
-    const __amdgpu_buffer_rsrc_t wrs = __builtin_amdgcn_make_buffer_rsrc(const_cast<short*>(p.w3), 0, (int)(4 * wplane_b), 0x00020000);
+    const __amdgpu_buffer_rsrc_t wrs = __builtin_amdgcn_make_buffer_rsrc(const_cast<short*>(NP == 2 ? p.wh : p.w3), 0, (int)((NP == 2 ? 2 : 4) * wplane_b), 0x00020000);
 
     int xoff[RPX];
     unsigned xvalid[RPX];
@@ -71,7 +71,8 @@
     }
 
     const int nks = p.K / 32;
-    const int ntiles = GEMM1X1 ? (nks + KS - 1) / KS : ntaps * (p.Cin / (32 * KS));
+    const int nsl = p.Cin / 32;
+    const int ntiles = GEMM1X1 ? (nks + KS - 1) / KS : ntaps * (NP == 2 ? (nsl + KS - 1) / KS : p.Cin / (32 * KS));
     int kt_begin = 0, kt_end = ntiles;
     if (p.split_k > 1) {
         const int per = (ntiles + p.split_k - 1) / p.split_k;
@@ -108,7 +109,11 @@
             l_xs = (l_ci >> 5) * slice_b;
         }
     };
-    auto steps_here = [&]() -> int { return KS == 1 ? 1 : min(KS, nks - l_k0 / 32); };
+    auto steps_here = [&]() -> int {
+        if (KS == 1) return 1;
+        if (NP == 2 && !GEMM1X1) return min(KS, nsl - (l_ci >> 5));
+        return min(KS, nks - l_k0 / 32);
+    };
 
     auto issue = [&](int stage) {
         char* sb = dsm + stage * STAGE;
@@ -197,13 +202,19 @@
         asm volatile("s_waitcnt vmcnt(0)" ::: "memory");
         __syncthreads();
     }
+    if constexpr (NP == 2) {
+#pragma unroll
+        for (int mi = 0; mi < MT; ++mi)
+#pragma unroll
+            for (int ni = 0; ni < NT; ++ni) acc[mi][ni] *= p.acc_scale;
+    }
     conv_epilogue<MT, NT>(p, acc, m0, n0, wm, wn, lane, HoWo);
 }
 
-template <int MT, int NT, int WM, int WN, int NP, bool GEMM1X1>
+template <int MT, int NT, int WM, int WN, int NP, bool GEMM1X1, int KSH = 1>
 __global__ __launch_bounds__(64 * WM * WN) void conv_dma_kernel(const ConvParams p) {
     extern __shared__ __attribute__((aligned(1024))) char dsm_dma[];
-    conv_dma_body<MT, NT, WM, WN, NP, GEMM1X1>(p, dsm_dma);
+    conv_dma_body<MT, NT, WM, WN, NP, GEMM1X1, KSH>(p, dsm_dma);
 }
 
 namespace {
@@ -212,13 +223,23 @@
 struct ConvDCfg {
     const char* name3;
     const char* name1;
+    const char* nameh;
+    const char* nameh2;
     int BM, BN, threads;
-    convd_kernel_t gemm3, general3, gemm1, general1;
+    convd_kernel_t gemm3, general3, gemm1, general1, gemmh, generalh, gemmh2, generalh2;
 };
+template <int MT, int NT, int WM, int WN, bool GEMM1X1>
+constexpr convd_kernel_t dmah_ks2_kernel() {
+    if constexpr (16 * MT * WM + 16 * NT * WN <= 320) return conv_dma_kernel<MT, NT, WM, WN, 2, GEMM1X1, 2>;
+    else return nullptr;
+}
 #define DCFG(MT, NT, WM, WN)                                                                                  \
-    {"dma3_" #MT "x" #NT "_" #WM "x" #WN, "dmab_" #MT "x" #NT "_" #WM "x" #WN, 16 * MT * WM, 16 * NT * WN, 64 * WM * WN, \
+    {"dma3_" #MT "x" #NT "_" #WM "x" #WN, "dmab_" #MT "x" #NT "_" #WM "x" #WN, "dmah_" #MT "x" #NT "_" #WM "x" #WN,          \
+     "dmah_" #MT "x" #NT "_" #WM "x" #WN "_ks2", 16 * MT * WM, 16 * NT * WN, 64 * WM * WN,                       \
      conv_dma_kernel<MT, NT, WM, WN, 3, true>, conv_dma_kernel<MT, NT, WM, WN, 3, false>,                       \
-     conv_dma_kernel<MT, NT, WM, WN, 1, true>, conv_dma_kernel<MT, NT, WM, WN, 1, false>}
+     conv_dma_kernel<MT, NT, WM, WN, 1, true>, conv_dma_kernel<MT, NT, WM, WN, 1, false>,                       \
+     conv_dma_kernel<MT, NT, WM, WN, 2, true>, conv_dma_kernel<MT, NT, WM, WN, 2, false>,                       \
+     dmah_ks2_kernel<MT, NT, WM, WN, true>(), dmah_ks2_kernel<MT, NT, WM, WN, false>()}
 const ConvDCfg kCfgD[] = {
     DCFG(4, 4, 4, 2),
     DCFG(2, 4, 4, 2),
@@ -236,6 +257,18 @@
     DCFG(2, 5, 6, 2),
 };
 constexpr int kNumCfgD = sizeof(kCfgD) / sizeof(kCfgD[0]);
+struct DmahList {
+    int n = 0, tile[2 * kNumCfgD], ks[2 * kNumCfgD];
+    DmahList() {
+        for (int i = 0; i < kNumCfgD; ++i) { tile[n] = i; ks[n++] = 1; }
+        for (int i = 0; i < kNumCfgD; ++i)
+            if (kCfgD[i].gemmh2) { tile[n] = i; ks[n++] = 2; }
+    }
+};
+const DmahList& dmah_list() {
+    static const DmahList l;
+    return l;
+}
 
 bool cd_gemm1x1(const ConvParams& p) {
     return p.kh == 1 && p.kw == 1 && p.stride == 1 && p.pad_t == 0 && p.pad_l == 0 && p.Ho == p.H && p.Wo == p.W;
@@ -254,6 +287,10 @@
     for (long e = (long)blockIdx.x * 256 + threadIdx.x; e < n; e += (long)gridDim.x * 256) {
         const long pix = e / C;
         const long s = plane_elem(pix, (int)(e - pix * C), P);
+        if (np == 2) {
+            x[e] = join_h(planes[s], planes[plane + s]);
+            continue;
+        }
         float v = __uint_as_float((unsigned)(unsigned short)planes[s] << 16);
         if (np == 3) {
             v += __uint_as_float((unsigned)(unsigned short)planes[plane + s] << 16);
@@ -263,14 +300,32 @@
     }
 }
 
+__global__ __launch_bounds__(256) void absmax_bits_kernel(const float* __restrict__ w, const long total, unsigned* __restrict__ out) {
+    unsigned m = 0;
+    for (long e = (long)blockIdx.x * 256 + threadIdx.x; e < total; e += (long)gridDim.x * 256) m = max(m, __float_as_uint(w[e]) & 0x7fffffffu);
+    atomicMax(out, m);
+}
+__global__ __launch_bounds__(256) void pack_f16x2_kernel(const float* __restrict__ w, const long total, const int Kpad, const int Npad,
+                                                         const float scale, short* __restrict__ out) {
+    for (long e = (long)blockIdx.x * 256 + threadIdx.x; e < total; e += (long)gridDim.x * 256) {
+        const long n = e / Kpad;
+        const long d = plane_elem(n, (int)(e - n * Kpad), Npad);
+        unsigned h, l;
+        split_h2(w[e] * scale, 0.f, h, l);
+        out[d] = (short)(h & 0xffffu);
+        out[total + d] = (short)(l & 0xffffu);
+    }
+}
+
 }
 
 int dma_num_configs() { return kNumCfgD; }
 const char* dma_config_name(int i, int np) { return (i >= 0 && i < kNumCfgD) ? (np == 1 ? kCfgD[i].name1 : kCfgD[i].name3) : "?"; }
 bool dma_config_valid(int i, int np, const ConvParams& p) {
     if (i < 0 || i >= kNumCfgD) return false;
-    if (!p.xp || !p.w3 || p.xp_np != np) return false;
-    if (((uintptr_t)p.xp & 15) || ((uintptr_t)p.w3 & 15) || (p.xp_plane & 7)) return false;
+    const short* wpl = np == 2 ? p.wh : p.w3;
+    if (!p.xp || !wpl || p.xp_np != np) return false;
+    if (((uintptr_t)p.xp & 15) || ((uintptr_t)wpl & 15) || (p.xp_plane & 7)) return false;
     if (p.M > 0x7fffffffL - 1024) return false;
     if (4 * (long)p.Npad * p.Kpad * 2 > 0x7fffffffL) return false;
     if ((long)p.B * p.H * p.W * p.Cin * 2 > 0x7fffffffL) return false;
@@ -306,8 +361,60 @@
     return SSD_OK;
 }
 
+int dmah_num_configs() { return dmah_list().n; }
+const char* dmah_config_name(int j) {
+    const DmahList& l = dmah_list();
+    return (j >= 0 && j < l.n) ? (l.ks[j] == 2 ? kCfgD[l.tile[j]].nameh2 : kCfgD[l.tile[j]].nameh) : "?";
+}
+int dmah_tile_index(int j) { return (j >= 0 && j < dmah_list().n) ? dmah_list().tile[j] : -1; }
+bool dmah_config_valid(int j, const ConvParams& p) {
+    if (j < 0 || j >= dmah_list().n) return false;
+    if (!(p.acc_scale > 0.f)) return false;
+    return dma_config_valid(dmah_list().tile[j], 2, p);
+}
+int dmah_k_tiles(int j, const ConvParams& p) {
+    const int ks = (j >= 0 && j < dmah_list().n) ? dmah_list().ks[j] : 1;
+    if (cd_gemm1x1(p)) return ((p.K + 31) / 32 + ks - 1) / ks;
+    return p.kh * p.kw * ((p.Cin / 32 + ks - 1) / ks);
+}
+int dmah_launch(const ConvParams& p, int j, hipStream_t st) {
+    if (!dmah_config_valid(j, p)) {
+        set_error("conv2d: two-plane fp16 LDS-DMA config %d cannot run Cin=%d k=%dx%d (input planes %s, %d of them; fp16 weight planes %s)", j,
+                  p.Cin, p.kh, p.kw, p.xp ? "present" : "missing", p.xp_np, p.wh ? "present" : "missing");
+        return SSD_E_UNSUPPORTED;
+    }
+    const int i = dmah_list().tile[j], ks = dmah_list().ks[j];
+    const long blocks = dma_grid_blocks(i, p);
+    SSD_UNSUPPORTED_IF(blocks > 0x7fffffffL, "conv2d: grid too large");
+    const ConvDCfg& g = kCfgD[i];
+    const convd_kernel_t fn = ks == 2 ? (cd_gemm1x1(p) ? g.gemmh2 : g.generalh2) : (cd_gemm1x1(p) ? g.gemmh : g.generalh);
+    const int lds = 2 * ks * 2 * (g.BM + g.BN) * 64;
+    if (lds > 64 * 1024) SSD_HIP(hipFuncSetAttribute(reinterpret_cast<const void*>(fn), hipFuncAttributeMaxDynamicSharedMemorySize, lds));
+    dim3 grid((unsigned)blocks, p.split_k > 1 ? p.split_k : 1);
+    hipLaunchKernelGGL(fn, grid, dim3(g.threads), lds, st, p);
+    SSD_LAUNCH_CHECK();
+    return SSD_OK;
+}
+
+int launch_absmax_bits(const float* packed, int K, int Cout, unsigned* absmax_bits_dev, hipStream_t st) {
+    const long total = (long)conv_kpad(K) * conv_npad(Cout);
+    if (total == 0) return SSD_OK;
+    const int blocks = (int)((total + 255) / 256 < 1024 ? (total + 255) / 256 : 1024);
+    hipLaunchKernelGGL(absmax_bits_kernel, dim3(blocks), dim3(256), 0, st, packed, total, absmax_bits_dev);
+    SSD_LAUNCH_CHECK();
+    return SSD_OK;
+}
+int launch_pack_f16x2(const float* packed, int K, int Cout, int k, short* planes, hipStream_t st) {
+    const long total = (long)conv_kpad(K) * conv_npad(Cout);
+    if (total == 0) return SSD_OK;
+    const int blocks = (int)((total + 255) / 256 < 8192 ? (total + 255) / 256 : 8192);
+    hipLaunchKernelGGL(pack_f16x2_kernel, dim3(blocks), dim3(256), 0, st, packed, total, conv_kpad(K), conv_npad(Cout), ldexpf(1.f, k), planes);
+    SSD_LAUNCH_CHECK();
+    return SSD_OK;
+}
+
 int launch_split_planes(const float* x, long n, int C, int np, short* planes, long plane, hipStream_t st) {
-    SSD_CHECK_ARG(n % 4 == 0 && (np == 1 || np == 3), "split_planes: element count %ld must be a multiple of 4, planes 1 or 3", n);
+    SSD_CHECK_ARG(n % 4 == 0 && np >= 1 && np <= 3, "split_planes: element count %ld must be a multiple of 4, planes 1, 2 or 3", n);
     SSD_CHECK_ARG(C > 0 && C % 32 == 0 && n % C == 0, "split_planes: %d channels (slice-major planes need a multiple of 32 that divides the %ld elements)", C, n);
     SSD_UNSUPPORTED_IF((((uintptr_t)x) & 15) || (((uintptr_t)planes) & 7) || (plane & 3),
                        "split_planes: needs a 16-byte aligned source and 8-byte aligned planes (16-byte loads, 8-byte stores)");
diff --git a/tf-ssd_amd/csrc/ssd_imgblock.hip b/tf-ssd_amd/csrc/ssd_imgblock.hip
--- a/tf-ssd_amd/csrc/ssd_imgblock.hip
+++ b/tf-ssd_amd/csrc/ssd_imgblock.hip
@@ -163,7 +163,7 @@
             if (p.e_out && real[t]) {
                 const long eo = ((long)img * H * W + opix[t]) * p.Ce + cbeg + j * kIC + g4 * 4;
                 if (!(p.planes_only & 2)) *reinterpret_cast<f32x4*>(p.e_out + eo) = v;
-                if (p.e_planes) store_planes4(p.e_planes, p.e_plane, p.planes_np, (long)img * H * W + opix[t], cbeg + j * kIC + g4 * 4, (long)B * H * W, v);
+                if (p.e_planes) store_planes4(p.e_planes, p.e_plane, p.e_planes_np, (long)img * H * W + opix[t], cbeg + j * kIC + g4 * 4, (long)B * H * W, v);
             }
         }
     };
@@ -462,7 +462,7 @@
             if (p.e_out && real[t]) {
                 const long eo = ((long)img * H * W + opix[t]) * p.Ce + cbeg + j * kIC + g4 * 4;
                 if (!(p.planes_only & 2)) *reinterpret_cast<f32x4*>(p.e_out + eo) = v;
-                if (p.e_planes) store_planes4(p.e_planes, p.e_plane, p.planes_np, (long)img * H * W + opix[t], cbeg + j * kIC + g4 * 4, (long)B * H * W, v);
+                if (p.e_planes) store_planes4(p.e_planes, p.e_plane, p.e_planes_np, (long)img * H * W + opix[t], cbeg + j * kIC + g4 * 4, (long)B * H * W, v);
             }
         }
     };
diff --git a/tf-ssd_amd/csrc/ssd_imgblock2.hip b/tf-ssd_amd/csrc/ssd_imgblock2.hip
--- a/tf-ssd_amd/csrc/ssd_imgblock2.hip
+++ b/tf-ssd_amd/csrc/ssd_imgblock2.hip
@@ -147,7 +147,7 @@
             if (S == 2 && p.e_out && real[t]) {
                 const int ch = cbeg + (j >> 1) * 32 + g4 * 8 + (j & 1) * 4;
                 if (!(p.planes_only & 2)) *reinterpret_cast<f32x4*>(p.e_out + ((long)img * (H * W) + opix[t]) * p.Ce + ch) = v;
-                if (p.e_planes) store_planes4(p.e_planes, p.e_plane, p.planes_np, (long)img * (H * W) + opix[t], ch, (long)B * (H * W), v);
+                if (p.e_planes) store_planes4(p.e_planes, p.e_plane, p.e_planes_np, (long)img * (H * W) + opix[t], ch, (long)B * (H * W), v);
             }
         }
     };
diff --git a/tf-ssd_amd/csrc/ssd_net.h b/tf-ssd_amd/csrc/ssd_net.h
--- a/tf-ssd_amd/csrc/ssd_net.h
+++ b/tf-ssd_amd/csrc/ssd_net.h
@@ -33,6 +33,7 @@
     short* planes = nullptr;
     long plane_stride = 0;
     int planes_np = 0;
+    int planes_cap = 0;
     bool planes_live = false;
     bool plane_only = false;
 };
@@ -55,6 +56,8 @@
     float* shift = nullptr;
     int cfg = -1;
     int split_k = 1;
+    float* wh = nullptr;
+    int wh_k = 0;
     int f_expand = -1, f_dw = -1, f_project = -1;
     int f_type = 0;
     int fused_by = -1;
@@ -124,6 +127,7 @@
     bool image_split = true;
     bool image_v2 = true;
     bool conv_dma = true;
+    bool conv_f16x2 = true;
     bool plane_only = true;
     bool image_ticket = false;
     float* img_slabs = nullptr;
@@ -133,6 +137,7 @@
     std::vector<float*> owned;
     float* arena = nullptr;
     size_t arena_bytes = 0, plane_bytes = 0, slab_bytes = 0;
+    size_t wplane_bytes = 0;
     float* splitk_ws = nullptr;
     size_t splitk_floats = 0;
     float* deltas = nullptr;
diff --git a/tf-ssd_amd/csrc/ssd_net.hip b/tf-ssd_amd/csrc/ssd_net.hip
--- a/tf-ssd_amd/csrc/ssd_net.hip
+++ b/tf-ssd_amd/csrc/ssd_net.hip
@@ -287,6 +287,10 @@
     p.w = l.packed;
     p.w3 = conv_split_planes(l.packed, l.kh * l.kw * l.Cin, l.Cout);
     p.bf16 = net.precision;
+    if (l.wh) {
+        p.wh = reinterpret_cast<const short*>(l.wh);
+        p.acc_scale = ldexpf(1.f, -(8 + l.wh_k));
+    }
     if (l.in >= 0 && net.tensors[l.in].planes) {
         const Tensor& ti = net.tensors[l.in];
         p.xp = ti.planes; p.xp_plane = ti.plane_stride; p.xp_np = ti.planes_np;
@@ -342,7 +346,7 @@
     }
     if (f.e_out >= 0 && net.tensors[f.e_out].planes_live) {
         const Tensor& te = net.tensors[f.e_out];
-        p.e_planes = te.planes; p.e_plane = te.plane_stride; p.planes_np = te.planes_np;
+        p.e_planes = te.planes; p.e_plane = te.plane_stride; p.e_planes_np = te.planes_np;
     }
     if (f.route == RT_IMAGE || f.route == RT_IMAGE_SPLIT)
         p.planes_only = (p.y_planes && net.tensors[f.out].plane_only ? 1 : 0) | (p.e_planes && net.tensors[f.e_out].plane_only ? 2 : 0);
@@ -529,6 +533,23 @@
     }
     for (int t = 0; t < nt; ++t) ok[t] = ok[t] && readers[t];
     return ok;
+}
+
+static bool tensor_relu6_bounded(const ssd_net& net, int t) {
+    if (net.precision != 0 || t < 1) return false;
+    bool any = false;
+    for (const Layer& l : net.layers) {
+        if (l.kind == LK_FUSED && l.e_out == t) {
+            const Layer& le = net.layers[l.f_expand];
+            if (le.act != SSD_ACT_RELU6 || le.res >= 0) return false;
+            any = true;
+            continue;
+        }
+        if (l.out != t) continue;
+        if (l.kind != LK_CONV || l.act != SSD_ACT_RELU6 || l.res >= 0 || l.head_kind != 0) return false;
+        any = true;
+    }
+    return any;
 }
 
 static int dev_alloc(ssd_net& net, size_t floats, float** out) {
@@ -605,7 +626,10 @@
     int rc = SSD_OK;
     const bool dbg_sync = getenv("SSD_HIP_DEBUG_SYNC") != nullptr;
     const bool dbg_tune = getenv("SSD_HIP_DEBUG_TUNE") != nullptr;
-    struct Best { float ms[2] = {1e30f, 1e30f}; int cfg[2] = {-1, -1}; int split[2] = {1, 1}; bool timed = false; };
+    struct Best {
+        float ms[3] = {1e30f, 1e30f, 1e30f}; int cfg[3] = {-1, -1, -1}; int split[3] = {1, 1, 1}; bool timed = false;
+        float ms_k64 = 1e30f, ms_k32 = 1e30f;
+    };
     std::vector<Best> bests(net.layers.size());
     constexpr int kReps = 4;
     for (size_t li = 0; li < net.layers.size(); ++li) {
@@ -618,11 +642,13 @@
         float* out = l.out >= 0 ? net.tensors[l.out].dev : nullptr;
         const float* res = l.res >= 0 ? net.tensors[l.res].dev : nullptr;
         for (int c = 0; c < conv_num_configs() && !rc; ++c) {
-            const int fam = conv_config_is_dma(c) ? 1 : 0;
+            const int fam = conv_config_is_dmah(c) ? 2 : conv_config_is_dma(c) ? 1 : 0;
+            if (fam == 2 && (!net.conv_f16x2 || !l.wh)) continue;
             for (int si = 0; si < kNumSplits && !rc; ++si) {
                 const int split = kSplits[si];
                 l.split_k = split;
                 ConvParams p = layer_conv_params(net, l, B, in, out, res, d, pr);
+                if (fam == 2) p.xp_np = 2;
                 if (!conv_config_valid(c, p) || !conv_config_allowed(c, net.precision)) break;
                 const bool direct = (c == conv_num_configs() - 1);
                 if (direct && (bb.cfg[0] >= 0 || bb.cfg[1] >= 0 || split > 1)) break;
@@ -651,6 +677,10 @@
                 }
                 if (rc) break;
                 if (ms < bb.ms[fam]) { bb.ms[fam] = ms; bb.cfg[fam] = c; bb.split[fam] = split; }
+                if (fam == 2) {
+                    float& m2 = strstr(conv_config_name(c), "_ks2") ? bb.ms_k64 : bb.ms_k32;
+                    m2 = ms < m2 ? ms : m2;
+                }
             }
         }
         if (rc) break;
@@ -663,9 +693,13 @@
         l.cfg = bb.cfg[f0];
         l.split_k = bb.split[f0];
         if (dbg_tune)
-            fprintf(stderr, "[ssd] tune %s: %s/s%d %.4f ms | %s/s%d %.4f ms\n", l.name.c_str(), bb.cfg[0] >= 0 ? conv_config_name(bb.cfg[0]) : "-",
-                    bb.split[0], bb.cfg[0] >= 0 ? bb.ms[0] / kReps : 0.f, bb.cfg[1] >= 0 ? conv_config_name(bb.cfg[1]) : "-", bb.split[1],
-                    bb.cfg[1] >= 0 ? bb.ms[1] / kReps : 0.f);
+            fprintf(stderr, "[ssd] tune %s: %s/s%d %.4f ms | %s/s%d %.4f ms | %s/s%d %.4f ms\n", l.name.c_str(),
+                    bb.cfg[0] >= 0 ? conv_config_name(bb.cfg[0]) : "-", bb.split[0], bb.cfg[0] >= 0 ? bb.ms[0] / kReps : 0.f,
+                    bb.cfg[1] >= 0 ? conv_config_name(bb.cfg[1]) : "-", bb.split[1], bb.cfg[1] >= 0 ? bb.ms[1] / kReps : 0.f,
+                    bb.cfg[2] >= 0 ? conv_config_name(bb.cfg[2]) : "-", bb.split[2], bb.cfg[2] >= 0 ? bb.ms[2] / kReps : 0.f);
+        if (dbg_tune && bb.cfg[2] >= 0)
+            fprintf(stderr, "[ssd] tune %s: dmah best with one k-step per barrier %.4f ms, with two %.4f ms\n", l.name.c_str(),
+                    bb.ms_k32 / kReps, bb.ms_k64 < 1e29f ? bb.ms_k64 / kReps : 0.f);
     }
     if (rc) return rc;
     std::vector<int> img_saved;
@@ -678,36 +712,48 @@
         const Tensor& tt = net.tensors[t];
         std::vector<size_t> flip;
         bool planes_anyway = false;
-        double sum0 = 0, sum1 = 0;
+        bool pair_ok = net.conv_f16x2;
+        double sum0 = 0, sum1 = 0, sum2 = 0;
         for (size_t li = 0; li < net.layers.size(); ++li) {
             const Layer& l = net.layers[li];
             if (l.kind != LK_CONV || l.in != (int)t) continue;
             const Best& bb = bests[li];
-            if (!bb.timed) { if (layer_runs(l) && conv_config_is_dma(l.cfg)) planes_anyway = true; continue; }
+            if (!bb.timed) {
+                if (layer_runs(l) && conv_config_is_dma(l.cfg)) planes_anyway = true;
+                if (conv_config_is_dma(l.cfg) && !conv_config_is_dmah(l.cfg)) pair_ok = false;
+                continue;
+            }
             if (bb.cfg[1] < 0) continue;
-            if (bb.cfg[0] < 0) { planes_anyway = true; continue; }
+            if (bb.cfg[0] < 0) { planes_anyway = true; pair_ok = false; continue; }
             if (!layer_runs(l)) {
                 if (bb.ms[1] + kReps * ((double)B * tt.per_image * 2.0 * tt.planes_np / 3.0e12 * 1e3) < bb.ms[0]) {
                     net.layers[li].cfg = bb.cfg[1];
                     net.layers[li].split_k = bb.split[1];
+                    pair_ok = false;
                 }
                 continue;
             }
             flip.push_back(li);
             sum0 += bb.ms[0];
             sum1 += bb.ms[1];
+            sum2 += bb.ms[2];
+            if (bb.cfg[2] < 0) pair_ok = false;
         }
         if (flip.empty()) continue;
         for (size_t li : flip) { net.layers[li].cfg = bests[li].cfg[1]; net.layers[li].split_k = bests[li].split[1]; }
         const bool only = plane_only_candidates(net, [&](int i) { return conv_config_is_dma(net.layers[i].cfg); })[t];
-        const double bytes = only ? 2.0 * tt.planes_np - 4.0 : planes_anyway ? 0.0 : 2.0 * tt.planes_np;
-        const double store_ms = kReps * ((double)B * tt.per_image * bytes / 3.0e12 * 1e3);
-        const bool take = sum1 + store_ms < sum0;
-        if (!take)
-            for (size_t li : flip) { net.layers[li].cfg = bests[li].cfg[0]; net.layers[li].split_k = bests[li].split[0]; }
+        auto store_ms_of = [&](int np) {
+            const double bytes = only ? 2.0 * np - 4.0 : planes_anyway ? 0.0 : 2.0 * np;
+            return kReps * ((double)B * tt.per_image * bytes / 3.0e12 * 1e3);
+        };
+        const double store_ms = store_ms_of(tt.planes_np), store2_ms = store_ms_of(2);
+        int take = sum1 + store_ms < sum0 ? 1 : 0;
+        if (pair_ok && sum2 + store2_ms < (take ? sum1 + store_ms : sum0)) take = 2;
+        for (size_t li : flip) { net.layers[li].cfg = bests[li].cfg[take]; net.layers[li].split_k = bests[li].split[take]; }
         if (dbg_tune)
-            fprintf(stderr, "[ssd] tune tensor %s: fp32 readers %.4f ms, plane readers %.4f + store %+.4f ms (%s) -> %s\n", tt.name.c_str(),
-                    sum0 / kReps, sum1 / kReps, store_ms / kReps, only ? "plane-only" : "both copies", take ? "planes" : "fp32");
+            fprintf(stderr, "[ssd] tune tensor %s: fp32 readers %.4f ms, plane readers %.4f + store %+.4f ms, fp16-pair readers %.4f + store %+.4f ms%s (%s) -> %s\n",
+                    tt.name.c_str(), sum0 / kReps, sum1 / kReps, store_ms / kReps, sum2 / kReps, store2_ms / kReps, pair_ok ? "" : " [not open]",
+                    only ? "plane-only" : "both copies", take == 2 ? "fp16 pair" : take ? "planes" : "fp32");
     }
     for (size_t i = 0; i < net.layers.size(); ++i) net.layers[i].img_choice = img_saved[i];
     resolve_routes(net);
@@ -912,6 +958,24 @@
     }
     if (!rc) rc = launch_pack_split(l.packed, K, l.Cout, st);
     if (rc) return rc;
+    l.wh = nullptr;
+    l.wh_k = 0;
+    if (net->conv_dma && l.in >= 0 && l.Cin % 32 == 0 && tensor_relu6_bounded(*net, l.in)) {
+        ScopedDev bits_dev;
+        unsigned bits = 0;
+        SSD_HIP(hipMalloc((void**)&bits_dev.p, sizeof(unsigned)));
+        SSD_HIP(hipMemsetAsync(bits_dev.p, 0, sizeof(unsigned), st));
+        rc = launch_absmax_bits(l.packed, K, l.Cout, reinterpret_cast<unsigned*>(bits_dev.p), st);
+        if (rc) return rc;
+        SSD_HIP(hipMemcpyAsync(&bits, bits_dev.p, sizeof(unsigned), hipMemcpyDeviceToHost, st));
+        SSD_HIP(hipStreamSynchronize(st));
+        if (bits < 0x7f800000u) {
+            l.wh_k = conv_f16x2_weight_exp(bits);
+            rc = dev_alloc(*net, (conv_f16x2_plane_shorts(K, l.Cout) + 1) / 2, &l.wh);
+            if (!rc) rc = launch_pack_f16x2(l.packed, K, l.Cout, l.wh_k, reinterpret_cast<short*>(l.wh), st);
+            if (rc) return rc;
+        }
+    }
     if (l.kh == 3 && l.kw == 3 && l.stride == 1 && l.dil == 1 && l.Cin % 16 == 0 && l.res < 0 && net->use_wino) {
         const int np = conv_npad(l.Cout);
         rc = dev_alloc(*net, wino_weight_floats(l.Cin, l.Cout), &l.wino);
@@ -1025,13 +1089,13 @@
         off += align_up(t.per_image * max_batch, 64) + gap;
     }
     SSD_HIP(hipMemset(net->arena, poison ? 0xFF : 0, total * sizeof(float)));
-    for (auto& t : net->tensors) { t.planes = nullptr; t.planes_live = false; t.plane_only = false; t.planes_np = 0; t.plane_stride = 0; }
+    for (auto& t : net->tensors) { t.planes = nullptr; t.planes_live = false; t.plane_only = false; t.planes_np = t.planes_cap = 0; t.plane_stride = 0; }
     if (net->conv_dma)
         for (const auto& l : net->layers) {
             if (l.kind != LK_CONV || l.in < 0 || l.Cin % 32 != 0) continue;
             Tensor& t = net->tensors[l.in];
             if (t.planes) continue;
-            t.planes_np = net->precision ? 1 : 3;
+            t.planes_np = t.planes_cap = net->precision ? 1 : 3;
             t.plane_stride = (long)align_up(t.per_image * max_batch, 64);
             float* pl = nullptr;
             const int rcp = dev_alloc(*net, (size_t)t.planes_np * t.plane_stride / 2 + 64, &pl);
@@ -1054,12 +1118,17 @@
         int cfg = -1;
         for (int c = 0; c < conv_num_configs(); ++c)
             if (it->second.first == conv_config_name(c)) cfg = c;
+        SSD_UNSUPPORTED_IF(cfg >= 0 && conv_config_is_dmah(cfg) && net->precision != 0,
+                           "finalize: the table puts layer %s on %s: the two-plane fp16 tiles are admitted in fp32 nets (precision 0) only",
+                           l.name.c_str(), conv_config_name(cfg));
+        if (cfg >= 0 && conv_config_is_dmah(cfg) && (!net->conv_f16x2 || !l.wh)) cfg = conv_dmah_twin(cfg);
         if (cfg < 0 || !conv_config_allowed(cfg, net->precision)) { ++n_tuned; continue; }
         l.cfg = cfg;
         l.split_k = it->second.second;
         ConvParams p = layer_conv_params(*net, l, max_batch, net->tensors[l.in].dev,
                                          l.out >= 0 ? net->tensors[l.out].dev : nullptr, nullptr,
                                          net->arena, net->arena);
+        if (conv_config_is_dmah(cfg)) p.xp_np = 2;
         const bool split_ok = l.split_k == 1 || conv_k_tiles(cfg, p) >= l.split_k;
         if (l.split_k < 1 || !split_ok || !conv_config_valid(cfg, p)) { l.cfg = -1; l.split_k = 1; ++n_tuned; continue; }
         ++n_preset;
@@ -1091,18 +1160,41 @@
     for (const auto& l : net->layers)
         if (l.kind == LK_CONV && l.in >= 0 && conv_config_is_dma(l.cfg)) read[l.in] = 1;
     SSD_HIP(hipStreamSynchronize(st));
-    net->plane_bytes = 0;
+    net->plane_bytes = net->wplane_bytes;
     for (size_t i = 0; i < net->tensors.size(); ++i) {
         Tensor& t = net->tensors[i];
         if (!t.planes) continue;
-        const size_t bytes = ((size_t)t.planes_np * t.plane_stride / 2 + 64) * sizeof(float);
+        const size_t bytes = ((size_t)t.planes_cap * t.plane_stride / 2 + 64) * sizeof(float);
         if (read[i]) { net->plane_bytes += bytes; continue; }
         float* pl = reinterpret_cast<float*>(t.planes);
         net->owned.erase(std::remove(net->owned.begin(), net->owned.end(), pl), net->owned.end());
         (void)hipFree(pl);
-        t.planes = nullptr; t.planes_np = 0; t.plane_stride = 0;
+        t.planes = nullptr; t.planes_np = t.planes_cap = 0; t.plane_stride = 0;
     }
     return SSD_OK;
+}
+
+static void finalize_resolve_f16x2(ssd_net* net) {
+    const int nt = (int)net->tensors.size();
+    std::vector<char> any(nt, 0), all(nt, 1);
+    for (const auto& l : net->layers) {
+        if (l.kind != LK_CONV || l.in < 0 || !conv_config_is_dma(l.cfg)) continue;
+        any[l.in] = 1;
+        if (!conv_config_is_dmah(l.cfg) || !l.wh || !net->conv_f16x2) all[l.in] = 0;
+    }
+    net->wplane_bytes = 0;
+    for (auto& l : net->layers) {
+        if (l.kind != LK_CONV) continue;
+        if (conv_config_is_dmah(l.cfg) && !(any[l.in] && all[l.in])) l.cfg = conv_dmah_twin(l.cfg);
+        if (conv_config_is_dmah(l.cfg)) {
+            net->tensors[l.in].planes_np = 2;
+            net->wplane_bytes += (conv_f16x2_plane_shorts(l.kh * l.kw * l.Cin, l.Cout) + 1) / 2 * sizeof(float);
+        } else if (l.wh) {
+            net->owned.erase(std::remove(net->owned.begin(), net->owned.end(), l.wh), net->owned.end());
+            (void)hipFree(l.wh);
+            l.wh = nullptr;
+        }
+    }
 }
 
 static int finalize_streams(ssd_net* net, int max_batch) {
@@ -1144,6 +1236,7 @@
     for (auto& l : net->layers) {
         l.packed = l.scale = l.shift = nullptr;
         l.wino = nullptr;
+        l.wh = nullptr;
         l.splitk_part = nullptr;
         if (l.kind == LK_CONV) rc = finalize_pack_conv(net, l, st);
         if (!rc && (l.kind == LK_CONV || l.kind == LK_DW)) rc = finalize_fold_bn(net, l, st);
@@ -1155,6 +1248,10 @@
     bool image_preset_ok = true;
     if (!rc) rc = finalize_apply_preset(net, max_batch, &image_preset_ok);
     if (!rc && net->n_autotuned) rc = autotune(*net, max_batch, st);
+    if (!rc) {
+        SSD_HIP(hipStreamSynchronize(st));
+        finalize_resolve_f16x2(net);
+    }
     if (!rc) rc = finalize_free_unread_planes(net, st);
     if (!rc) rc = finalize_streams(net, max_batch);
     if (rc) return rc;
@@ -1500,6 +1597,7 @@
     {"use_wino", &ssd_net::use_wino, nullptr, 0, 1, 2},
     {"image_v2", &ssd_net::image_v2, nullptr, 0, 1, 0},
     {"conv_dma", &ssd_net::conv_dma, nullptr, 0, 1, 1},
+    {"conv_f16x2", &ssd_net::conv_f16x2, nullptr, 0, 1, 1},
     {"plane_only", &ssd_net::plane_only, nullptr, 0, 1, 0},
     {"use_graph", &ssd_net::use_graph, nullptr, 0, 1, 0},
 };
diff --git a/tf-ssd_amd/models/_net.py b/tf-ssd_amd/models/_net.py
--- a/tf-ssd_amd/models/_net.py
+++ b/tf-ssd_amd/models/_net.py
@@ -8,7 +8,7 @@
 import ssd_hip as _h
 
 _TABLE_OPTIONS = ("use_wino", "image_split", "conv_dma")
-_REFINALIZE_OPTIONS = ("precision", "image_split", "use_wino", "conv_dma")
+_REFINALIZE_OPTIONS = ("precision", "image_split", "use_wino", "conv_dma", "conv_f16x2")
 _STALE_WARNED = set()
 
 
diff --git a/tf-ssd_amd/ssd_hip.py b/tf-ssd_amd/ssd_hip.py
--- a/tf-ssd_amd/ssd_hip.py
+++ b/tf-ssd_amd/ssd_hip.py
@@ -198,6 +198,10 @@
     "ssd_join_planes": (ctypes.c_int, [vp, ctypes.c_long, ctypes.c_int, ctypes.c_int, ctypes.c_long, vp, vp]),
     "ssd_conv2d_planes": (ctypes.c_int, [ctypes.POINTER(ConvDesc), vp, ctypes.c_int, ctypes.c_long, vp, vp, vp, vp, vp,
                                          ctypes.c_long, ctypes.c_long, vp, ctypes.c_long, ctypes.c_int, ctypes.c_int, vp, vp]),
+    "ssd_conv_f16x2_weight_bytes": (ctypes.c_size_t, [ctypes.c_int] * 4),
+    "ssd_conv_pack_weights_f16x2": (ctypes.c_int, [vp] + [ctypes.c_int] * 4 + [vp, c_int_p, vp]),
+    "ssd_conv2d_planes_f16x2": (ctypes.c_int, [ctypes.POINTER(ConvDesc), vp, ctypes.c_long, vp, vp, ctypes.c_int, vp, vp, vp, vp,
+                                               ctypes.c_long, ctypes.c_long, vp, ctypes.c_long, ctypes.c_int, ctypes.c_int, vp, vp]),
     "ssd_conv_wino_weight_floats": (ctypes.c_size_t, [ctypes.c_int, ctypes.c_int]),
     "ssd_conv_wino_pack_weights": (ctypes.c_int, [vp, ctypes.c_int, ctypes.c_int, vp, vp]),
     "ssd_conv_wino_num_configs": (ctypes.c_int, []),
```
